# mushroomfire/mdapy

Measured on AMD Instinct MI355X. Metric: atoms/sec for neighbor+CNA on 10M-atom FCC Cu; 1/2/4/8-GPU scaling, higher is better.
Workload: dtype f64 (CNA pair tests: f32 filter + f64 finish, labels exact); 1 GPU; FCC Cu a=3.615, 136^3 cells per GPU (10061824 atoms/GPU, 10061824 total), build_neighbor(rc=0.854a=3.08721, max_neigh=16) + fixed-cutoff CNA as one C-ABI call (mdh_build_neighbor_fcna: lists and labels), positions resident in HBM; atoms_per_gpu=10061824, max_neigh=16, parallelism=single, world_size_checked=1, launched_by=single process

## Files before the change

### include/mdapy_amd.h

```cpp
#ifndef MDAPY_AMD_H
#define MDAPY_AMD_H

#include <stdint.h>

#ifdef __cplusplus
extern "C" {
#endif

#define MDH_HOST 0
#define MDH_DEVICE 1

#define MDH_OK 0
#define MDH_ERR_BOX (-1)
#define MDH_ERR_HIP (-2)
#define MDH_ERR_ARG (-3)
#define MDH_ERR_NOMEM (-4)

const char *mdh_last_error(void);
int mdh_version(void);
int mdh_device_count(void);
int mdh_set_device(int device);
int mdh_warm(void);
int mdh_min_max_i32(const int *v, int64_t n, int *min_max2, int space, void *stream);
int mdh_dense_codes_i32(const int *v, int64_t n, int low, int span, int *codes, int64_t *counts_span, int space, void *stream);
int mdh_release_workspace(void);
int64_t mdh_workspace_bytes(void);
int mdh_prof_enable(int on);
int mdh_prof_reset(void);
int mdh_prof_report(char *buf, int buflen);
int mdh_debug_set_neighbor_variant(int variant);
int mdh_debug_set_indirect(int on);
int mdh_debug_neighbor_plan(int *plan8);
int mdh_debug_set_fcna_variant(int variant);
int mdh_debug_track_counters(int on);
int mdh_debug_counters(int64_t *out4);
int mdh_debug_set_rdf_variant(int variant);
int mdh_debug_set_knn_variant(int variant);
int mdh_debug_set_sq_variant(int variant);
int mdh_debug_set_entropy_variant(int variant);
int mdh_debug_set_ptm_order_cap(int cap);
int mdh_debug_image_thresholds(double L, double *out4);

int mdh_parse_table(const char *text, int64_t nbytes, int text_space, int64_t nrows, int ncol, const int *kinds,
                    void *const *columns, int64_t *redo, int64_t redo_cap, int64_t *status4, int space, void *stream);
int mdh_debug_text_pow5(int q, uint64_t *out2);
int mdh_debug_parse_double(const char *s, int64_t len, double *out);
int64_t mdh_debug_assign_groups(const int *cells, int64_t n, int *head, int *count, int *rank);

int mdh_build_neighbor(const double *x, const double *y, const double *z, int64_t N, const double *box9,
                       const double *origin3, const int *boundary3, double rc, int *verlet, double *dist, int *nn,
                       int64_t max_neigh, int fill_pads, int space, void *stream);
int mdh_build_neighbor_keyed(const double *x, const double *y, const double *z, int64_t N, const double *box9,
                             const double *origin3, const int *boundary3, double rc, int *verlet, double *dist, int *nn,
                             int64_t max_neigh, int fill_pads, const int64_t *key, int space, void *stream);

int mdh_build_neighbor_fcna(const double *x, const double *y, const double *z, int64_t N, const double *box9,
                            const double *origin3, const int *boundary3, double rc, int *verlet, double *dist, int *nn,
                            int64_t max_neigh, int fill_pads, int *pattern, const int64_t *key, int space, void *stream);

int mdh_hint_cell_window(int axis, double frac_lo, double frac_hi);
int mdh_hint_centre_window(int axis, double frac_lo, double frac_hi);
int mdh_cell_window_check(void *stream);

int mdh_slab_halo_select(const double *x, const double *y, const double *z, int64_t n, const double *origin3_host,
                         const double *hi3_host, double up_from, double down_below, int *up, int *down, int64_t *counts_host,
                         const int64_t *gid, double *up_pack, double *down_pack, int64_t capacity, int space, void *stream);
int mdh_slab_halo_messages(const double *x, const double *y, const double *z, int64_t n, const double *origin3_host,
                           const double *hi3_host, double up_from, double down_below, const int64_t *gid,
                           const double *const *extras_host_array_of_device_pointers, int nextra, double *msg_up,
                           double *msg_down, int64_t cap, void *stream);
int mdh_slab_append_ghosts(const double *msg_from_left, const double *msg_from_right, int64_t cap, int64_t nl, int64_t nr,
                           double *const *columns_host_array_of_device_pointers, int ncol, int64_t *gid, int64_t n_owned,
                           void *stream);
int mdh_slab_append_ghosts_static(const double *msg_from_left, const double *msg_from_right, int64_t cap,
                                  double *const *columns_host_array_of_device_pointers, int ncol, int64_t *gid, int64_t n_owned,
                                  void *stream);
int mdh_slab_overflow_check(void);
int mdh_slab_reset_absent_rows(const double *x, int *verlet, double *dist, int *nn, int64_t first, int64_t n, int64_t max_neigh, double pad,
                               void *stream);

int mdh_order_statistic(const double *x, const double *y, const double *z, int64_t N, const double *box9, const double *origin3,
                        const int *boundary3, double *far_fraction, int space, void *stream);
int mdh_spatial_sort(const double *x, const double *y, const double *z, int64_t N, const double *box9, const double *origin3,
                     const int *boundary3, double *xs, double *ys, double *zs, int *perm, int64_t *n_sorted, int space, void *stream);
int mdh_permute(const void *in, const int *perm, int64_t N, int elem_bytes, int scatter, void *out, int space, void *stream);
int mdh_gather_positions(const double *x, const double *y, const double *z, const int *perm, int64_t N, double *xs, double *ys, double *zs,
                         int space, void *stream);
int mdh_translate_rows(const int *verlet_sorted, const double *dist_sorted, const int *nn_sorted, const int *perm, int64_t N,
                       int64_t M, int *verlet, double *dist, int *nn, int space, void *stream);

int mdh_neighbor_count(const double *x, const double *y, const double *z, int64_t N, const double *box9,
                       const double *origin3, const int *boundary3, double rc, int *nn, int *max_count, int space,
                       void *stream);

typedef int (*mdh_alloc_rows_fn)(void *user, int64_t N, int64_t M, int **verlet, double **dist);
int mdh_build_neighbor_exact(const double *x, const double *y, const double *z, int64_t N, const double *box9,
                             const double *origin3, const int *boundary3, double rc, int *nn, int64_t *width,
                             mdh_alloc_rows_fn alloc, void *user, int space, void *stream);
int mdh_build_neighbor_exact_keyed(const double *x, const double *y, const double *z, int64_t N, const double *box9,
                                   const double *origin3, const int *boundary3, double rc, int *nn, int64_t *width,
                                   mdh_alloc_rows_fn alloc, void *user, const int64_t *key, int space, void *stream);
int mdh_build_neighbor_exact_fcna(const double *x, const double *y, const double *z, int64_t N, const double *box9,
                                  const double *origin3, const int *boundary3, double rc, int *nn, int64_t *width,
                                  mdh_alloc_rows_fn alloc, void *user, int *pattern, const int64_t *key, int space, void *stream);

int mdh_sort_verlet_by_distance(int *verlet, double *dist, int64_t N, int64_t M, int sort_num, int space,
                                void *stream);

int mdh_wrap_positions(double *x, double *y, double *z, int64_t N, const double *box9, const double *origin3,
                       const int *boundary3, int space, void *stream);

int mdh_average_by_neighbor(double rc, const int *verlet, const double *dist, const int *nn, int64_t N, int64_t M,
                            const double *value, double *value_ave, int include_self, int space, void *stream);

// ... 153 lines not shown
```

### mdapy_amd/_lib.py

```python
from __future__ import annotations

import ctypes as C
import os

import numpy as np

_HERE = os.path.dirname(os.path.abspath(__file__))
LIB_PATH = os.path.join(_HERE, "csrc", "libmdapy_amd.so")

HOST, DEVICE = 0, 1
ERR_BOX, ERR_HIP, ERR_ARG, ERR_NOMEM = -1, -2, -3, -4

_lib = None

i64, dbl, cint, vp = C.c_int64, C.c_double, C.c_int, C.c_void_p
ALLOC_ROWS = C.CFUNCTYPE(C.c_int, C.c_void_p, C.c_int64, C.c_int64, C.POINTER(C.POINTER(C.c_int)), C.POINTER(C.POINTER(C.c_double)))

_SIGNATURES = {
    "mdh_last_error": [],
    "mdh_version": [],
    "mdh_device_count": [],
    "mdh_set_device": [cint],
    "mdh_warm": [],
    "mdh_min_max_i32": [vp, i64, vp, cint, vp],
    "mdh_dense_codes_i32": [vp, i64, cint, cint, vp, vp, cint, vp],
    "mdh_release_workspace": [],
    "mdh_workspace_bytes": [],
    "mdh_prof_enable": [cint],
    "mdh_prof_reset": [],
    "mdh_prof_report": [vp, cint],
    "mdh_debug_set_neighbor_variant": [cint],
    "mdh_debug_set_indirect": [cint],
    "mdh_debug_neighbor_plan": [vp],
    "mdh_debug_set_fcna_variant": [cint],
    "mdh_debug_track_counters": [cint],
    "mdh_debug_counters": [vp],
    "mdh_debug_set_rdf_variant": [cint],
    "mdh_debug_set_knn_variant": [cint],
    "mdh_debug_set_sq_variant": [cint],
    "mdh_debug_set_entropy_variant": [cint],
    "mdh_debug_set_ptm_order_cap": [cint],
    "mdh_debug_image_thresholds": [dbl, vp],
    "mdh_parse_table": [vp, i64, cint, i64, cint, vp, vp, vp, i64, vp, cint, vp],
    "mdh_debug_text_pow5": [cint, vp],
    "mdh_debug_parse_double": [C.c_char_p, i64, vp],
    "mdh_debug_assign_groups": [vp, i64, vp, vp, vp],
    "mdh_build_neighbor": [vp, vp, vp, i64, vp, vp, vp, dbl, vp, vp, vp, i64, cint, cint, vp],
    "mdh_slab_halo_select": [vp, vp, vp, i64, vp, vp, dbl, dbl, vp, vp, vp, vp, vp, vp, i64, cint, vp],
    "mdh_hint_cell_window": [cint, dbl, dbl],
    "mdh_hint_centre_window": [cint, dbl, dbl],
    "mdh_cell_window_check": [vp],
    "mdh_slab_halo_messages": [vp, vp, vp, i64, vp, vp, dbl, dbl, vp, vp, cint, vp, vp, i64, vp],
    "mdh_slab_append_ghosts": [vp, vp, i64, i64, i64, vp, cint, vp, i64, vp],
    "mdh_order_statistic": [vp, vp, vp, i64, vp, vp, vp, vp, cint, vp],
    "mdh_spatial_sort": [vp, vp, vp, i64, vp, vp, vp, vp, vp, vp, vp, vp, cint, vp],
    "mdh_permute": [vp, vp, i64, cint, cint, vp, cint, vp],
    "mdh_gather_positions": [vp, vp, vp, vp, i64, vp, vp, vp, cint, vp],
    "mdh_translate_rows": [vp, vp, vp, vp, i64, i64, vp, vp, vp, cint, vp],
    "mdh_slab_append_ghosts_static": [vp, vp, i64, vp, cint, vp, i64, vp],
    "mdh_slab_overflow_check": [],
    "mdh_slab_reset_absent_rows": [vp, vp, vp, vp, i64, i64, i64, dbl, vp],
    "mdh_build_neighbor_keyed": [vp, vp, vp, i64, vp, vp, vp, dbl, vp, vp, vp, i64, cint, vp, cint, vp],
    "mdh_build_neighbor_fcna": [vp, vp, vp, i64, vp, vp, vp, dbl, vp, vp, vp, i64, cint, vp, vp, cint, vp],
    "mdh_neighbor_count": [vp, vp, vp, i64, vp, vp, vp, dbl, vp, vp, cint, vp],
    "mdh_build_neighbor_exact": [vp, vp, vp, i64, vp, vp, vp, dbl, vp, vp, ALLOC_ROWS, vp, cint, vp],
    "mdh_build_neighbor_exact_keyed": [vp, vp, vp, i64, vp, vp, vp, dbl, vp, vp, ALLOC_ROWS, vp, vp, cint, vp],
    "mdh_build_neighbor_exact_fcna": [vp, vp, vp, i64, vp, vp, vp, dbl, vp, vp, ALLOC_ROWS, vp, vp, vp, cint, vp],
    "mdh_sort_verlet_by_distance": [vp, vp, i64, i64, cint, cint, vp],
    "mdh_wrap_positions": [vp, vp, vp, i64, vp, vp, vp, cint, vp],
    "mdh_average_by_neighbor": [dbl, vp, vp, vp, i64, i64, vp, vp, cint, cint, vp],
    "mdh_fcna": [vp, vp, vp, i64, vp, vp, vp, vp, i64, vp, vp, dbl, cint, vp],
    "mdh_acna": [vp, vp, vp, i64, vp, vp, vp, vp, i64, vp, cint, vp],
    "mdh_ids": [vp, vp, vp, i64, vp, vp, vp, vp, i64, vp, vp, cint, vp],
    "mdh_csp": [vp, vp, vp, i64, vp, vp, vp, vp, i64, cint, vp, cint, vp],
    "mdh_get_sq": [vp, vp, vp, i64, vp, vp, vp, vp, vp, i64, vp, vp, vp, cint, cint, cint, cint, cint, cint, cint,
                   dbl, cint, vp, vp, vp, cint, vp],
    "mdh_identify_solid_liquid": [cint, vp, vp, vp, vp, i64, i64, vp, vp, cint, cint, dbl, cint, vp, vp, cint, cint,
                                  dbl, cint, vp],
    "mdh_rdf": [vp, vp, vp, vp, i64, i64, vp, cint, dbl, cint, cint, vp],
    "mdh_rdf_single_species": [vp, vp, vp, i64, i64, vp, dbl, cint, cint, vp],
    "mdh_rdf_streaming": [vp, vp, vp, vp, i64, vp, vp, vp, vp, cint, dbl, cint, cint, vp],
    "mdh_bond_analysis": [vp, vp, vp, i64, vp, vp, vp, vp, vp, vp, i64, dbl, dbl, dbl, cint, vp, vp, cint, vp],
    "mdh_angular_distribution": [vp, vp, vp, i64, vp, vp, vp, vp, vp, vp, vp, i64, dbl, vp, vp, cint, cint, vp, cint, vp],
    "mdh_debug_angle_edges": [cint, dbl, vp],
    "mdh_debug_set_bond_variant": [cint],
    "mdh_strain_pack": [vp, vp, vp, i64, vp, vp, cint, vp],
    "mdh_atomic_strain_records": [vp, vp, i64, i64, vp, vp, vp, vp, vp, vp, vp, vp, vp, cint, vp],
    "mdh_atomic_strain": [vp, vp, i64, i64, vp, vp, vp, vp, vp, vp, vp, vp, vp, vp, vp, vp, vp, vp, cint, vp],
    "mdh_chill_plus": [vp, vp, vp, i64, vp, vp, vp, vp, vp, vp, i64, dbl, vp, cint, vp],
    "mdh_wcp": [vp, vp, vp, i64, i64, cint, vp, cint, vp],
    "mdh_wcp_counts": [vp, vp, vp, vp, i64, i64, cint, vp, cint, vp],
    "mdh_knn": [vp, vp, vp, i64, vp, vp, vp, cint, vp, vp, cint, vp],
    "mdh_knn_keyed": [vp, vp, vp, i64, vp, vp, vp, cint, vp, vp, vp, cint, vp],
    "mdh_knn_keyed_rows": [vp, vp, vp, i64, vp, vp, vp, cint, vp, vp, vp, vp, vp, cint, vp, cint, vp],
    "mdh_knn_rows_width": [cint],
    "mdh_repeat_cell": [vp, vp, vp, i64, cint, cint, cint, cint, vp],
    "mdh_ptm": [C.c_char_p, vp, vp, vp, i64, vp, vp, vp, vp, i64, vp, dbl, vp, cint, vp, cint, cint, vp],
    "mdh_ptm_flags": [C.c_char_p],
    "mdh_aja": [vp, vp, vp, i64, vp, vp, vp, vp, vp, i64, vp, cint, vp],
    "mdh_cnp": [vp, vp, vp, i64, vp, vp, vp, vp, vp, vp, i64, vp, dbl, cint, vp],
    "mdh_structure_entropy": [dbl, dbl, cint, dbl, vp, vp, i64, i64, vp, cint, vp],
    "mdh_atomic_temperature": [vp, vp, i64, i64, vp, vp, vp, vp, vp, dbl, cint, vp],
    "mdh_cluster": [vp, vp, vp, i64, i64, dbl, cint, vp, vp, cint, vp],
    "mdh_identify_sftb_fcc": [vp, i64, vp, vp, vp, i64, vp, cint, cint, vp],
    "mdh_filter_overlap_atom": [vp, vp, vp, i64, vp, vp, vp, dbl, vp, cint, vp],
    "mdh_voronoi_volume_number_radius": [vp, vp, vp, i64, vp, vp, vp, vp, vp, vp, cint, vp],
    "mdh_voronoi_neighbor_count": [vp, vp, vp, i64, vp, vp, vp, vp, vp, cint, vp],
    "mdh_voronoi_neighbor": [vp, vp, vp, i64, vp, vp, vp, dbl, dbl, vp, vp, vp, cint, cint, vp],
    "mdh_voronoi_neighbor_rows": [vp, vp, vp, i64, vp, vp, vp, dbl, dbl, vp, vp, vp, cint, vp, vp, cint, vp],
    "mdh_filter_overlap_atom_with_grain": [vp, vp, vp, vp, vp, i64, vp, vp, vp, dbl, dbl, dbl, vp, cint, vp],
    "mdh_transform_and_filter": [vp, vp, vp, i64, vp, vp, vp, vp, cint, vp, vp, cint, vp],
    "mdh_voronoi_cell_info": [vp, vp, vp, i64, vp, vp, vp, cint, cint, vp, vp, vp, vp, vp, vp, vp, cint, vp],
    "mdh_voronoi_row_distance": [vp, i64, cint, vp, vp, vp, vp, vp, vp, vp, cint, vp],
    "mdh_sfc_direct": [vp, vp, vp, i64, vp, vp, cint, dbl, dbl, vp, vp, vp, i64, C.c_uint, cint, vp],
    "mdh_sfc_direct_partial": [vp, vp, vp, vp, cint, i64, vp, vp, cint, dbl, dbl, cint, vp],
# ... 88 lines not shown
```

### mdapy_amd/csrc/cell_grid.hip

```cpp
#include "common.hpp"
#include "grid.hpp"
#include "assign_groups.hpp"
#include <algorithm>
#include <atomic>

namespace mdh {
static std::atomic<int> g_indirect{[] { const char *e = std::getenv("MDH_INDIRECT"); return e ? std::atoi(e) : 1; }()};

struct CellPlanes { int p0, p1, p2, p3; int *bad; };
template <bool TRI, int K>
__global__ __launch_bounds__(256) void k_assign(const double *__restrict__ x, const double *__restrict__ y,
                                                const double *__restrict__ z, int64_t N, DBox b, Grid g,
                                                int wrap_first, int2 *__restrict__ ent,
                                                unsigned *__restrict__ cell_count, unsigned *__restrict__ ctl, unsigned gen,
                                                double slack, unsigned short *__restrict__ mv, CellPlanes win,
                                                CellGrid::Packed *__restrict__ rec, int drop_absent)
{
    const int lane = threadIdx.x & 63;
    const int64_t i0 = ((int64_t)blockIdx.x * (blockDim.x >> 6) + (threadIdx.x >> 6)) * (64 * K) + lane;
    bool moved = false, outside = false, coded = false;
    double xr[K], yr[K], zr[K];
#pragma unroll
    for (int k = 0; k < K; ++k) {
        const int64_t i = i0 + 64 * k;
        xr[k] = yr[k] = zr[k] = 0.0;
        if (i < N) { xr[k] = x[i]; yr[k] = y[i]; zr[k] = z[i]; }
    }
    int cells[K];
#pragma unroll
    for (int k = 0; k < K; ++k) {
        const int64_t i = i0 + 64 * k;
        int cell = -1 - lane;
        const bool absent = drop_absent && i < N && xr[k] != xr[k];
        if (absent && mv) mv[i] = (unsigned short)img::ATOM_NEUTRAL;
        if (i < N && !absent) {
            double xi = xr[k], yi = yr[k], zi = zr[k];
            int code = img::ATOM_NEUTRAL;
            if (wrap_first && b.anypbc) {
                wrap<TRI>(b, xi, yi, zi);
                if (!TRI) {
                    const double raw[3] = {xr[k], yr[k], zr[k]}, wrp[3] = {xi, yi, zi};
                    code = 0;
#pragma unroll
                    for (int d = 0; d < 3; ++d) {
                        double m = 0.0;
                        if (b.pbc[d] && raw[d] != wrp[d]) {
                            m = rint((raw[d] - wrp[d]) / b.h[d * 4]);
                            if (!(fabs(m) <= (double)img::MAX_M) || !(fabs(raw[d] - m * b.h[d * 4] - wrp[d]) <= slack)) { moved = true; m = 0.0; }
                        }
                        code |= ((int)m + 15) << (5 * d);
                    }
                }
            }
            if (mv) mv[i] = (unsigned short)code;
            if (rec) rec[i] = CellGrid::Packed{xr[k], yr[k], zr[k], (int)i, code};
            coded = coded || code != img::ATOM_NEUTRAL;
            int c0, c1, c2;
            cell_coords<TRI>(b, g, xi, yi, zi, c0, c1, c2);
            cell = (c0 * g.nc[1] + c1) * g.nc[2] + c2;
            if (win.bad && !((c0 >= win.p0 && c0 < win.p1) || (c0 >= win.p2 && c0 < win.p3))) {
                outside = true;
                cell = -1 - lane;
            }
        }
        cells[k] = cell;
    }
    unsigned base[K];
    int head[K], slot[K];
#pragma unroll
    for (int k = 0; k < K; ++k) {
        const int cell = cells[k];
        const int c1 = __shfl_up(cell, 1, 64);
        const unsigned eq = assign_groups::equal_bits(cell, c1, __shfl_up(cell, 2, 64), __shfl_up(cell, 3, 64), lane);
        const unsigned long long primary = __ballot(eq == 0);
        int d = assign_groups::member_distance(eq, primary, lane);
        const bool start = assign_groups::starts_run(cell, c1, lane);
        const unsigned long long starts = __ballot(start);
        int count;
        if (assign_groups::use_runs(__popcll(__ballot(start && cell >= 0)), __popcll(__ballot(d == 0 && cell >= 0))))
            d = assign_groups::run_distance(starts, lane, &count, &slot[k]);
        else
            assign_groups::count_and_rank(d, __ballot(d == 1), __ballot(d == 2), __ballot(d == 3), lane, &count, &slot[k]);
        head[k] = lane - d;
        base[k] = 0;
        if (d == 0 && cell >= 0)
            base[k] = atomicAdd(&cell_count[cell], (unsigned)count);
    }
#pragma unroll
    for (int k = 0; k < K; ++k) {
        const unsigned bs = __shfl(base[k], head[k], 64);
        const int64_t i = i0 + 64 * k;
        if (i < N)
            ent[i] = make_int2(cells[k], (int)(bs + (unsigned)slot[k]));
    }
    if (__any(moved) && lane == 0)
        ctl[1] = gen;
    if (__any(coded) && lane == 0)
        ctl[2] = gen;
    if (__any(outside) && lane == 0)
        *win.bad = 1;
}

static constexpr int SCAN_BLOCK = 256;
static constexpr int SCAN_ITEMS = 4;
static constexpr int SCAN_ITEMS_BIG = 32;
static constexpr int64_t SCAN_BIG_FROM = 1 << 19;

__device__ __forceinline__ unsigned wave_incl_scan(unsigned v, int lane)
{
#pragma unroll
    for (int d = 1; d < 64; d <<= 1) {
        unsigned t = __shfl_up(v, d, 64);
        if (lane >= d) v += t;
    }
    return v;
}

__device__ __forceinline__ unsigned block_excl_scan(unsigned v, unsigned *tot)
{
    __shared__ unsigned wsum[4];
    const int lane = threadIdx.x & 63, w = threadIdx.x >> 6;
    unsigned inc = wave_incl_scan(v, lane);
    if (lane == 63) wsum[w] = inc;
    __syncthreads();
    unsigned off = 0, t = 0;
#pragma unroll
    for (int k = 0; k < 4; ++k) {
        if (k < w) off += wsum[k];
        t += wsum[k];
    }
    __syncthreads();
    *tot = t;
    return off + inc - v;
}

static std::atomic<unsigned> g_scan_gen{0};
static unsigned next_scan_gen()
{
    unsigned g = (++g_scan_gen) & 0x3fffffffu;
    if (g == 0) {
        reset_kept_blocks(Scope::KEEP_SCAN);
        g = (++g_scan_gen) & 0x3fffffffu;
    }
    return g;
}

template <bool REZERO, int ITEMS = SCAN_ITEMS>
__global__ __launch_bounds__(SCAN_BLOCK) void k_scan_onepass(unsigned *__restrict__ in, int *__restrict__ out, int64_t n,
                                                             unsigned *__restrict__ ctl, unsigned gen, int *__restrict__ flags)
{
    constexpr int SCAN_ITEMS = ITEMS;
    __shared__ unsigned s_blk, s_excl;
    unsigned long long *status = reinterpret_cast<unsigned long long *>(ctl + 64);
    const int tid = threadIdx.x, lane = tid & 63;
    if (tid == 0) s_blk = atomicAdd(&ctl[0], 1u);
    __syncthreads();
    const unsigned blk = s_blk, nblk = gridDim.x;
    if (tid == 0) {
        if (blk == nblk - 1) ctl[0] = 0;
        if (blk == 0 && flags) {
            flags[0] = ctl[1] == gen ? 1 : 0; flags[1] = 0; flags[2] = 0; flags[3] = 0;
            flags[4] = ctl[2] == gen ? 1 : 0; flags[5] = 0; flags[6] = 0; flags[7] = 0;
        }
    }
    const int64_t base = ((int64_t)blk * SCAN_BLOCK + tid) * SCAN_ITEMS;
    unsigned v[SCAN_ITEMS], s = 0;
    const bool vec = base + SCAN_ITEMS <= n && ((reinterpret_cast<uintptr_t>(in + base) | reinterpret_cast<uintptr_t>(out + base)) & 15u) == 0;
    if (vec) {
#pragma unroll
        for (int c = 0; c < SCAN_ITEMS / 4; ++c) {
            const uint4 q = reinterpret_cast<const uint4 *>(in + base)[c];
            v[4 * c] = q.x; v[4 * c + 1] = q.y; v[4 * c + 2] = q.z; v[4 * c + 3] = q.w;
        }
        if (REZERO) {
// ... 64 lines not shown
}

static size_t scan_ctl_bytes(int64_t n)
{
    const int64_t per = (int64_t)SCAN_BLOCK * SCAN_ITEMS;
    return 256 + (size_t)((n + per - 1) / per) * 8;
}
static void launch_scan_gen(hipStream_t st, unsigned *in, int *out, int64_t n, unsigned *ctl, unsigned gen, bool rezero, int *flags)
{
    const bool big = n >= SCAN_BIG_FROM;
    const int64_t per = (int64_t)SCAN_BLOCK * (big ? SCAN_ITEMS_BIG : SCAN_ITEMS);
    const dim3 grid((unsigned)std::max<int64_t>(1, (n + per - 1) / per)), block(SCAN_BLOCK);
    if (big) {
        if (rezero) hipLaunchKernelGGL((k_scan_onepass<true, SCAN_ITEMS_BIG>), grid, block, 0, st, in, out, n, ctl, gen, flags);
        else hipLaunchKernelGGL((k_scan_onepass<false, SCAN_ITEMS_BIG>), grid, block, 0, st, in, out, n, ctl, gen, flags);
    } else {
        if (rezero) hipLaunchKernelGGL((k_scan_onepass<true, SCAN_ITEMS>), grid, block, 0, st, in, out, n, ctl, gen, flags);
        else hipLaunchKernelGGL((k_scan_onepass<false, SCAN_ITEMS>), grid, block, 0, st, in, out, n, ctl, gen, flags);
    }
}
static void launch_scan(hipStream_t st, unsigned *in, int *out, int64_t n, unsigned *ctl, bool rezero, int *flags)
{
    launch_scan_gen(st, in, out, n, ctl, next_scan_gen(), rezero, flags);
}

int exclusive_scan_u32(Scope &sc, const unsigned *in, int *out, int64_t n)
{
    unsigned *ctl = static_cast<unsigned *>(sc.alloc_kept(scan_ctl_bytes(n), Scope::KEEP_SCAN));
    if (sc.failed())
        return sc.error();
    launch_scan(sc.stream(), const_cast<unsigned *>(in), out, n, ctl, false, nullptr);
    MDH_HIP(hipGetLastError());
    return MDH_OK;
}

__global__ __launch_bounds__(256) void k_scatter(const int2 *__restrict__ ent, const int *__restrict__ cell_start,
                                                 int *__restrict__ order, int64_t N)
{
    const int64_t i = 2 * ((int64_t)blockIdx.x * blockDim.x + threadIdx.x);
    if (i >= N)
        return;
    int4 e;
    if (i + 1 < N) e = *reinterpret_cast<const int4 *>(ent + i);
    else { const int2 last = ent[i]; e = make_int4(last.x, last.y, -1, 0); }
    if (e.x >= 0)
        order[cell_start[e.x] + e.y] = (int)i;
    if (e.z >= 0)
        order[cell_start[e.z] + e.w] = (int)(i + 1);
}

template <int W, typename K>
__device__ __forceinline__ void sort_cell_net(int *__restrict__ order, int s, int n, const int64_t *__restrict__ key)
{
    int id[W];
    K k[W];
#pragma unroll
    for (int u = 0; u < W; ++u) id[u] = order[s + min(u, n - 1)];
#pragma unroll
    for (int u = 0; u < W; ++u) {
        const K v = key ? (K)key[id[u]] : (K)id[u];
        k[u] = u < n ? v : (sizeof(K) == 8 ? (K)INT64_MIN : (K)INT32_MIN);
    }
    auto ce = [&](int a, int b) {
        const bool sw = k[a] < k[b];
        const K ka = sw ? k[b] : k[a], kb = sw ? k[a] : k[b];
        const int ia = sw ? id[b] : id[a], ib = sw ? id[a] : id[b];
        k[a] = ka; k[b] = kb; id[a] = ia; id[b] = ib;
    };
    if (W == 4) {
        ce(0, 1); ce(2, 3); ce(0, 2); ce(1, 3); ce(1, 2);
    } else {
        ce(0, 1); ce(2, 3); ce(4, 5); ce(6, 7);
        ce(0, 2); ce(1, 3); ce(4, 6); ce(5, 7);
        ce(1, 2); ce(5, 6);
        ce(0, 4); ce(1, 5); ce(2, 6); ce(3, 7);
        ce(2, 4); ce(3, 5);
        ce(1, 2); ce(3, 4); ce(5, 6);
    }
#pragma unroll
    for (int u = 0; u < W; ++u)
        if (u < n) order[s + u] = id[u];
}

__global__ __launch_bounds__(256) void k_sort_cells(const int *__restrict__ cell_start, int *__restrict__ order,
                                                    int64_t ncell, const int64_t *__restrict__ key, int *__restrict__ tmp)
{
    int64_t c = (int64_t)blockIdx.x * blockDim.x + threadIdx.x;
    if (c >= ncell)
        return;
    const int s = cell_start[c], e = cell_start[c + 1];
    const int n = e - s;
    if (n <= 1)
        return;
    if (n <= 4) {
        if (key) sort_cell_net<4, int64_t>(order, s, n, key);
        else sort_cell_net<4, int>(order, s, n, nullptr);
        return;
    }
    if (n <= 8) {
        if (key) sort_cell_net<8, int64_t>(order, s, n, key);
        else sort_cell_net<8, int>(order, s, n, nullptr);
        return;
    }
    if (!key && tmp) {
        for (int a = s; a < e; ++a) tmp[a] = order[a];
        for (int a = s; a < e; ++a) {
            const int mine = tmp[a];
            int larger = 0;
            for (int q = s; q < e; ++q) larger += tmp[q] > mine ? 1 : 0;
            order[s + larger] = mine;
        }
        return;
    }
    for (int a = s + 1; a < e; ++a) {
        int v = order[a], q = a - 1;
        const int64_t kv = key ? key[v] : (int64_t)v;
        while (q >= s && (key ? key[order[q]] : (int64_t)order[q]) < kv) {
            order[q + 1] = order[q];
            --q;
        }
        order[q + 1] = v;
    }
}

constexpr int SORT_DENSE_CAP = 64;
__global__ __launch_bounds__(256) void k_sort_cells_dense(const int *__restrict__ cell_start, int *__restrict__ order, int64_t ncell,
                                                          int *__restrict__ tmp)
{
    __shared__ int ids[32 * SORT_DENSE_CAP];
    const int sub = threadIdx.x & 7, lc = threadIdx.x >> 3;
    const int64_t c = (int64_t)blockIdx.x * 32 + lc;
    int s = 0, n = 0;
    if (c < ncell) {
        s = cell_start[c];
        n = cell_start[c + 1] - s;
    }
    const bool staged = n > 1 && n <= SORT_DENSE_CAP, big = n > SORT_DENSE_CAP;
    if (staged)
        for (int a = sub; a < n; a += 8) ids[lc * SORT_DENSE_CAP + a] = order[s + a];
    if (big)
        for (int a = sub; a < n; a += 8) tmp[s + a] = order[s + a];
    __syncthreads();
    if (staged) {
        for (int a = sub; a < n; a += 8) {
            const int mine = ids[lc * SORT_DENSE_CAP + a];
            int larger = 0;
            for (int q = 0; q < n; ++q) larger += ids[lc * SORT_DENSE_CAP + q] > mine ? 1 : 0;
            order[s + larger] = mine;
        }
    } else if (big) {
        for (int a = sub; a < n; a += 8) {
            const int mine = tmp[s + a];
            int larger = 0;
            for (int q = 0; q < n; ++q) larger += tmp[s + q] > mine ? 1 : 0;
            order[s + larger] = mine;
        }
    }
}

__global__ __launch_bounds__(256) void k_gather(const double *__restrict__ x, const double *__restrict__ y,
                                                const double *__restrict__ z, const int *__restrict__ order,
                                                double *__restrict__ xs, double *__restrict__ ys,
                                                double *__restrict__ zs, int64_t N,
                                                const unsigned short *__restrict__ mv, unsigned short *__restrict__ mvs,
                                                CellGrid::Packed *__restrict__ pk, const int *__restrict__ any_code,
                                                const int *__restrict__ n_binned)
{
    int64_t p = (int64_t)blockIdx.x * blockDim.x + threadIdx.x;
    if (p >= N)
        return;
    if (n_binned && p >= *n_binned)
        return;
    const int i = order[p];

    const double a = x[i], b = y[i], c = z[i];
    const unsigned short m = *any_code ? mv[i] : (unsigned short)img::ATOM_NEUTRAL;
    if (pk) {
        pk[p] = CellGrid::Packed{a, b, c, i, (int)m};
        return;
    }
    xs[p] = a;
    ys[p] = b;
    zs[p] = c;
    mvs[p] = m;
}

__global__ __launch_bounds__(256) void k_gather_records(const CellGrid::Packed *__restrict__ rec, const int *__restrict__ order,
                                                        CellGrid::Packed *__restrict__ pk, int64_t N, const int *__restrict__ n_binned)
{
    const int64_t p = (int64_t)blockIdx.x * blockDim.x + threadIdx.x;
    if (p >= N || p >= *n_binned)
        return;
    pk[p] = rec[order[p]];
}

__global__ __launch_bounds__(256) void k_unpack(const CellGrid::Packed *__restrict__ pk, int64_t N, double *__restrict__ xs,
                                                double *__restrict__ ys, double *__restrict__ zs, unsigned short *__restrict__ mvs)
{
    const int64_t p = (int64_t)blockIdx.x * blockDim.x + threadIdx.x;
    if (p >= N)
        return;
    const CellGrid::Packed r = pk[p];
    xs[p] = r.x; ys[p] = r.y; zs[p] = r.z; mvs[p] = (unsigned short)r.code;
}

int ensure_unpacked(Scope &sc, CellGrid &cg, int64_t N)
{
    if ((!cg.pk && !cg.ix) || cg.xs)
        return MDH_OK;
    cg.xs = sc.alloc_n<double>((size_t)N);
    cg.ys = sc.alloc_n<double>((size_t)N);
    cg.zs = sc.alloc_n<double>((size_t)N);
    cg.mvs = sc.alloc_n<unsigned short>((size_t)N);
    if (sc.failed())
        return sc.error();
    if (cg.pk)
        hipLaunchKernelGGL(k_unpack, dim3(grid_for(N, 256)), dim3(256), 0, sc.stream(), cg.pk, N, cg.xs, cg.ys, cg.zs, cg.mvs);
    else
        hipLaunchKernelGGL(k_gather, dim3(grid_for(N, 256)), dim3(256), 0, sc.stream(), cg.ix, cg.iy, cg.iz, cg.order, cg.xs, cg.ys, cg.zs, N, cg.imv,
                           cg.mvs, (CellGrid::Packed *)nullptr, cg.flags + 4, cg.cell_start + cg.g.ncell);
    MDH_HIP(hipGetLastError());
    return MDH_OK;
}

struct CellWindow { int axis = 0; double lo = 0.0, hi = 0.0; bool set = false; };
struct PendingWindows { CellWindow cells, centre; };
static thread_local PendingWindows g_pending;
static thread_local int *g_window_violations = nullptr;

static int take_pending_windows(PendingWindows &w)
{
    w = g_pending;
    g_pending = PendingWindows{};
    if (g_window_violations && *(volatile int *)g_window_violations != 0) {
        *g_window_violations = 0;
        set_error("an earlier neighbor build on this thread found atoms outside the cell window it had been promised (mdh_hint_cell_window)");
        return MDH_ERR_ARG;
    }
    return MDH_OK;
}
// ... 7 lines not shown
        return;
    }
    const int64_t a4 = (a + 3) & ~(int64_t)3, b4 = b & ~(int64_t)3;
    const int64_t q = a4 + 4 * i;
    if (q + 4 <= b4) *reinterpret_cast<int4 *>(out + q) = make_int4(val, val, val, val);
    if (i < 4) {
        if (a + i < a4) out[a + i] = val;
        if (b4 + i < b) out[b4 + i] = val;
    }
}
__global__ __launch_bounds__(256) void k_fill_outside(int *__restrict__ out, int64_t a0, int64_t a1, int64_t n1, const int *__restrict__ v)
{
    const int val = *v;
    const int64_t q = 4 * ((int64_t)blockIdx.x * blockDim.x + threadIdx.x);
    const int64_t head4 = (a0 + 3) >> 2 << 2;
    const int64_t t0 = (a1 + 1 + 3) & ~(int64_t)3;
    if (q < head4) {
        if (q + 4 <= a0) *reinterpret_cast<int4 *>(out + q) = make_int4(0, 0, 0, 0);
        else for (int64_t i = q; i < a0; ++i) out[i] = 0;
        return;
    }
    const int64_t r = q - head4 + t0;
    if (r == t0) for (int64_t i = a1 + 1; i < t0 && i < n1; ++i) out[i] = val;
    if (r + 4 <= n1) *reinterpret_cast<int4 *>(out + r) = make_int4(val, val, val, val);
    else for (int64_t i = r; i < n1; ++i) out[i] = val;
}
static void fill_from(hipStream_t st, int *out, int64_t a, int64_t b, const int *v)
{
    if (b > a)
        hipLaunchKernelGGL(k_fill_from, dim3(grid_for((b - a) / 4 + 8, 256)), dim3(256), 0, st, out, a, b, v);
}

__global__ __launch_bounds__(256) void k_add_from(int *__restrict__ out, int64_t a, int64_t b, const int *__restrict__ v, int64_t skip)
{
    const int64_t i = a + (int64_t)blockIdx.x * blockDim.x + threadIdx.x;
    if (i < b && i != skip) out[i] += *v;
}

int neighbor_grid_dims(const DBox &b, double rc, Grid &g)
{
    double nc_total = 1.0;
    for (int d = 0; d < 3; ++d) {
        double f = std::floor(b.thick[d] / rc);
        if (!(f < 2147483647.0)) { set_error("cell grid too large (box thickness / rc overflows int)"); return MDH_ERR_ARG; }
        int n = (int)f;
        g.nc[d] = n > 3 ? n : 3;
        nc_total *= (double)g.nc[d];
    }
    if (nc_total > 2147483000.0) {
        set_error("cell grid too large: " + std::to_string(nc_total) + " cells (the reference indexes cells with int32)");
        return MDH_ERR_ARG;
    }
    g.ncell = (int64_t)g.nc[0] * g.nc[1] * g.nc[2];
    g.rc_inv = 1.0 / rc;
    g.mode = 0;
    return MDH_OK;
}

__global__ __launch_bounds__(1024) void k_order_far_flag(const double *__restrict__ x, const double *__restrict__ y, const double *__restrict__ z,
                                                         int64_t N, DBox b, double nb0, double nb1, double nb2, int *__restrict__ flag)
{
    __shared__ int s_far;
    if (threadIdx.x == 0) s_far = 0;
    __syncthreads();
    const int64_t step = (N - 1) / 1024 > 0 ? (N - 1) / 1024 : 1;
    const int64_t i = (int64_t)threadIdx.x * step;
    bool far = false;
    if (i + 1 < N) {
        const double dx = x[i + 1] - x[i], dy = y[i + 1] - y[i], dz = z[i + 1] - z[i];
        double f[3] = {dx * b.hi[0] + dy * b.hi[3] + dz * b.hi[6], dx * b.hi[1] + dy * b.hi[4] + dz * b.hi[7], dx * b.hi[2] + dy * b.hi[5] + dz * b.hi[8]};
        const double nb[3] = {nb0, nb1, nb2};
#pragma unroll
        for (int d = 0; d < 3; ++d) {
            if (b.pbc[d]) f[d] -= rint(f[d]);
            far = far || !(fabs(f[d]) * nb[d] <= 2.0);
        }
    }
    const unsigned long long m = __ballot(far);
    if ((threadIdx.x & 63) == 0 && m) atomicAdd(&s_far, __popcll(m));
    __syncthreads();
    if (threadIdx.x == 0) *flag = 4 * s_far > 1024 ? 1 : 0;
}

int build_cell_grid(Scope &sc, const double *x, const double *y, const double *z, int64_t N, const DBox &b, const GridRequest &rq,
                    CellGrid &cg)
{
    PendingWindows hints;
    MDH_TRY(take_pending_windows(hints));
    const CellWindow &window = hints.cells, &centre = hints.centre;
    const bool packed = rq.atoms != GridRequest::SORTED_ARRAYS;
    bool scattered = rq.atoms == GridRequest::FOR_ROWS_UNORDERED;
    const Grid &g = cg.g;
    hipStream_t st = sc.stream();

    unsigned *cell_count = static_cast<unsigned *>(sc.alloc_kept(sizeof(unsigned) * (size_t)g.ncell, Scope::KEEP_ZERO));
    unsigned *ctl = static_cast<unsigned *>(sc.alloc_kept(scan_ctl_bytes(g.ncell), Scope::KEEP_SCAN));
    cg.flags = sc.alloc_n<int>(8);
    cg.cell_start = sc.alloc_n<int>((size_t)g.ncell + 1);
    int2 *ent = sc.alloc_n<int2>((size_t)N);
    int *rank = reinterpret_cast<int *>(ent);
    cg.order = sc.alloc_n<int>((size_t)N + 4);
    unsigned short *mv = sc.alloc_n<unsigned short>((size_t)N);
    cg.xs = cg.ys = cg.zs = nullptr;
    cg.mvs = nullptr;
    cg.pk = nullptr;
    CellGrid::Packed *rec = nullptr;
    int *rec_flag = nullptr;
    cg.ix = cg.iy = cg.iz = nullptr;
    cg.imv = nullptr;
    if (packed) {
        if (!scattered && N >= (int64_t(1) << 18)) {
            const OrderHint h = order_hint(1, N, g.ncell, x);
            scattered = h.word && *(volatile int *)h.word != 0;
            if (h.word && h.sample) rec_flag = h.word;
        }
        const bool indirect = g_indirect.load(std::memory_order_relaxed) != 0 && !scattered && rq.sort_desc && (double)N <= 6.0 * (double)g.ncell && rq.row_width <= 16;
        if (!indirect) cg.pk = sc.alloc_n<CellGrid::Packed>((size_t)N);
        if (scattered) rec = sc.alloc_n<CellGrid::Packed>((size_t)N);
    } else {
        cg.xs = sc.alloc_n<double>((size_t)N);
        cg.ys = sc.alloc_n<double>((size_t)N);
        cg.zs = sc.alloc_n<double>((size_t)N);
        cg.mvs = sc.alloc_n<unsigned short>((size_t)N);
    }
    if (sc.failed())
        return sc.error();

    int p0 = 0, p1 = g.nc[0], p2 = 0, p3 = 0;
    bool windowed = false;
    if (window.set) {
        const CellWindow &w = window;
        if (packed && w.axis == 0 && !b.tri && g.mode == 0 && g.nc[0] >= 16 && w.hi > w.lo && w.hi - w.lo < 0.75) {
            const double L = b.h[0];
            int lo = (int)std::floor(w.lo * L * g.rc_inv) - 1, hi = (int)std::ceil(w.hi * L * g.rc_inv) + 1;
            if (hi - lo < g.nc[0] - 2) {
                windowed = true;
                if (lo < 0) { p0 = 0; p1 = std::min(hi, g.nc[0]); p2 = g.nc[0] + lo; p3 = g.nc[0]; }
                else if (hi > g.nc[0]) { p0 = 0; p1 = hi - g.nc[0]; p2 = lo; p3 = g.nc[0]; }
                else { p0 = lo; p1 = hi; p2 = p3 = 0; }
                if (p2 < p1 && p3 > p2) { windowed = false; p0 = 0; p1 = g.nc[0]; p2 = p3 = 0; }
            }
        }
    }
    const int64_t plane = (int64_t)g.nc[1] * g.nc[2];
    cg.win_lo = cg.win_hi = 0;
    if (windowed && p3 <= p2) { cg.win_lo = p0; cg.win_hi = p1; }
    cg.cen_lo = cg.cen_hi = 0;
    if (centre.set) {
        const CellWindow &c = centre;
        if (packed && c.axis == 0 && !b.tri && g.mode == 0 && c.hi > c.lo && c.lo >= 0.0 && c.hi <= 1.0) {
            const double L = b.h[0];
            cg.cen_lo = std::max(0, std::min(g.nc[0] - 1, (int)std::floor(c.lo * L * g.rc_inv * (1.0 - 1e-9) - 1e-9)));
            cg.cen_hi = std::min(g.nc[0], (int)std::floor(c.hi * L * g.rc_inv * (1.0 + 1e-9) + 1e-9) + 1);
        }
    }
    cg.flags_fresh = true;
    const double slack = 0.01 / (g.rc_inv > 0 ? g.rc_inv : 1.0);
    CellPlanes win{p0, p1, p2, p3, nullptr};
    if (windowed) {
        if (!g_window_violations) MDH_HIP(hipHostMalloc(reinterpret_cast<void **>(&g_window_violations), sizeof(int), hipHostMallocDefault));
        *g_window_violations = 0;
        win.bad = g_window_violations;
    }
    if (rec_flag) {
        const double *h = b.h;
        const double vol = std::fabs(h[0] * (h[4] * h[8] - h[5] * h[7]) - h[1] * (h[3] * h[8] - h[5] * h[6]) + h[2] * (h[3] * h[7] - h[4] * h[6]));
        const double edge = std::cbrt(64.0 * vol / (double)N);
        double nb[3];
        for (int d = 0; d < 3; ++d) nb[d] = std::max(1.0, std::floor(b.thick[d] / edge));
        hipLaunchKernelGGL(k_order_far_flag, dim3(1), dim3(1024), 0, st, x, y, z, N, b, nb[0], nb[1], nb[2], rec_flag);
    }
    const unsigned gen = next_scan_gen();
    const bool assign4 = N >= (int64_t)1 << 20 && !scattered;
#define MDH_ASSIGN(TRI, K) hipLaunchKernelGGL((k_assign<TRI, K>), dim3(grid_for(N, 256 * K)), dim3(256), 0, st, x, y, z, N, b, g, (int)rq.wrap_first, ent, cell_count, ctl, gen, slack, mv, win, rec, packed ? 1 : 0)
    if (b.tri) {
        if (assign4) MDH_ASSIGN(true, 4); else MDH_ASSIGN(true, 1);
    } else {
        if (assign4) MDH_ASSIGN(false, 4); else MDH_ASSIGN(false, 1);
    }
#undef MDH_ASSIGN
    auto scan_piece = [&](int64_t from, int64_t to, unsigned use_gen, int *flags) {
        launch_scan_gen(st, cell_count + from, cg.cell_start + from, to - from, ctl, use_gen, true, flags);
    };
    if (!windowed) {
        scan_piece(0, g.ncell, gen, cg.flags);
    } else {
        const int64_t a0 = p0 * plane, a1 = p1 * plane, b0 = p2 * plane, b1 = p3 * plane;
        hipError_t fill_err = hipSuccess;
        auto fill_const = [&](int64_t from, int64_t to, int v) {
            if (to > from && fill_err == hipSuccess)
                fill_err = hipMemsetD32Async(reinterpret_cast<hipDeviceptr_t>(cg.cell_start + from), v, (size_t)(to - from), st);
        };
        if (b1 > b0) fill_const(0, a0, 0);
        scan_piece(a0 & ~(int64_t)3, a1, gen, cg.flags);
        if (b1 <= b0) {
            const int64_t n1 = g.ncell + 1, quads = ((a0 + 3) >> 2) + ((n1 - std::min(n1, (a1 + 1 + 3) & ~(int64_t)3) + 3) >> 2) + 1;
            hipLaunchKernelGGL(k_fill_outside, dim3(grid_for(quads, 256)), dim3(256), 0, st, cg.cell_start, a0, a1, n1, cg.cell_start + a1);
        } else if (b1 > b0) {
            fill_from(st, cg.cell_start, a1 + 1, b0, cg.cell_start + a1);
            scan_piece(b0, b1, next_scan_gen(), nullptr);
            hipLaunchKernelGGL(k_add_from, dim3(grid_for(b1 - b0 + 1, 256)), dim3(256), 0, st, cg.cell_start, b0, b1 + 1, cg.cell_start + a1, (int64_t)-1);
            if (b1 < g.ncell)
                fill_from(st, cg.cell_start, b1 + 1, g.ncell + 1, cg.cell_start + b1);
        }
        MDH_HIP(fill_err);
    }
    sc.keep_confirm(cell_count);
    hipLaunchKernelGGL(k_scatter, dim3(grid_for((N + 1) / 2, 256)), dim3(256), 0, st, ent, cg.cell_start, cg.order, N);
    if (rq.sort_desc) {
        if (!windowed && !rq.sort_key && (double)N > 6.0 * (double)g.ncell) {
            hipLaunchKernelGGL(k_sort_cells_dense, dim3(grid_for(g.ncell, 32)), dim3(256), 0, st, cg.cell_start, cg.order, g.ncell, rank);
        } else if (!windowed) {
            hipLaunchKernelGGL(k_sort_cells, dim3(grid_for(g.ncell, 256)), dim3(256), 0, st, cg.cell_start, cg.order, g.ncell, rq.sort_key, rank);
        } else {
            hipLaunchKernelGGL(k_sort_cells, dim3(grid_for((p1 - p0) * plane, 256)), dim3(256), 0, st, cg.cell_start + p0 * plane, cg.order, (p1 - p0) * plane, rq.sort_key, rank);
            if (p3 > p2)
                hipLaunchKernelGGL(k_sort_cells, dim3(grid_for((p3 - p2) * plane, 256)), dim3(256), 0, st, cg.cell_start + p2 * plane, cg.order, (p3 - p2) * plane, rq.sort_key, rank);
        }
    }
    const int *n_binned = cg.cell_start + g.ncell;
    if (packed && !cg.pk) { cg.ix = x; cg.iy = y; cg.iz = z; cg.imv = mv; }
    else if (rec) hipLaunchKernelGGL(k_gather_records, dim3(grid_for(N, 256)), dim3(256), 0, st, rec, cg.order, cg.pk, N, n_binned);
    else hipLaunchKernelGGL(k_gather, dim3(grid_for(N, 256)), dim3(256), 0, st, x, y, z, cg.order, cg.xs, cg.ys, cg.zs, N, mv, cg.mvs, cg.pk, cg.flags + 4, n_binned);
    MDH_HIP(hipGetLastError());
    return MDH_OK;
}

}

using namespace mdh;

extern "C" {

int mdh_hint_centre_window(int axis, double frac_lo, double frac_hi)
{
    g_pending.centre = CellWindow{axis, frac_lo, frac_hi, true};
    return MDH_OK;
}

int mdh_hint_cell_window(int axis, double frac_lo, double frac_hi)
{
    g_pending.cells = CellWindow{axis, frac_lo, frac_hi, true};
    return MDH_OK;
}

int mdh_cell_window_check(void *stream)
{
    if (!g_window_violations)
        return MDH_OK;
    MDH_HIP(hipStreamSynchronize(reinterpret_cast<hipStream_t>(stream)));
    if (*(volatile int *)g_window_violations != 0) {
        *g_window_violations = 0;
        set_error("the last neighbor build on this thread found atoms outside the cell window it had been promised (mdh_hint_cell_window): its rows are incomplete");
        return MDH_ERR_ARG;
    }
    return MDH_OK;
}

int mdh_debug_set_indirect(int on) { return g_indirect.exchange(on ? 1 : 0); }
}

MDH_WARM_UNIT(cell_grid)

extern "C" int64_t mdh_debug_assign_groups(const int *cells, int64_t n, int *head, int *count, int *rank)
{
    int64_t atomics = 0;
    for (int64_t s0 = 0; s0 < n; s0 += 64) {
        int c[64], h[64], k[64], r[64];
        for (int l = 0; l < 64; ++l) c[l] = s0 + l < n ? cells[s0 + l] : -1 - l;
        mdh::assign_groups::slice(c, h, k, r);
        for (int l = 0; l < 64 && s0 + l < n; ++l) {
            head[s0 + l] = h[l]; count[s0 + l] = k[l]; rank[s0 + l] = r[l];
            atomics += k[l] > 0 && c[l] >= 0 ? 1 : 0;
        }
    }
    return atomics;
}
```

### mdapy_amd/csrc/common.hpp

```cpp
#pragma once
#include <hip/hip_runtime.h>
#include <stdint.h>
#include <string>
#include "../../include/mdapy_amd.h"

namespace mdh {

struct DBox {
    double h[9];
    double hi[9];
    double o[3];
    double thick[3];
    double tn[3][4];
    int pbc[3];
    int tri;
    int anypbc;
};

int make_box(DBox &b, const double *box9, const double *origin3, const int *boundary3);

__device__ __forceinline__ double pbc_axis(double d, double L, const double *t)
{
    double n;
    if (d >= t[0] && d < t[3])
// ... 4 lines not shown
}

template <bool TRI>
__device__ __forceinline__ void pbc(const DBox &b, double &dx, double &dy, double &dz)
{
    if (TRI) {
        double fx = dx * b.hi[0] + dy * b.hi[3] + dz * b.hi[6];
        double fy = dx * b.hi[1] + dy * b.hi[4] + dz * b.hi[7];
        double fz = dx * b.hi[2] + dy * b.hi[5] + dz * b.hi[8];
        if (b.pbc[0]) fx -= floor(fx + 0.5);
        if (b.pbc[1]) fy -= floor(fy + 0.5);
        if (b.pbc[2]) fz -= floor(fz + 0.5);
        dx = fx * b.h[0] + fy * b.h[3] + fz * b.h[6];
        dy = fx * b.h[1] + fy * b.h[4] + fz * b.h[7];
        dz = fx * b.h[2] + fy * b.h[5] + fz * b.h[8];
    } else {
        if (b.pbc[0]) dx = pbc_axis(dx, b.h[0], b.tn[0]);
        if (b.pbc[1]) dy = pbc_axis(dy, b.h[4], b.tn[1]);
        if (b.pbc[2]) dz = pbc_axis(dz, b.h[8], b.tn[2]);
    }
}

__device__ __forceinline__ double wrap_count(double d, double L)
{
    if (d >= 0.0 && d < L * 0.999999999999)
        return 0.0;
    return floor(d / L);
}

template <bool TRI>
__device__ __forceinline__ void wrap(const DBox &b, double &x, double &y, double &z)
{
    if (TRI) {
        double dx = x - b.o[0], dy = y - b.o[1], dz = z - b.o[2];
        double fx = dx * b.hi[0] + dy * b.hi[3] + dz * b.hi[6];
        double fy = dx * b.hi[1] + dy * b.hi[4] + dz * b.hi[7];
        double fz = dx * b.hi[2] + dy * b.hi[5] + dz * b.hi[8];
        if (b.pbc[0]) fx -= floor(fx);
        if (b.pbc[1]) fy -= floor(fy);
        if (b.pbc[2]) fz -= floor(fz);
        x = b.o[0] + fx * b.h[0] + fy * b.h[3] + fz * b.h[6];
        y = b.o[1] + fx * b.h[1] + fy * b.h[4] + fz * b.h[7];
        z = b.o[2] + fx * b.h[2] + fy * b.h[5] + fz * b.h[8];
    } else {
        if (b.pbc[0]) { double d = x - b.o[0]; x = b.o[0] + d - b.h[0] * wrap_count(d, b.h[0]); }
        if (b.pbc[1]) { double d = y - b.o[1]; y = b.o[1] + d - b.h[4] * wrap_count(d, b.h[4]); }
        if (b.pbc[2]) { double d = z - b.o[2]; z = b.o[2] + d - b.h[8] * wrap_count(d, b.h[8]); }
    }
}

template <bool TRI>
__device__ __forceinline__ double pair_d2(const DBox &b, double xi, double yi, double zi, double xj, double yj,
                                          double zj)
{
    double dx = xj - xi, dy = yj - yi, dz = zj - zi;
    pbc<TRI>(b, dx, dy, dz);
    return dx * dx + dy * dy + dz * dz;
}

void set_error(const std::string &msg);
int hip_fail(hipError_t e, const char *what, const char *file, int line);

#define MDH_HIP(call)                                                         \
    do {                                                                      \
        hipError_t e__ = (call);                                              \
        if (e__ != hipSuccess)                                                \
            return ::mdh::hip_fail(e__, #call, __FILE__, __LINE__);           \
    } while (0)

#define MDH_TRY(expr)                                                         \
    do {                                                                      \
        int rc__ = (expr);                                                    \
        if (rc__ != MDH_OK)                                                   \
            return rc__;                                                      \
    } while (0)

class Scope {
  public:
    explicit Scope(void *stream);
    ~Scope();
    hipStream_t stream() const { return stream_; }
    void *alloc(size_t bytes);
    template <class T> T *alloc_n(size_t n) { return static_cast<T *>(alloc((n ? n : 1) * sizeof(T))); }
    enum Keep { KEEP_NONE = 0, KEEP_ZERO = 1, KEEP_SCAN = 2, KEEP_TODO = 3 };
    void *alloc_kept(size_t bytes, Keep tag);
    void keep_confirm(void *p);

    template <class T> T *stage(T *p, size_t n, int space, bool in, bool out)
    {
        return static_cast<T *>(stage_raw(const_cast<void *>(static_cast<const void *>(p)), n * sizeof(T), space, in, out));
    }
    template <class T> const T *stage_in(const T *p, size_t n, int space)
    {
        return static_cast<const T *>(stage_raw(const_cast<T *>(p), n * sizeof(T), space, true, false));
    }
    int finish(int space);
    bool failed() const { return failed_; }
    int error() const { return err_; }

  private:
    void *stage_raw(void *p, size_t bytes, int space, bool in, bool out);
    struct Out { void *host; void *dev; size_t bytes; };
    hipStream_t stream_;
    int device_;
    bool failed_ = false;
    int err_ = MDH_ERR_NOMEM;
    static const int kMaxHeld = 64;
    void *held_[kMaxHeld];
    size_t held_bytes_[kMaxHeld];
    unsigned char held_keep_[kMaxHeld];
    int nheld_ = 0;
    void *alloc_impl(size_t bytes, int tag);
    Out outs_[16];
    int nouts_ = 0;
};

void reset_kept_blocks(int tag);

struct OrderHint { int *word; bool sample; };
OrderHint order_hint(int tag, int64_t a, int64_t b, const void *array);

struct __attribute__((aligned(16))) Pos4 { double x, y, z, w; };
typedef int RowQuad __attribute__((ext_vector_type(4), aligned(4)));
template <int NI>
__device__ __forceinline__ void load_row(const int *__restrict__ row, int (&ids)[NI])
{
#pragma unroll
    for (int q = 0; q < NI / 4; ++q) {
        const RowQuad v = *reinterpret_cast<const RowQuad *>(row + 4 * q);
        ids[4 * q] = v.x; ids[4 * q + 1] = v.y; ids[4 * q + 2] = v.z; ids[4 * q + 3] = v.w;
    }
#pragma unroll
    for (int a = NI & ~3; a < NI; ++a) ids[a] = row[a];
}
const Pos4 *pack_positions(Scope &sc, const double *x, const double *y, const double *z, int64_t N);

constexpr int ROW_CHUNK = 16;
typedef double RowPair __attribute__((ext_vector_type(2), aligned(8)));
template <bool WITH_DIST>
__device__ __forceinline__ void stage_row_chunk(const int *__restrict__ verlet, const double *__restrict__ dist, int64_t N, int64_t M,
                                                int64_t row0, int c0, int *__restrict__ ids, double *__restrict__ dst)
{
    const int t = threadIdx.x;
#pragma unroll
    for (int e = t; e < 64 * (ROW_CHUNK / 4); e += 64) {
        const int row = e / (ROW_CHUNK / 4), c = (e % (ROW_CHUNK / 4)) * 4;
        const int64_t i = row0 + row;
        if (i < N && c0 + c < M) {
            const int *src = verlet + i * M + c0 + c;
            if (c0 + c + 3 < M) {
                const RowQuad v = *reinterpret_cast<const RowQuad *>(src);
                ids[(c + 0) * 64 + row] = v.x; ids[(c + 1) * 64 + row] = v.y; ids[(c + 2) * 64 + row] = v.z; ids[(c + 3) * 64 + row] = v.w;
            } else {
                for (int k = 0; c0 + c + k < M; ++k) ids[(c + k) * 64 + row] = src[k];
            }
        }
    }
    if (WITH_DIST) {
#pragma unroll
        for (int e = t; e < 64 * (ROW_CHUNK / 2); e += 64) {
            const int row = e / (ROW_CHUNK / 2), c = (e % (ROW_CHUNK / 2)) * 2;
            const int64_t i = row0 + row;
            if (i < N && c0 + c < M) {
                const double *src = dist + i * M + c0 + c;
                if (c0 + c + 1 < M) {
                    const RowPair v = *reinterpret_cast<const RowPair *>(src);
                    dst[(c + 0) * 64 + row] = v.x; dst[(c + 1) * 64 + row] = v.y;
                } else {
                    dst[c * 64 + row] = src[0];
// ... 35 lines not shown
```

### mdapy_amd/csrc/grid.hpp

```cpp
#pragma once
#include "common.hpp"
#include <cmath>

namespace mdh {

struct Grid {
    int nc[3];
    int64_t ncell;
    double rc_inv;
    int mode;
};

namespace img {
constexpr int MAX_M = 14;
constexpr int ATOM_NEUTRAL = 15 | (15 << 5) | (15 << 10);
constexpr int CELL_NEUTRAL = 1 | (1 << 2) | (1 << 4);
constexpr int NEUTRAL = 16 | (16 << 5) | (16 << 10);
__host__ __device__ __forceinline__ int combine(int cc, int ca)
{
    return ((cc & 3) + (ca & 31)) | ((((cc >> 2) & 3) + ((ca >> 5) & 31)) << 5) | ((((cc >> 4) & 3) + ((ca >> 10) & 31)) << 10);
}
__host__ __device__ __forceinline__ int axis(int code, int d) { return ((code >> (5 * d)) & 31) - 16; }
}

struct CellGrid {
    Grid g;
    int win_lo = 0, win_hi = 0;
    int cen_lo = 0, cen_hi = 0;
    mutable bool flags_fresh = false;
    int *cell_start;
    int *order;
    double *xs, *ys, *zs;
    int *flags;
    unsigned short *mvs;
    struct Packed { double x, y, z; int id, code; };
    Packed *pk;
    const double *ix = nullptr, *iy = nullptr, *iz = nullptr;
    const unsigned short *imv = nullptr;
};
struct SortedView {
    const double *xs, *ys, *zs;
    const int *order;
    const CellGrid::Packed *pk;
    bool indirect;
    __device__ __forceinline__ void get(int64_t q, double &x, double &y, double &z, int &id) const
    {
        if (pk) { const CellGrid::Packed r = pk[q]; x = r.x; y = r.y; z = r.z; id = r.id; }
        else if (indirect) { id = order[q]; x = xs[id]; y = ys[id]; z = zs[id]; }
        else { x = xs[q]; y = ys[q]; z = zs[q]; id = order[q]; }
    }
    __device__ __forceinline__ int id_of(int64_t q) const { return pk ? pk[q].id : order[q]; }
};
inline SortedView view_of(const CellGrid &cg)
{
    if (!cg.pk && !cg.xs && cg.ix) return SortedView{cg.ix, cg.iy, cg.iz, cg.order, nullptr, true};
    return SortedView{cg.xs, cg.ys, cg.zs, cg.order, cg.pk, false};
}
int ensure_unpacked(Scope &sc, CellGrid &cg, int64_t N);

struct TiledPlan {
    int tile;
    int tile_z;
    bool cellshift;
    bool full;
    int64_t occupied;
};
struct TileFilter {
    const unsigned char *flag = nullptr;
    const int *any = nullptr;
    const int *moved = nullptr;
    const int *list = nullptr;
    int list_cap = 0;
    int *cna_todo = nullptr;
    int tile = 1, tile_z = 1;
    int nt[3] = {1, 1, 1};
    int *listed_sink = nullptr;
};
TiledPlan plan_tiled(const DBox &b, const Grid &g, int64_t N, int64_t M, int64_t occupied_cells);
int occupied_cells_hint(Scope &sc, const CellGrid &cg, int64_t N, int64_t *occupied);

struct RowsRequest {
    enum Pads { COUNT_ONLY, KEEP_PADS, WRITE_PADS };
    int *verlet = nullptr;
    double *dist = nullptr;
    int *nn = nullptr;
    int64_t M = 1;
    Pads pads = WRITE_PADS;
    bool ids_only = false;
    int *max_count = nullptr;
    int *pattern = nullptr, *todo = nullptr;
};
int launch_neighbor_tiled(Scope &sc, const CellGrid &cg, const TiledPlan &plan, int64_t N, const DBox &b, double rc,
                          const RowsRequest &rows, TileFilter &tf);

struct GridStats {
    static constexpr int NBIN = 99;
    int v[NBIN];
    int last_listed = -1;
    int *listed_sink = nullptr;
};
struct LanePlan {
    int txy, tz;
    int cap;
    bool tk8;
    int wgs;
    int rw;
    float mid, T;
    int last_listed = -1; int *listed_sink = nullptr;
    bool full;
    int64_t occupied;
};
int grid_stats_hint(Scope &sc, const CellGrid &cg, int64_t N, GridStats *out);
LanePlan plan_lane(const DBox &b, const Grid &g, int64_t N, int64_t M, const GridStats &gs, double rc, bool fcna, bool count);
int lane_last_listed();
int launch_neighbor_lane(Scope &sc, const CellGrid &cg, const LanePlan &plan, int64_t N, const DBox &b, double rc,
                         const RowsRequest &rows, TileFilter &tf);
int neighbor_rows_device(Scope &sc, const double *dx, const double *dy, const double *dz, int64_t N, const DBox &b, double rc, int *dv,
                         double *dd, int *dn, int64_t M, const int64_t *dkey, bool ids_only);
void launch_fcna_all(hipStream_t st, const DBox &b, const double *x, const double *y, const double *z, int64_t N, const int *verlet,
                     int64_t M, const int *nn, int *pattern, double rc, int *todo, int *done = nullptr, const Pos4 *pos = nullptr, const int *use_pos = nullptr);
void launch_fcna_listed(hipStream_t st, const DBox &b, const double *x, const double *y, const double *z, int64_t N, const int *verlet,
                        int64_t M, const int *nn, int *pattern, double rc, int *todo, int *done = nullptr);

__host__ __device__ __forceinline__ int pmod(int a, int n)
{
    int r = a % n;
    return r < 0 ? r + n : r;
}

template <bool TRI>
__device__ __forceinline__ void cell_coords(const DBox &b, const Grid &g, double x, double y, double z, int &c0,
                                            int &c1, int &c2)
{
    double f0, f1, f2;
    if (TRI) {
        double dx = x - b.o[0], dy = y - b.o[1], dz = z - b.o[2];
        double nx = dx * b.hi[0] + dy * b.hi[3] + dz * b.hi[6];
        double ny = dx * b.hi[1] + dy * b.hi[4] + dz * b.hi[7];
        double nz = dx * b.hi[2] + dy * b.hi[5] + dz * b.hi[8];
        if (g.mode == 0) {
            f0 = floor(nx * b.thick[0] * g.rc_inv);
            f1 = floor(ny * b.thick[1] * g.rc_inv);
            f2 = floor(nz * b.thick[2] * g.rc_inv);
        } else {
            f0 = floor(nx * g.nc[0]);
            f1 = floor(ny * g.nc[1]);
            f2 = floor(nz * g.nc[2]);
        }
    } else if (g.mode == 0) {
        f0 = floor((x - b.o[0]) * g.rc_inv);
        f1 = floor((y - b.o[1]) * g.rc_inv);
        f2 = floor((z - b.o[2]) * g.rc_inv);
    } else {
        f0 = floor((x - b.o[0]) / b.h[0] * g.nc[0]);
        f1 = floor((y - b.o[1]) / b.h[4] * g.nc[1]);
        f2 = floor((z - b.o[2]) / b.h[8] * g.nc[2]);
    }
    f0 = fmin(fmax(f0, 0.0), (double)(g.nc[0] - 1));
    f1 = fmin(fmax(f1, 0.0), (double)(g.nc[1] - 1));
    f2 = fmin(fmax(f2, 0.0), (double)(g.nc[2] - 1));
    c0 = (int)f0;
    c1 = (int)f1;
    c2 = (int)f2;
}

int neighbor_grid_dims(const DBox &b, double rc, Grid &g);

struct GridRequest {
    enum Atoms { SORTED_ARRAYS, FOR_ROWS, FOR_ROWS_UNORDERED };
    bool wrap_first = false;
    bool sort_desc = false;
    const int64_t *sort_key = nullptr;
    Atoms atoms = SORTED_ARRAYS;
    int row_width = 0;
};
int build_cell_grid(Scope &sc, const double *x, const double *y, const double *z, int64_t N, const DBox &b, const GridRequest &rq,
                    CellGrid &cg);

int exclusive_scan_u32(Scope &sc, const unsigned *in, int *out, int64_t n);

}
```

### mdapy_amd/csrc/neighbor.hip

```cpp
#include "common.hpp"
#include "grid.hpp"
#include "cna_core.hpp"
#include <algorithm>
#include <mutex>
#include <vector>

namespace mdh {

static int *g_moved_probe = nullptr;
int g_neighbor_variant = 0;

template <bool TRI, int MODE>
__device__ __forceinline__ int neighbor_one(const SortedView &sv, const int *__restrict__ cell_start, const DBox &b,
                                            const Grid &g, double rc, int *__restrict__ verlet, double *__restrict__ dist,
                                            int *__restrict__ nn, int64_t M, int64_t p, double xi, double yi, double zi, int c0, int c1,
                                            int c2)
{
    int cnt = 0;
    const int i = sv.id_of(p);
    const double rcsq = rc * rc;
    const int64_t row = (int64_t)i * M;
    const bool zrun = (c2 >= 1) && (c2 + 1 < g.nc[2]);
    for (int a = c0 - 1; a <= c0 + 1; ++a) {
        const int ca = pmod(a, g.nc[0]);
        for (int bb = c1 - 1; bb <= c1 + 1; ++bb) {
            const int64_t base = ((int64_t)ca * g.nc[1] + pmod(bb, g.nc[1])) * g.nc[2];
            for (int seg = 0; seg < (zrun ? 1 : 3); ++seg) {
                int s, e;
                if (zrun) {
                    s = cell_start[base + c2 - 1];
                    e = cell_start[base + c2 + 2];
                } else {
                    const int cc = pmod(c2 - 1 + seg, g.nc[2]);
                    s = cell_start[base + cc];
                    e = cell_start[base + cc + 1];
                }
                for (int q0 = s; q0 < e; q0 += 4) {
                    double xq[4], yq[4], zq[4];
                    int jq[4];
#pragma unroll
                    for (int u = 0; u < 4; ++u)
                        sv.get(min(q0 + u, e - 1), xq[u], yq[u], zq[u], jq[u]);
#pragma unroll
                    for (int u = 0; u < 4; ++u) {
                        if (q0 + u >= e || jq[u] == i)
                            continue;
                        double dx = xq[u] - xi, dy = yq[u] - yi, dz = zq[u] - zi;
                        pbc<TRI>(b, dx, dy, dz);
                        const double d2 = dx * dx + dy * dy + dz * dz;
                        if (d2 <= rcsq) {
                            if (MODE != 0 && cnt < M) {
                                verlet[row + cnt] = jq[u];
                                dist[row + cnt] = sqrt(d2);
                            }
                            ++cnt;
                        }
                    }
                }
            }
        }
    }
    nn[i] = cnt;
    if (MODE == 2) {
        const double pad = rc + 1.0;
        for (int64_t n = cnt; n < M; ++n) {
            verlet[row + n] = -1;
            dist[row + n] = pad;
        }
    }
    return cnt;
}

template <bool TRI, int MODE>
__device__ __forceinline__ int neighbor_one_wave(const SortedView &sv, const int *__restrict__ cell_start, const DBox &b,
                                                 const Grid &g, double rc, int *__restrict__ verlet, double *__restrict__ dist,
                                                 int *__restrict__ nn, int64_t M, int64_t p, double xi, double yi, double zi, int c0,
                                                 int c1, int c2)
{
    const int lane = (int)(threadIdx.x & 63);
    int cnt = 0;
    const int i = sv.id_of(p);
    const double rcsq = rc * rc;
    const int64_t row = (int64_t)i * M;
    const bool zrun = (c2 >= 1) && (c2 + 1 < g.nc[2]);
    for (int a = c0 - 1; a <= c0 + 1; ++a) {
        const int ca = pmod(a, g.nc[0]);
        for (int bb = c1 - 1; bb <= c1 + 1; ++bb) {
            const int64_t base = ((int64_t)ca * g.nc[1] + pmod(bb, g.nc[1])) * g.nc[2];
            for (int seg = 0; seg < (zrun ? 1 : 3); ++seg) {
                int s, e;
                if (zrun) {
                    s = cell_start[base + c2 - 1];
                    e = cell_start[base + c2 + 2];
                } else {
                    const int cc = pmod(c2 - 1 + seg, g.nc[2]);
                    s = cell_start[base + cc];
                    e = cell_start[base + cc + 1];
                }
                for (int q0 = s; q0 < e; q0 += 64) {
                    const int q = q0 + lane;
                    bool hit = false;
                    int j = -1;
                    double d2 = 0.0;
                    if (q < e) {
                        double xq, yq, zq;
                        sv.get(q, xq, yq, zq, j);
                        double dx = xq - xi, dy = yq - yi, dz = zq - zi;
                        pbc<TRI>(b, dx, dy, dz);
                        d2 = dx * dx + dy * dy + dz * dz;
                        hit = j != i && d2 <= rcsq;
                    }
                    const unsigned long long m = __ballot(hit);
                    if (MODE != 0 && hit) {
                        const int slot = cnt + __popcll(m & ((1ull << lane) - 1ull));
                        if (slot < M) {
                            verlet[row + slot] = j;
                            dist[row + slot] = sqrt(d2);
                        }
                    }
                    cnt += __popcll(m);
                }
            }
        }
    }
    if (lane == 0) nn[i] = cnt;
    if (MODE == 2) {
        const double pad = rc + 1.0;
        for (int64_t n = cnt + lane; n < M; n += 64) {
            verlet[row + n] = -1;
            dist[row + n] = pad;
        }
    }
    return cnt;
}

template <bool TRI, int MODE>
__device__ __forceinline__ void neighbor_atoms_body(const SortedView &sv,
                                                  const int *__restrict__ cell_start, int64_t N, const DBox &b, const Grid &g,
                                                  double rc, int *__restrict__ verlet, double *__restrict__ dist,
                                                  int *__restrict__ nn, int64_t M, int *__restrict__ max_count,
                                                  const TileFilter &tf)
{
    const bool take_all = tf.moved && *tf.moved != 0;
    if (tf.flag && !take_all && (tf.list || *tf.any == 0))
        return;
    int cnt = 0;
    N = min(N, (int64_t)cell_start[g.ncell]);
    for (int64_t base = (int64_t)blockIdx.x * blockDim.x; base < N; base += (int64_t)gridDim.x * blockDim.x) {
        const int64_t p = base + threadIdx.x;
        bool mine = p < N;
        int c0 = 0, c1 = 0, c2 = 0;
        double xi = 0, yi = 0, zi = 0;
        if (mine) {
            { int idp; sv.get(p, xi, yi, zi, idp); }
            if (b.anypbc)
                wrap<TRI>(b, xi, yi, zi);
            cell_coords<TRI>(b, g, xi, yi, zi, c0, c1, c2);
            if (tf.flag) {
                const int t = ((c0 / tf.tile) * tf.nt[1] + (c1 / tf.tile)) * tf.nt[2] + (c2 / tf.tile_z);
                mine = take_all || tf.flag[t] != 0;
            }
        }
        if (mine) {
            cnt = max(cnt, neighbor_one<TRI, MODE>(sv, cell_start, b, g, rc, verlet, dist, nn, M, p, xi, yi, zi, c0, c1, c2));
            if (tf.cna_todo) defer(tf.cna_todo, sv.id_of(p));
        }
    }
    if (MODE == 0) {
        int m = cnt;
#pragma unroll
        for (int d = 32; d >= 1; d >>= 1) {
            int t = __shfl_xor(m, d, 64);
            m = t > m ? t : m;
        }
        if ((threadIdx.x & 63) == 0 && m > __hip_atomic_load(max_count, __ATOMIC_RELAXED, __HIP_MEMORY_SCOPE_AGENT))
            atomicMax(max_count, m);
    }
}

template <bool TRI, int MODE>
__global__ __launch_bounds__(256) void k_neighbor(SortedView sv, const int *__restrict__ cell_start, int64_t N, DBox b, Grid g, double rc,
                                                  int *__restrict__ verlet, double *__restrict__ dist, int *__restrict__ nn, int64_t M,
                                                  int *__restrict__ max_count, TileFilter tf)
{
    neighbor_atoms_body<TRI, MODE>(sv, cell_start, N, b, g, rc, verlet, dist, nn, M, max_count, tf);
}

template <bool TRI, int MODE>
__device__ __forceinline__ void neighbor_tiles_body(const SortedView &sv,
                                                        const int *__restrict__ cell_start, const DBox &b, const Grid &g, double rc,
                                                        int *__restrict__ verlet, double *__restrict__ dist, int *__restrict__ nn,
                                                        int64_t M, int *__restrict__ max_count, const TileFilter &tf)
{
    if (tf.moved && *tf.moved != 0)
        return;
    const int nlist = min(*tf.any, tf.list_cap);
    int best = 0;
    const int ncol = tf.tile * tf.tile;
    const int wave = (int)(threadIdx.x >> 6), nwave = (int)(blockDim.x >> 6);
    constexpr int MOP_CHUNKS = 8;
    for (int64_t w8 = blockIdx.x; w8 < (int64_t)nlist * ncol * MOP_CHUNKS; w8 += gridDim.x) {
        const int64_t w = w8 / MOP_CHUNKS;
        const int chunk = (int)(w8 - w * MOP_CHUNKS);
        const int t = tf.list[w / ncol], colq = (int)(w % ncol);
        const int t2 = t % tf.nt[2], t1 = (t / tf.nt[2]) % tf.nt[1], t0 = t / (tf.nt[2] * tf.nt[1]);
        const int z0 = t2 * tf.tile_z, z1 = min(z0 + tf.tile_z, g.nc[2]);
        const int a = t0 * tf.tile + colq / tf.tile, c = t1 * tf.tile + colq % tf.tile;
        if (a < g.nc[0] && c < g.nc[1]) {
            const int64_t col = ((int64_t)a * g.nc[1] + c) * g.nc[2];
            const int s = cell_start[col + z0], e = cell_start[col + z1];
            for (int p = s + chunk * nwave + wave; p < e; p += nwave * MOP_CHUNKS) {
                double xi, yi, zi;
                { int idp; sv.get(p, xi, yi, zi, idp); }
                if (b.anypbc)
                    wrap<TRI>(b, xi, yi, zi);
                int c0, c1, c2;
                cell_coords<TRI>(b, g, xi, yi, zi, c0, c1, c2);
                best = max(best, neighbor_one_wave<TRI, MODE>(sv, cell_start, b, g, rc, verlet, dist, nn, M, p, xi, yi, zi, c0, c1, c2));
                if (tf.cna_todo && (threadIdx.x & 63) == 0) defer(tf.cna_todo, sv.id_of(p));
            }
        }
    }
    if (MODE == 0) {
#pragma unroll
        for (int d = 32; d >= 1; d >>= 1) best = max(best, __shfl_xor(best, d, 64));
        if ((threadIdx.x & 63) == 0 && best > __hip_atomic_load(max_count, __ATOMIC_RELAXED, __HIP_MEMORY_SCOPE_AGENT))
            atomicMax(max_count, best);
    }
}

template <bool TRI, int MODE>
__global__ __launch_bounds__(256) void k_neighbor_tiles(SortedView sv, const int *__restrict__ cell_start, DBox b, Grid g, double rc,
                                                        int *__restrict__ verlet, double *__restrict__ dist, int *__restrict__ nn, int64_t M,
                                                        int *__restrict__ max_count, TileFilter tf)
{
    neighbor_tiles_body<TRI, MODE>(sv, cell_start, b, g, rc, verlet, dist, nn, M, max_count, tf);
}

template <bool TRI, int MODE>
__global__ __launch_bounds__(256) void k_neighbor_mop(SortedView sv, const int *__restrict__ cell_start, int64_t N, DBox b, Grid g, double rc,
                                                      int *__restrict__ verlet, double *__restrict__ dist, int *__restrict__ nn, int64_t M,
                                                      int *__restrict__ max_count, TileFilter tf)
{
    if (tf.listed_sink && blockIdx.x == 0 && threadIdx.x == 0)
        *tf.listed_sink = min(*tf.any, tf.list_cap);
    if (tf.moved && *tf.moved != 0) neighbor_atoms_body<TRI, MODE>(sv, cell_start, N, b, g, rc, verlet, dist, nn, M, max_count, tf);
    else neighbor_tiles_body<TRI, MODE>(sv, cell_start, b, g, rc, verlet, dist, nn, M, max_count, tf);
}

template <int MODE>
static void launch_neighbor(hipStream_t st, const CellGrid &cg, int64_t N, const DBox &b, double rc, int *verlet,
                            double *dist, int *nn, int64_t M, int *max_count, TileFilter tf = TileFilter{})
{
    dim3 grid(std::min(grid_for(N, 256), tf.list ? 2048 : 8192)), block(256);
    if (tf.list) {
        if (b.tri)
            hipLaunchKernelGGL((k_neighbor_mop<true, MODE>), grid, block, 0, st, view_of(cg), cg.cell_start, N, b, cg.g, rc, verlet, dist, nn, M, max_count, tf);
        else
            hipLaunchKernelGGL((k_neighbor_mop<false, MODE>), grid, block, 0, st, view_of(cg), cg.cell_start, N, b, cg.g, rc, verlet, dist, nn, M, max_count, tf);
        return;
    }
    if (b.tri)
        hipLaunchKernelGGL((k_neighbor<true, MODE>), grid, block, 0, st, view_of(cg), cg.cell_start, N, b, cg.g, rc, verlet, dist, nn, M, max_count, tf);
    else
        hipLaunchKernelGGL((k_neighbor<false, MODE>), grid, block, 0, st, view_of(cg), cg.cell_start, N, b, cg.g, rc, verlet, dist, nn, M, max_count, tf);
}

template <int L>
__global__ __launch_bounds__(64) void k_sort_rows(int *__restrict__ verlet, double *__restrict__ dist, int64_t N, int M, int k,
                                                  unsigned inv_m)
{
    constexpr int ROWS = 64 / L;
    extern __shared__ __attribute__((aligned(16))) unsigned char sort_lds[];
    double *ld = reinterpret_cast<double *>(sort_lds);
    int *lv = reinterpret_cast<int *>(ld + (size_t)M * ROWS);
    const int64_t row0 = (int64_t)blockIdx.x * ROWS;
    const int rows = (int)((N - row0) < ROWS ? (N - row0) : ROWS);
    const int total = rows * M;
    const int t = threadIdx.x;
    double *__restrict__ gd = dist + row0 * M;
    int *__restrict__ gv = verlet + row0 * M;
    auto slot = [&](int e) {
        const int r = (int)__umulhi((unsigned)e, inv_m);
        return (e - r * M) * ROWS + r;
    };
    const bool vec = rows == ROWS && ((reinterpret_cast<uintptr_t>(dist) | reinterpret_cast<uintptr_t>(verlet)) & 15) == 0;
    if (vec) {
        {
            const double2 *gd2 = reinterpret_cast<const double2 *>(gd);
            const int4 *gv4 = reinterpret_cast<const int4 *>(gv);
#pragma unroll 4
            for (int p = t; p < (total >> 1); p += 64) {
                const double2 v = gd2[p];
                ld[slot(2 * p)] = v.x; ld[slot(2 * p + 1)] = v.y;
            }
#pragma unroll 4
            for (int p = t; p < (total >> 2); p += 64) {
                const int4 v = gv4[p];
                lv[slot(4 * p)] = v.x; lv[slot(4 * p + 1)] = v.y; lv[slot(4 * p + 2)] = v.z; lv[slot(4 * p + 3)] = v.w;
            }
        }
    } else {
        for (int e = t; e < total; e += 64) { const int s = slot(e); ld[s] = gd[e]; lv[s] = gv[e]; }
    }
    __syncthreads();
    const int r = t & (ROWS - 1), j = t / ROWS;
    const bool live = r < rows;
    const double *lr = ld + r;
    int first = k;
    if (live) {
        double s = __builtin_inf();
        for (int c = k + j; c < M; c += L) {
            const double v = lr[c * ROWS];
            if (v < s) s = v;
        }
#pragma unroll
        for (int w = ROWS; w < 64; w <<= 1) {
            const double o = __shfl_xor(s, w);
            if (o < s) s = o;
        }
        for (int a = k - 1; a >= 0; --a) {
            const double v = lr[a * ROWS];
            if (s < v) first = a;
            if (v < s) s = v;
        }
    }
#pragma unroll
    for (int w = 1; w < 64; w <<= 1) {
        const int o = __shfl_xor(first, w);
        first = o < first ? o : first;
    }
    bool moved = false;
    for (int a = first; a < k; ++a) {
        int best = a;
        double db = live ? lr[a * ROWS] : 0.0;
        if (live) {
            int c = a + 1 + j;
            for (; c + 3 * L < M; c += 4 * L) {
                const double v0 = lr[c * ROWS], v1 = lr[(c + L) * ROWS], v2 = lr[(c + 2 * L) * ROWS], v3 = lr[(c + 3 * L) * ROWS];
                if (v0 < db) { db = v0; best = c; }
                if (v1 < db) { db = v1; best = c + L; }
                if (v2 < db) { db = v2; best = c + 2 * L; }
                if (v3 < db) { db = v3; best = c + 3 * L; }
            }
            for (; c < M; c += L) {
                const double v = lr[c * ROWS];
                if (v < db) { db = v; best = c; }
            }
// ... 120 lines not shown
#pragma unroll
        for (int q = 0; q < ROW_CHUNK; ++q)
            if (c0 + q < n && dst[q * 64 + threadIdx.x] <= rc) { s += val[q]; ++cnt; }
    }
    if (on) out[i] = cnt > 0 ? s / cnt : 0.0;
}

template <bool TRI>
__global__ __launch_bounds__(256) void k_filter_overlap(const double *__restrict__ xs, const double *__restrict__ ys,
                                                        const double *__restrict__ zs, const int *__restrict__ order,
                                                        const int *__restrict__ cell_start, int64_t N, DBox b, Grid g,
                                                        double rc, unsigned char *__restrict__ keep)
{
    const int64_t p = (int64_t)blockIdx.x * blockDim.x + threadIdx.x;
    if (p >= N)
        return;
    const double xr = xs[p], yr = ys[p], zr = zs[p];
    double xw = xr, yw = yr, zw = zr;
    if (b.anypbc)
        wrap<TRI>(b, xw, yw, zw);
    int c0, c1, c2;
    cell_coords<TRI>(b, g, xw, yw, zw, c0, c1, c2);
    const int j = order[p];
    const double rcsq = rc * rc;
    bool hit = false;
    for (int a = c0 - 1; a <= c0 + 1 && !hit; ++a) {
        const int ca = pmod(a, g.nc[0]);
        for (int bb = c1 - 1; bb <= c1 + 1 && !hit; ++bb) {
            const int64_t base = ((int64_t)ca * g.nc[1] + pmod(bb, g.nc[1])) * g.nc[2];
            for (int cc = c2 - 1; cc <= c2 + 1 && !hit; ++cc) {
                const int64_t cell = base + pmod(cc, g.nc[2]);
                for (int q = cell_start[cell]; q < cell_start[cell + 1]; ++q) {
                    if (order[q] >= j)
                        continue;
                    double xi = xs[q], yi = ys[q], zi = zs[q];
                    if (b.anypbc)
                        wrap<TRI>(b, xi, yi, zi);
                    double dx = xr - xi, dy = yr - yi, dz = zr - zi;
                    pbc<TRI>(b, dx, dy, dz);
                    if (dx * dx + dy * dy + dz * dz <= rcsq) { hit = true; break; }
                }
            }
        }
    }
    keep[j] = hit ? 0 : 1;
}

__global__ __launch_bounds__(256) void k_max_i32(const int *__restrict__ v, int64_t n, int *__restrict__ out)
{
    int m = 0;
    for (int64_t i = (int64_t)blockIdx.x * blockDim.x + threadIdx.x; i < n; i += (int64_t)gridDim.x * blockDim.x) m = max(m, v[i]);
#pragma unroll
    for (int d = 32; d >= 1; d >>= 1) m = max(m, __shfl_xor(m, d, 64));
    if ((threadIdx.x & 63) == 0 && m > __hip_atomic_load(out, __ATOMIC_RELAXED, __HIP_MEMORY_SCOPE_AGENT)) atomicMax(out, m);
}

static int width_hint(int64_t N, int64_t ncell, int set)
{
    struct Entry { int64_t N, ncell; int width; };
    static std::mutex mu;
    static std::vector<Entry> table;
    std::lock_guard<std::mutex> lk(mu);
    for (auto &e : table)
        if (e.N == N && e.ncell == ncell) {
            if (set >= 0) e.width = set;
            return e.width;
        }
    if (set > 0) {
        if (table.size() >= 64) table.erase(table.begin());
        table.push_back(Entry{N, ncell, set});
    }
    return 0;
}

struct RowsDone { bool labelled = false; };
static int neighbor_pass(Scope &sc, const CellGrid &cg, const DBox &b, int64_t N, double rc, const RowsRequest &rows, RowsDone &out)
{
    hipStream_t st = sc.stream();
    const bool count = rows.pads == RowsRequest::COUNT_ONLY;
    out.labelled = false;
    if (!cg.flags_fresh) MDH_HIP(hipMemsetAsync(cg.flags + 2, 0, sizeof(int) * 2, st));
    cg.flags_fresh = false;
    TileFilter tf{};
    bool done = false;
    if (g_neighbor_variant == 0) {
        GridStats gs;
        MDH_TRY(grid_stats_hint(sc, cg, N, &gs));
        const bool cna = rows.pattern && !count;
        const LanePlan lp = plan_lane(b, cg.g, N, count ? 1 : rows.M, gs, rc, cna, count);
        if (lp.txy) {
            if (cna) tf.cna_todo = rows.todo;
            MDH_TRY(launch_neighbor_lane(sc, cg, lp, N, b, rc, rows, tf));
            done = true;
            out.labelled = cna;
        }
    }
    if (!done && !count && g_neighbor_variant != 1 && !b.tri) {
        int64_t occ = 0;
        MDH_TRY(occupied_cells_hint(sc, cg, N, &occ));
        const TiledPlan plan = plan_tiled(b, cg.g, N, rows.M, occ);
        if (plan.tile) {
            MDH_TRY(ensure_unpacked(sc, const_cast<CellGrid &>(cg), N));
            MDH_TRY(launch_neighbor_tiled(sc, cg, plan, N, b, rc, rows, tf));
        }
    }
    if (count) launch_neighbor<0>(st, cg, N, b, rc, nullptr, nullptr, rows.nn, 1, rows.max_count, tf);
    else if (rows.pads == RowsRequest::WRITE_PADS) launch_neighbor<2>(st, cg, N, b, rc, rows.verlet, rows.dist, rows.nn, rows.M, nullptr, tf);
    else launch_neighbor<1>(st, cg, N, b, rc, rows.verlet, rows.dist, rows.nn, rows.M, nullptr, tf);
    if (g_moved_probe)
        MDH_HIP(hipMemcpyAsync(g_moved_probe, cg.flags, sizeof(int), hipMemcpyDeviceToHost, st));
    MDH_HIP(hipGetLastError());
    return MDH_OK;
}

static GridRequest rows_grid(const int64_t *key, int64_t row_width)
{
    GridRequest rq;
    rq.wrap_first = rq.sort_desc = true; rq.sort_key = key; rq.atoms = GridRequest::FOR_ROWS;
    rq.row_width = (int)std::min<int64_t>(row_width, 1 << 20);
    return rq;
}

static int launch_labels(Scope &sc, const DBox &b, const double *dx, const double *dy, const double *dz, int64_t N, const RowsRequest &rows,
                          double rc, int *done, const RowsDone &pass)
{
    ProfRange pr("k_fcna", sc.stream());
    if (pass.labelled) launch_fcna_listed(sc.stream(), b, dx, dy, dz, N, rows.verlet, rows.M, rows.nn, rows.pattern, rc, rows.todo, done);
    else launch_fcna_all(sc.stream(), b, dx, dy, dz, N, rows.verlet, rows.M, rows.nn, rows.pattern, rc, rows.todo, done);
    MDH_HIP(hipGetLastError());
    sc.keep_confirm(done);
    return MDH_OK;
}

int neighbor_rows_device(Scope &sc, const double *dx, const double *dy, const double *dz, int64_t N, const DBox &b, double rc, int *dv,
                         double *dd, int *dn, int64_t M, const int64_t *dkey, bool ids_only)
{
    CellGrid cg;
    MDH_TRY(neighbor_grid_dims(b, rc, cg.g));
    MDH_TRY(build_cell_grid(sc, dx, dy, dz, N, b, rows_grid(dkey, M), cg));
    RowsRequest rows;
    rows.verlet = dv; rows.dist = dd; rows.nn = dn; rows.M = M;
    rows.pads = RowsRequest::WRITE_PADS; rows.ids_only = ids_only;
    RowsDone pass;
    return neighbor_pass(sc, cg, b, N, rc, rows, pass);
}

int moved_probe(int enable)
{
    if (enable > 0 && !g_moved_probe) {
        if (hipHostMalloc(reinterpret_cast<void **>(&g_moved_probe), sizeof(int), hipHostMallocDefault) != hipSuccess) { g_moved_probe = nullptr; return -1; }
        *g_moved_probe = -1;
    } else if (enable == 0 && g_moved_probe) {
        int *p = g_moved_probe;
        g_moved_probe = nullptr;
        (void)hipDeviceSynchronize();
        (void)hipHostFree(p);
    }
    return g_moved_probe ? *(volatile int *)g_moved_probe : -1;
}

}

using namespace mdh;

extern "C" {

int mdh_build_neighbor(const double *x, const double *y, const double *z, int64_t N, const double *box9,
                       const double *origin3, const int *boundary3, double rc, int *verlet, double *dist, int *nn,
                       int64_t max_neigh, int fill_pads, int space, void *stream)
{
    return mdh_build_neighbor_keyed(x, y, z, N, box9, origin3, boundary3, rc, verlet, dist, nn, max_neigh, fill_pads, nullptr,
                                    space, stream);
}

int mdh_build_neighbor_keyed(const double *x, const double *y, const double *z, int64_t N, const double *box9,
                             const double *origin3, const int *boundary3, double rc, int *verlet, double *dist, int *nn,
                             int64_t max_neigh, int fill_pads, const int64_t *key, int space, void *stream)
{
    return mdh_build_neighbor_fcna(x, y, z, N, box9, origin3, boundary3, rc, verlet, dist, nn, max_neigh, fill_pads, nullptr, key,
                                   space, stream);
}

int mdh_build_neighbor_fcna(const double *x, const double *y, const double *z, int64_t N, const double *box9,
                            const double *origin3, const int *boundary3, double rc, int *verlet, double *dist, int *nn,
                            int64_t max_neigh, int fill_pads, int *pattern, const int64_t *key, int space, void *stream)
{
    if (N < 0 || N >= 2147483647LL || !(rc > 0) || max_neigh <= 0) { set_error(pattern ? "mdh_build_neighbor_fcna: invalid N, rc or max_neigh" : "mdh_build_neighbor: invalid N, rc or max_neigh"); return MDH_ERR_ARG; }
    DBox b;
    MDH_TRY(make_box(b, box9, origin3, boundary3));
    if (N == 0)
        return MDH_OK;
    Scope sc(stream);
    const double *dx = sc.stage_in(x, (size_t)N, space), *dy = sc.stage_in(y, (size_t)N, space), *dz = sc.stage_in(z, (size_t)N, space);
    RowsRequest rows;
    rows.verlet = sc.stage(verlet, (size_t)(N * max_neigh), space, !fill_pads, true);
    rows.dist = sc.stage(dist, (size_t)(N * max_neigh), space, !fill_pads, true);
    rows.nn = sc.stage(nn, (size_t)N, space, false, true);
    rows.M = max_neigh; rows.pads = fill_pads ? RowsRequest::WRITE_PADS : RowsRequest::KEEP_PADS;
    int *done = nullptr;
    if (pattern) {
        rows.pattern = sc.stage(pattern, (size_t)N, space, true, true);
        done = static_cast<int *>(sc.alloc_kept(sizeof(int) * ((size_t)N + 1 + 64), Scope::KEEP_TODO));
// ... 262 lines not shown
```

### mdapy_amd/csrc/neighbor_lane.hip

```cpp
#include "common.hpp"
#include "grid.hpp"
#include "cna_core.hpp"
#include <algorithm>
#include <cmath>
#include <type_traits>
#include <cstdio>
#include <cstdlib>
#include <cstring>
#include <mutex>
#include <vector>

namespace mdh {
namespace lane {

constexpr int NW = 4;
constexpr int CEN_CAP = 80 * NW;
__host__ __device__ constexpr int ticket_row(int M, bool cna_rows) { return (cna_rows && ((M + 4) & ~3) < 28) ? 28 : ((M + 4) & ~3); }
static constexpr int NEUTRAL = img::CELL_NEUTRAL;
static constexpr int NEUTRAL3 = img::NEUTRAL;

struct FastDiv {
    unsigned mul, sh1, sh2, d;
    __device__ __forceinline__ unsigned div(unsigned n) const
    {
// ... 181 lines not shown
        if (j < len) {
            const double2 cj = lxy[k];
            const double d2 = exact_d2<TRI ? 2 : 1>(b, cj.x, cj.y, lz[k], xi, yi, zi, TRI ? 0 : lsh[k]);
            h = (d2 <= rcsq) && (!SELF || k != li);
        }
        m = m + m + (h ? 1u : 0u);
    }
    return m;
}

template <int NN, class Index>
__device__ __forceinline__ int lane_fcna_f32(Index index_of, const float4 *__restrict__ f4, float negc, float W)
{
    float ux[NN], uy[NN], uz[NN];
#pragma unroll
    for (int a = 0; a < NN; ++a) {
        const float4 c = f4[index_of(a)];
        ux[a] = c.x; uy[a] = c.y; uz[a] = c.z;
    }
    unsigned adj[NN];
#pragma unroll
    for (int a = 0; a < NN; ++a)
        adj[a] = 0;
    unsigned w = 0x7f7fffffu;
    pair_tests_f32_rev<NN, NN, 0>(ux, uy, uz, negc, adj, w);
    unsigned r[NN];
#pragma unroll
    for (int a = 0; a < NN; ++a)
        r[a] = adj[NN - 1 - a];
    if (w <= __float_as_uint(W))
        return -1;
    if constexpr (NN == 12) {
        if (fcc_certificate<NN>(r))
            return 1;
        return fcna_label_pairs<NN>(r);
    }
    return fcna_label_words<NN, RowsReg<NN>>(r, RowsReg<NN>(r));
}

__device__ __forceinline__ int bit_select(int m, int a, int b)
{
    int d;
    asm("v_bfi_b32 %0, %1, %2, %3" : "=v"(d) : "v"(m), "v"(a), "v"(b));
    return d;
}
__device__ __forceinline__ void quad_transpose(int (&P)[4][4], int odd1, int odd2)
{
#pragma unroll
    for (int pp = 0; pp < 4; pp += 2)
#pragma unroll
        for (int w = 0; w < 4; ++w) {
            const int x = bit_select(odd1, P[pp][w], P[pp + 1][w]);
            const int y = __builtin_amdgcn_mov_dpp(x, 0xB1, 0xF, 0xF, true);
            P[pp + 1][w] = bit_select(odd1, P[pp + 1][w], y);
            P[pp][w] = bit_select(odd1, y, P[pp][w]);
        }
#pragma unroll
    for (int pp = 0; pp < 2; ++pp)
#pragma unroll
        for (int w = 0; w < 4; ++w) {
            const int x = bit_select(odd2, P[pp][w], P[pp + 2][w]);
            const int y = __builtin_amdgcn_mov_dpp(x, 0x4E, 0xF, 0xF, true);
            P[pp + 2][w] = bit_select(odd2, P[pp + 2][w], y);
            P[pp][w] = bit_select(odd2, y, P[pp][w]);
        }
}

struct IndirectSrc { const double *x, *y, *z; const unsigned short *mv; const int *order; };
__device__ __forceinline__ CellGrid::Packed load_atom(const IndirectSrc &src, int id, int coded)
{
    int code = (int)img::ATOM_NEUTRAL;
    if (coded) code = src.mv[id];
    return CellGrid::Packed{src.x[id], src.y[id], src.z[id], id, code};
}
struct __attribute__((packed, aligned(4))) Ids4 { int v[4]; };
template <bool IND>
__device__ __forceinline__ CellGrid::Packed load_record(const CellGrid::Packed *__restrict__ pk, const IndirectSrc &src, int q, int coded)
{
    if (!IND)
        return pk[q];
    return load_atom(src, src.order[q], coded);
}

template <bool COUNT, bool TRI, bool LOOP, bool FCNA, bool TK8, bool IND = false>
__global__ __launch_bounds__(NW * 64, (TK8 && (!FCNA || !LOOP)) ? 16 / NW : 1) void k_neighbor_lane(
    const CellGrid::Packed *__restrict__ pk, const int *__restrict__ cell_start, DBox b,
    Grid g, double rc, float negc, float W, int *__restrict__ verlet, double *__restrict__ dist, int *__restrict__ nn,
    int M, int write_pads, int cap, int *__restrict__ flags, unsigned char *__restrict__ tile_flag, int nt0,
    int nt1, int nt2, Shape ts, const int *__restrict__ tile_list, const int *__restrict__ n_live, int list_mode,
    int *__restrict__ max_count, int *__restrict__ flagged, const int *__restrict__ parent, int parent_nt2, int nsub,
    int flag_slot, int *__restrict__ pattern, int *__restrict__ cna_todo, int jt0, int rw, int tile_base, int *__restrict__ listed_sink,
    int cen_lo, int cen_hi, IndirectSrc isrc)
{
    const int TXY = ts.txy, TZ = ts.tz;
    const int coded = IND ? flags[4] : 0;
    const int HXY = TXY + 2, HZ = TZ + 2, NH = HXY * HXY * HZ;

    extern __shared__ __attribute__((aligned(16))) unsigned char smem[];
    const int tid = threadIdx.x, lane = tid & 63;
    typedef typename std::conditional<TK8, unsigned char, unsigned short>::type Ticket;
    constexpr int JB = TK8 ? 5 : 8;
    float4 *f4 = reinterpret_cast<float4 *>(smem);
    double2 *lxy = reinterpret_cast<double2 *>(f4 + cap);
    double *lz = reinterpret_cast<double *>(lxy + cap);
    unsigned *cen = reinterpret_cast<unsigned *>(lz + cap);
    unsigned short *lsh = reinterpret_cast<unsigned short *>(cen + CEN_CAP);
    Ticket *tk = reinterpret_cast<Ticket *>(lsh + cap + (cap & 1));
    const unsigned f4_lds = (unsigned)(unsigned long)(lds_byte *)smem;
    const int TKS = ticket_row(M, false);
    const int wstride = max(rw * TKS, 256 / (int)sizeof(Ticket));
    auto hc = [&](int t) -> unsigned & { return reinterpret_cast<unsigned *>(tk + (size_t)(t >> 6) * wstride)[t & 63]; };
    __shared__ unsigned hr[NW * 64 + 2];
    __shared__ int scan_tmp[NW];
    __shared__ int s_flag[4];

    const double rcsq = rc * rc, pad = rc + 1.0;
    const double cw = rc;
    int vmax = 0;

    const int nlive = parent ? min(*n_live, nt0 * nt1 * parent_nt2) * nsub : ((list_mode && tile_list) ? *n_live : nt0 * nt1 * nt2);
    const int per = (nlive + 7) / 8;
    if (parent && listed_sink && blockIdx.x == 0 && tid == 0)
        *listed_sink = min(*n_live, nt0 * nt1 * parent_nt2);
    struct Tile { int id, T0, T1, T2; bool empty; };
    struct Halo { int cnt, src, img, hz; bool edge, centre; };
    auto tile_of = [&](int slot) {
        Tile t;
        int t0, t1, t2;
        if (parent) {
            const int pt = parent[slot / nsub];
            t2 = (pt % parent_nt2) * nsub + slot % nsub;
            t1 = (pt / parent_nt2) % nt1;
            t0 = pt / (parent_nt2 * nt1);
            t.id = (t0 * nt1 + t1) * nt2 + t2;
        } else {
            t.id = (list_mode && tile_list) ? tile_list[slot] : slot + tile_base;
            const unsigned col = ts.by_nt2.div((unsigned)t.id);
            t2 = t.id - (int)col * nt2;
            t0 = (int)ts.by_nt1.div(col);
            t1 = (int)col - t0 * nt1;
        }
        t.T0 = t0 * TXY; t.T1 = t1 * TXY; t.T2 = t2 * TZ;
        t.empty = t.T2 >= g.nc[2];
        return t;
    };
    auto halo_of = [&](const Tile &t) {
        Halo h{0, 0, NEUTRAL, 0, false, false};
        if (tid < NH && !t.empty) {
            const int hcol = (int)(((unsigned)tid * ts.mhz) >> 16);
            h.hz = tid - hcol * HZ;
            const int hx = (int)(((unsigned)hcol * ts.mhxy) >> 16), hy = hcol - hx * HXY;
            const int g0 = t.T0 + hx - 1, g1 = t.T1 + hy - 1, g2 = t.T2 + h.hz - 1;
            const bool in0 = b.pbc[0] ? (g0 >= -1 && g0 <= g.nc[0]) : (g0 >= 0 && g0 < g.nc[0]);
            const bool in1 = b.pbc[1] ? (g1 >= -1 && g1 <= g.nc[1]) : (g1 >= 0 && g1 < g.nc[1]);
            const bool in2 = b.pbc[2] ? (g2 >= -1 && g2 <= g.nc[2]) : (g2 >= 0 && g2 < g.nc[2]);
            if (in0 && in1 && in2) {
                const int a0 = g0 < 0 ? g0 + g.nc[0] : (g0 >= g.nc[0] ? g0 - g.nc[0] : g0);
                const int a1 = g1 < 0 ? g1 + g.nc[1] : (g1 >= g.nc[1] ? g1 - g.nc[1] : g1);
                const int a2 = g2 < 0 ? g2 + g.nc[2] : (g2 >= g.nc[2] ? g2 - g.nc[2] : g2);
                const int c = (a0 * g.nc[1] + a1) * g.nc[2] + a2;
                h.src = cell_start[c];
                h.cnt = cell_start[c + 1] - h.src;
                const int n0 = g0 < 0 ? 1 : (g0 >= g.nc[0] ? -1 : 0);
                const int n1 = g1 < 0 ? 1 : (g1 >= g.nc[1] ? -1 : 0);
                const int n2 = g2 < 0 ? 1 : (g2 >= g.nc[2] ? -1 : 0);
                h.img = (n0 + 1) | ((n1 + 1) << 2) | ((n2 + 1) << 4);
                h.edge = (!b.pbc[0] && (a0 == 0 || a0 == g.nc[0] - 1)) || (!b.pbc[1] && (a1 == 0 || a1 == g.nc[1] - 1)) ||
                         (!b.pbc[2] && (a2 == 0 || a2 == g.nc[2] - 1));
                h.centre = hx >= 1 && hx <= TXY && hy >= 1 && hy <= TXY && h.hz >= 1 && h.hz <= TZ && g0 < g.nc[0] && g1 < g.nc[1] && g2 < g.nc[2] &&
                           g0 >= cen_lo && g0 < cen_hi;
            }
        }
        return h;
    };
    auto request = [&](const Halo &h, double (&ra)[4], double (&rb)[4], double (&rc4)[4], int (&rd)[4], int (&rm)[4]) {
        Ids4 ids{};
        if (IND) ids = *reinterpret_cast<const Ids4 *>(isrc.order + h.src);
#pragma unroll
        for (int v = 0; v < 4; ++v) {
            const int q = h.cnt > 0 ? h.src + min(v, h.cnt - 1) : 0;
            const CellGrid::Packed a = IND ? load_atom(isrc, v < h.cnt ? ids.v[v] : (h.cnt > 0 ? ids.v[0] : 0), coded) : load_record<false>(pk, isrc, q, coded);
            ra[v] = a.x; rb[v] = a.y; rc4[v] = a.z; rd[v] = a.id; rm[v] = a.code;
        }
    };
    for (int jt = jt0 + (int)(blockIdx.x >> 3); jt < per; jt += (int)(gridDim.x >> 3)) {
        const int slot = (int)(blockIdx.x & 7) * per + jt;
        if (slot >= nlive)
            break;
        const Tile tile = tile_of(slot);
        STAMP(0);
        Halo cur = halo_of(tile);
#ifdef MDH_STAMPS
        asm volatile("" : "+v"(cur.src), "+v"(cur.cnt));
        STAMP(1);
#endif
        double pa[4], pb[4], pc[4];
        int pd[4], pm[4];
        request(cur, pa, pb, pc, pd, pm);
        if (flags[0] != 0)
            return;
        const int tile_id = tile.id, T0 = tile.T0, T1 = tile.T1, T2 = tile.T2;
        const int cnt = cur.cnt, src = cur.src, img = cur.img, hz = cur.hz;
        const bool edge = cur.edge, centre_cell = cur.centre;
        if (tid == 0) { s_flag[0] = 0; s_flag[1] = 0; s_flag[2] = 0; s_flag[3] = 0; }
        hc(tid) = (unsigned)cnt;

        int total2;
        const int off2 = excl_scan_block(cnt | (centre_cell ? cnt << 16 : 0), scan_tmp, &total2);
        const int total = total2 & 0xffff, ncentres = total2 >> 16;
        const int off0 = off2 & 0xffff, coff = off2 >> 16;
        bool ok = !(total > cap || ncentres > CEN_CAP);
        const bool no_centres = ncentres == 0;
        if (no_centres) ok = false;
        STAMP(2);
        if (ok && tid < NH && hz >= 1 && hz <= HZ - 2) {
            const unsigned k0 = (unsigned)off0 - hc(tid - 1), len = hc(tid - 1) + (unsigned)cnt + hc(tid + 1);
            hr[tid] = k0 | (len << 16);
            if (len > (TK8 ? 32u : 96u)) s_flag[2] = 1;
            if (TK8 && len > 12u) s_flag[3] = 1;
        }
        if (ok && cnt > 0) {
            double X0, Y0, Z0, XS, YS, ZS;
            const int code0 = combine_codes(img, img::ATOM_NEUTRAL);
            if (TRI) {
                const double f0 = (double)(T0 - 1) * (cw / b.thick[0]) + (double)img::axis(code0, 0);
                const double f1 = (double)(T1 - 1) * (cw / b.thick[1]) + (double)img::axis(code0, 1);
                const double f2 = (double)(T2 - 1) * (cw / b.thick[2]) + (double)img::axis(code0, 2);
                XS = b.o[0] + f0 * b.h[0] + f1 * b.h[3] + f2 * b.h[6];
                YS = b.o[1] + f0 * b.h[1] + f1 * b.h[4] + f2 * b.h[7];
                ZS = b.o[2] + f0 * b.h[2] + f1 * b.h[5] + f2 * b.h[8];
                X0 = XS; Y0 = YS; Z0 = ZS;
            } else {
                X0 = b.o[0] + (double)(T0 - 1) * cw; Y0 = b.o[1] + (double)(T1 - 1) * cw; Z0 = b.o[2] + (double)(T2 - 1) * cw;
                XS = X0 + b.h[0] * (double)img::axis(code0, 0); YS = Y0 + b.h[4] * (double)img::axis(code0, 1);
                ZS = Z0 + b.h[8] * (double)img::axis(code0, 2);
            }
            const float flo = (float)(-1.5 * cw);
            const float fhx = (float)(((double)HXY + 1.5) * cw), fhz = (float)(((double)HZ + 1.5) * cw);
            bool general = code0 != NEUTRAL3, far = false;
            auto stage4 = [&](int k, const double (&a)[4], const double (&bb)[4], const double (&c)[4], const int (&d)[4], const int (&m)[4]) {
#pragma unroll
                for (int v = 0; v < 4; ++v) {
                    if (k + v < cnt) {
                        int code = code0;
                        float ux, uy, uz;
                        if (TRI) {
                            double wx = a[v], wy = bb[v], wz = c[v];
                            wrap<true>(b, wx, wy, wz);
                            const double rx = wx - XS, ry = wy - YS, rz = wz - ZS;
                            ux = (float)rx; uy = (float)ry; uz = (float)rz;
                            if (edge) {
                                const double s0 = (rx * b.hi[0] + ry * b.hi[3] + rz * b.hi[6]) * (b.thick[0] / cw);
                                const double s1 = (rx * b.hi[1] + ry * b.hi[4] + rz * b.hi[7]) * (b.thick[1] / cw);
                                const double s2 = (rx * b.hi[2] + ry * b.hi[5] + rz * b.hi[8]) * (b.thick[2] / cw);
                                far = far || !(s0 >= -1.5 && s0 <= (double)HXY + 1.5 && s1 >= -1.5 && s1 <= (double)HXY + 1.5 && s2 >= -1.5 && s2 <= (double)HZ + 1.5);
                            }
                        } else {
                            ux = (float)(a[v] - XS); uy = (float)(bb[v] - YS); uz = (float)(c[v] - ZS);
                        }
                        if (!TRI && m[v] != img::ATOM_NEUTRAL) {
                            code = combine_codes(img, m[v]);
                            ux = (float)((a[v] - b.h[0] * (double)img::axis(code, 0)) - X0);
                            uy = (float)((bb[v] - b.h[4] * (double)img::axis(code, 1)) - Y0);
                            uz = (float)((c[v] - b.h[8] * (double)img::axis(code, 2)) - Z0);
                            general = true;
                        }
                        if (!TRI && edge)
                            far = far || !(ux >= flo && ux <= fhx && uy >= flo && uy <= fhx && uz >= flo && uz <= fhz);
                        const int p = off0 + k + v;
                        f4[p] = make_float4(ux, uy, uz, __int_as_float(d[v]));
                        lxy[p] = make_double2(a[v], bb[v]);
                        lz[p] = c[v];
                        lsh[p] = (unsigned short)code;
                        if (centre_cell) cen[coff + k + v] = (unsigned)p | ((unsigned)tid << 11);
                    }
                }
            };
            if (TK8) {
                for (int k = 0; k < cnt; k += 4) {
                    double a[4], bb[4], c[4];
                    int d[4], m[4];
#pragma unroll
                    for (int v = 0; v < 4; ++v) {
                        if (k == 0) { a[v] = pa[v]; bb[v] = pb[v]; c[v] = pc[v]; d[v] = pd[v]; m[v] = pm[v]; }
                        else {
                            const int q = src + min(k + v, cnt - 1);
                            const CellGrid::Packed r = load_record<IND>(pk, isrc, q, coded);
                            a[v] = r.x; bb[v] = r.y; c[v] = r.z; d[v] = r.id; m[v] = r.code;
                        }
                    }
                    stage4(k, a, bb, c, d, m);
                }
            } else {
                double a[4], bb[4], c[4];
                int d[4], m[4];
#pragma unroll
                for (int v = 0; v < 4; ++v) { a[v] = pa[v]; bb[v] = pb[v]; c[v] = pc[v]; d[v] = pd[v]; m[v] = pm[v]; }
                for (int k = 0; k < cnt; k += 4) {
                    double na[4], nb[4], nc[4];
                    int nd[4], nm[4];
#pragma unroll
                    for (int v = 0; v < 4; ++v) {
                        const int q = src + min(k + 4 + v, cnt - 1);
                        const CellGrid::Packed r = load_record<IND>(pk, isrc, q, coded);
                        na[v] = r.x; nb[v] = r.y; nc[v] = r.z; nd[v] = r.id; nm[v] = r.code;
                    }
                    stage4(k, a, bb, c, d, m);
#pragma unroll
                    for (int v = 0; v < 4; ++v) { a[v] = na[v]; bb[v] = nb[v]; c[v] = nc[v]; d[v] = nd[v]; m[v] = nm[v]; }
                }
            }
            if (general) s_flag[0] = 1;
            if (far) s_flag[1] = 1;
        }
        __syncthreads();
        STAMP(3);
        if (ok && (s_flag[1] | s_flag[2]))
            ok = false;
        if (!ok && !no_centres && tid == 0) {
            if (tile_flag) tile_flag[tile_id] = 1;
            flagged[atomicAdd(&flags[flag_slot], 1)] = tile_id;
        }
        const bool general_tile = s_flag[0] != 0;
        const bool short_runs = TK8 && s_flag[3] == 0;
        const int wv = tid >> 6;
        Ticket *tkw = tk + (size_t)wv * wstride;
        const int A2 = HXY * HZ;
        auto run_cell = [&](int cbv, int r) {
            const int r3 = (r * 11) >> 5;
            return cbv + __mul24(r3, A2 - 3 * HZ) + __mul24(r, HZ) - (A2 + HZ);
        };
        for (int cbase = (int)((unsigned)(wv - jt) & (unsigned)(NW - 1)) * rw; ok && cbase < ncentres; cbase += NW * rw) {
            const int q = cbase + lane;
            const bool mine = lane < rw && q < ncentres;
            int kept = 0, kept8 = 0, cb = 0, id = 0;
            double xi = 0, yi = 0, zi = 0;
            Ticket *my = tkw + (size_t)lane * TKS;
            if (mine) {
                const unsigned cv = cen[q];
                const int li = (int)(cv & 2047u);
                cb = (int)(cv >> 11);
                const float4 s = f4[li];
                constexpr bool WIDE = !TK8;
                unsigned hv[9], mk[9], mk2[WIDE ? 9 : 1], mk3[WIDE ? 9 : 1];
#pragma unroll
                for (int r = 0; r < 9; ++r)
                    hv[r] = hr[cb + ((r / 3 - 1) * HXY + (r % 3 - 1)) * HZ];
                unsigned w = 0x7f7fffffu;
                if (TK8 && short_runs) {
#pragma unroll
                    for (int r = 0; r < 9; ++r) {
                        const int len = (int)(hv[r] >> 16);
                        scan_run12_asm(f4_lds + ((hv[r] & 0xffffu) << 4), s.x, s.y, s.z, negc, mk[r], w);
                        mk[r] = (mk[r] << 20) & (~0u << ((32 - len) & 31)) & (len > 0 ? ~0u : 0u);
                    }
                } else {
#pragma unroll
                    for (int r = 0; r < 9; ++r) {
                        const int len = (int)(hv[r] >> 16), la = WIDE ? min(len, 32) : len;
                        scan_run_asm(f4_lds + ((hv[r] & 0xffffu) << 4), la, s.x, s.y, s.z, negc, mk[r], w);
                        mk[r] &= ~0u << (run_slots(la) - la);
                        if (TK8) mk[r] <<= (32 - run_slots(la)) & 31;
                        if (WIDE) {
                            const int lb = min(len - la, 32), lc = len - la - lb;
                            mk2[r] = 0;
                            mk3[r] = 0;
                            if (__builtin_amdgcn_ballot_w64(lb > 0)) {
                                scan_run_asm(f4_lds + (((hv[r] & 0xffffu) + 32u) << 4), lb, s.x, s.y, s.z, negc, mk2[r], w);
                                mk2[r] &= lb > 0 ? ~0u << (run_slots(lb) - lb) : 0u;
                                if (__builtin_amdgcn_ballot_w64(lc > 0)) {
                                    scan_run_asm(f4_lds + (((hv[r] & 0xffffu) + 64u) << 4), lc, s.x, s.y, s.z, negc, mk3[r], w);
                                    mk3[r] &= lc > 0 ? ~0u << (run_slots(lc) - lc) : 0u;
                                }
                            }
                        }
                    }
                }
                {
                    const int len = (int)(hv[4] >> 16), idx = li - (int)(hv[4] & 0xffffu);
                    if (TK8) mk[4] &= ~(0x80000000u >> idx);
                    else if (idx < 32) mk[4] &= ~(1u << (run_slots(min(len, 32)) - 1 - idx));
                    else if (idx < 64) mk2[4] &= ~(1u << (run_slots(min(len - 32, 32)) - 1 - (idx - 32)));
                    else mk3[4] &= ~(1u << (run_slots(len - 64) - 1 - (idx - 64)));
                }
                STAMP(4);
                {
// ... 218 lines not shown
                    }
                    if (g0 < maxk) {
                        const uint2 t4 = *reinterpret_cast<const uint2 *>(my + g0);
                        int k[4];
                        bool h[4];
#pragma unroll
                        for (int u = 0; u < 4; ++u) {
                            h[u] = g0 + u < kept;
                            const unsigned t = ((u < 2 ? t4.x : t4.y) >> (16 * (u & 1))) & 0xffffu;
                            const int r = h[u] ? (int)(t >> JB) : 4;
                            k[u] = (int)(hr[run_cell(cb, r)] & 0xffffu) + (h[u] ? (int)(t & ((1u << JB) - 1u)) : 0);
                        }
                        double2 cj[4];
                        double zj[4], d2[4];
                        int nid[4], sh[4];
#pragma unroll
                        for (int u = 0; u < 4; ++u) {
                            cj[u] = lxy[k[u]];
                            zj[u] = lz[k[u]];
                            nid[u] = __float_as_int(f4[k[u]].w);
                            sh[u] = (!TRI && general_tile) ? (int)lsh[k[u]] : 0;
                        }
                        bool slow = false;
                        double rr[4] = {pad, pad, pad, pad};
                        if (!ids_only) {
#pragma unroll
                        for (int u = 0; u < 4; ++u) {
                            if (TRI) d2[u] = exact_d2<2>(b, cj[u].x, cj[u].y, zj[u], xi, yi, zi, 0);
                            else if (general_tile) d2[u] = exact_d2<1>(b, cj[u].x, cj[u].y, zj[u], xi, yi, zi, sh[u]);
                            else d2[u] = exact_d2<0>(b, cj[u].x, cj[u].y, zj[u], xi, yi, zi, 0);
                            d2[u] = h[u] ? d2[u] : 1.0;
                            slow = slow || !sqrt_fast_ok(d2[u]);
                        }
                        if (__builtin_expect(__builtin_amdgcn_ballot_w64(slow) == 0, 1)) {
#pragma unroll
                            for (int u = 0; u < 4; ++u) rr[u] = sqrt_fast(d2[u]);
                        } else {
#pragma unroll
                            for (int u = 0; u < 4; ++u) rr[u] = sqrt(d2[u]);
                        }
                        }
#pragma unroll
                        for (int u = 0; u < 4; ++u) {
                            idv[u] = h[u] ? nid[u] : -1;
                            dv[u] = h[u] ? rr[u] : pad;
                        }
                    }
                    if (mine) {
                        if (write_pads && g0 + 4 <= M) {
                            *reinterpret_cast<Int4 *>(verlet + row + g0) = Int4{idv[0], idv[1], idv[2], idv[3]};
                            if (!ids_only) {
                                Int4 *dp = reinterpret_cast<Int4 *>(dist + row + g0);
                                dp[0] = Int4{__double2loint(dv[0]), __double2hiint(dv[0]), __double2loint(dv[1]), __double2hiint(dv[1])};
                                dp[1] = Int4{__double2loint(dv[2]), __double2hiint(dv[2]), __double2loint(dv[3]), __double2hiint(dv[3])};
                            }
                        } else {
#pragma unroll
                            for (int u = 0; u < 4; ++u)
                                if (g0 + u < M && (g0 + u < kept || write_pads)) {
                                    verlet[row + g0 + u] = idv[u];
                                    if (!ids_only) dist[row + g0 + u] = dv[u];
                                }
                        }
                    }
                }
                STAMP(6);
                __builtin_amdgcn_fence(__ATOMIC_RELEASE, "wavefront");
                __builtin_amdgcn_wave_barrier();
                STAMP(7);
            }
        }
        if (!LOOP)
            break;
        if (jt + (int)(gridDim.x >> 3) < per) lds_barrier();
    }
    if (COUNT) {
        int m = vmax;
#pragma unroll
        for (int d = 32; d >= 1; d >>= 1) m = max(m, __shfl_xor(m, d, 64));
        if (lane == 0 && m > __hip_atomic_load(max_count, __ATOMIC_RELAXED, __HIP_MEMORY_SCOPE_AGENT)) atomicMax(max_count, m);
    }
}

__global__ __launch_bounds__(256) void k_tile_live(const int *__restrict__ cell_start, Grid g, int nt0, int nt1, int nt2, Shape ts,
                                                   unsigned *__restrict__ live)
{
    const int t = blockIdx.x * blockDim.x + threadIdx.x;
    if (t >= nt0 * nt1 * nt2)
        return;
    const int t2 = t % nt2, t1 = (t / nt2) % nt1, t0 = t / (nt2 * nt1);
    const int z0 = t2 * ts.tz, z1 = min(z0 + ts.tz, g.nc[2]);
    bool any = false;
    for (int a = t0 * ts.txy; a < min((t0 + 1) * ts.txy, g.nc[0]) && !any; ++a)
        for (int c = t1 * ts.txy; c < min((t1 + 1) * ts.txy, g.nc[1]) && !any; ++c) {
            const int64_t col = ((int64_t)a * g.nc[1] + c) * g.nc[2];
            any = cell_start[col + z1] > cell_start[col + z0];
        }
    live[t] = any ? 1u : 0u;
}

__global__ __launch_bounds__(256) void k_tile_compact(const unsigned *__restrict__ live, const int *__restrict__ slot, int ntiles,
                                                      int *__restrict__ tile_list)
{
    const int t = blockIdx.x * blockDim.x + threadIdx.x;
    if (t < ntiles && live[t]) tile_list[slot[t]] = t;
}

__global__ __launch_bounds__(256) void k_grid_stats(const int *__restrict__ cell_start, Grid g, int *__restrict__ out)
{
    __shared__ int hist[GridStats::NBIN];
    for (int k = threadIdx.x; k < GridStats::NBIN; k += blockDim.x) hist[k] = 0;
    __syncthreads();
    const int nb0 = (g.nc[0] + 3) >> 2, nb1 = (g.nc[1] + 3) >> 2, nb2 = (g.nc[2] + 3) >> 2;
    const int64_t nblk = (int64_t)nb0 * nb1 * nb2;
    int mine = 0;
    for (int64_t q = (int64_t)blockIdx.x * blockDim.x + threadIdx.x; q < nblk; q += (int64_t)gridDim.x * blockDim.x) {
        const int b2 = (int)(q % nb2), b1 = (int)((q / nb2) % nb1), b0 = (int)(q / ((int64_t)nb2 * nb1));
        const int x1 = min(b0 * 4 + 4, g.nc[0]), y1 = min(b1 * 4 + 4, g.nc[1]), z0 = b2 * 4, z1 = min(z0 + 4, g.nc[2]);
        bool any = false;
        for (int a = b0 * 4; a < x1; ++a)
            for (int c = b1 * 4; c < y1; ++c) {
                const int64_t col = ((int64_t)a * g.nc[1] + c) * g.nc[2];
                any = any || cell_start[col + z1] > cell_start[col + z0];
            }
        if (any) {
            mine += (x1 - b0 * 4) * (y1 - b1 * 4) * (z1 - z0);
            for (int a = b0 * 4; a < x1; ++a)
                for (int c = b1 * 4; c < y1; ++c) {
                    const int64_t col = ((int64_t)a * g.nc[1] + c) * g.nc[2];
                    for (int k = z0; k < z1; ++k) {
                        const int len = cell_start[col + min(k + 2, g.nc[2])] - cell_start[col + max(k - 1, 0)];
                        atomicAdd(&hist[1 + min(len, 97)], 1);
                    }
                }
        }
    }
#pragma unroll
    for (int d = 32; d >= 1; d >>= 1) mine += __shfl_xor(mine, d, 64);
    if ((threadIdx.x & 63) == 0 && mine) atomicAdd(&hist[0], mine);
    __syncthreads();
    for (int k = threadIdx.x; k < GridStats::NBIN; k += blockDim.x)
        if (hist[k]) atomicAdd(&out[k], hist[k]);
}

namespace {
struct StatEntry { int64_t N, ncell; int device; int *host; unsigned calls; };
std::mutex g_stat_mu;
std::vector<StatEntry> g_stat;
}

}

int grid_stats_hint(Scope &sc, const CellGrid &cg, int64_t N, GridStats *out)
{
    using namespace lane;
    hipStream_t st = sc.stream();
    int device = 0;
    (void)hipGetDevice(&device);
    std::lock_guard<std::mutex> lk(g_stat_mu);
    auto count = [&](int *host_dst) -> int {
        int *dcnt = sc.alloc_n<int>(GridStats::NBIN);
        if (sc.failed())
            return sc.error();
        MDH_HIP(hipMemsetAsync(dcnt, 0, sizeof(int) * GridStats::NBIN, st));
        const int blocks = (int)std::min<int64_t>((cg.g.ncell / 64 + 255) / 256 + 1, 2048);
        hipLaunchKernelGGL(k_grid_stats, dim3(blocks), dim3(256), 0, st, cg.cell_start, cg.g, dcnt);
        MDH_HIP(hipMemcpyAsync(host_dst, dcnt, sizeof(int) * GridStats::NBIN, hipMemcpyDeviceToHost, st));
        return MDH_OK;
    };
    auto read = [&](const int *host) {
        for (int k = 0; k < GridStats::NBIN; ++k) out->v[k] = ((const volatile int *)host)[k];
        if (out->v[0] <= 0) out->v[0] = (int)std::min<int64_t>(cg.g.ncell, 2147483647);
        out->last_listed = ((const volatile int *)host)[GridStats::NBIN];
        out->listed_sink = const_cast<int *>(host) + GridStats::NBIN;
    };
    for (auto &e : g_stat)
        if (e.N == N && e.ncell == cg.g.ncell && e.device == device) {
            read(e.host);
            if ((++e.calls & 7u) == 0)
                MDH_TRY(count(e.host));
            return MDH_OK;
        }
    int *host = nullptr;
    if (g_stat.size() >= 64) {
        host = g_stat.front().host;
        g_stat.erase(g_stat.begin());
    } else {
        MDH_HIP(hipHostMalloc(reinterpret_cast<void **>(&host), sizeof(int) * (GridStats::NBIN + 1), hipHostMallocDefault));
    }
    host[GridStats::NBIN] = -1;
    MDH_TRY(count(host));
    MDH_HIP(hipStreamSynchronize(st));
    read(host);
    g_stat.push_back(StatEntry{N, cg.g.ncell, device, host, 0u});
    return MDH_OK;
}

namespace lane {

static size_t lds_bytes(int cap, int64_t M, bool tk8, int rw, bool fcna = false)
{
    const size_t wave = std::max<size_t>((size_t)rw * (size_t)ticket_row((int)M, false) * (tk8 ? 1 : 2), 256);
    const size_t tk = (size_t)NW * wave;
    return (size_t)cap * 16 + (size_t)cap * 16 + (size_t)cap * 8 + (size_t)CEN_CAP * 4 + (size_t)(cap + (cap & 1)) * 2 + ((tk + 15) & ~(size_t)15);
}

}

static int lane_refusal(const DBox &b, const Grid &g, int64_t M)
{
    if (g.mode != 0 || M <= 0 || M > 128) return -1;
    for (int d = 0; d < 3; ++d)
        if (g.nc[d] < (b.pbc[d] ? 7 : 4)) return -3;
    return 0;
}

static LanePlan plan_lane_fresh(const DBox &b, const Grid &g, int64_t N, int64_t M, const GridStats &gs, double rc, bool fcna, bool count);

LanePlan plan_lane(const DBox &b, const Grid &g, int64_t N, int64_t M, const GridStats &gs, double rc, bool fcna, bool count)
{
    struct Key { int nc[3], pbc[3], tri; int64_t N, M; double rc, o[3], h[9], thick[3]; int fcna, count; int v[GridStats::NBIN]; };
    struct Memo { bool set = false; Key key; LanePlan plan; int hook[8]; };
    static thread_local Memo memo;
    Key k;
    std::memset(&k, 0, sizeof(k));
    for (int d = 0; d < 3; ++d) { k.nc[d] = g.nc[d]; k.pbc[d] = b.pbc[d]; k.o[d] = b.o[d]; k.thick[d] = b.thick[d]; }
    for (int d = 0; d < 9; ++d) k.h[d] = b.h[d];
    k.tri = b.tri; k.N = N; k.M = M; k.rc = rc; k.fcna = fcna; k.count = count;
    for (int q = 0; q < GridStats::NBIN; ++q) k.v[q] = gs.v[q];
    if (memo.set && std::memcmp(&k, &memo.key, sizeof(k)) == 0) {
        LanePlan p = memo.plan;
        p.last_listed = gs.last_listed;
        p.listed_sink = gs.listed_sink;
        lane::g_last_listed = gs.listed_sink ? *(volatile int *)gs.listed_sink : gs.last_listed;
        for (int q = 0; q < 8; ++q) lane::g_last_plan[q] = memo.hook[q];
        return p;
    }
    const LanePlan p = plan_lane_fresh(b, g, N, M, gs, rc, fcna, count);
    memo.key = k;
    memo.plan = p;
    for (int q = 0; q < 8; ++q) memo.hook[q] = lane::g_last_plan[q];
    memo.set = true;
    return p;
}

static LanePlan plan_lane_fresh(const DBox &b, const Grid &g, int64_t N, int64_t M, const GridStats &gs, double rc, bool fcna, bool count)
{
    using namespace lane;
    LanePlan p{};
// ... 40 lines not shown
                const double score = util * (0.35 + reuse) * (wpc == 16 ? 1.1 : (wpc == 12 ? 1.0 : (wpc == 8 ? 0.85 : (M > 64 ? 0.45 : 0.6))));
                if (score > best_score) { best_score = score; best = Shape{txy, tz}; best_cap = cap; best_wgs = wgs; best_rw = rw; }
            }
    }
    if (!best.txy) { g_last_plan[6] = -6; return p; }
    const int hmax = std::max(best.txy, best.tz) + 2;
    double E = ((double)hmax + 1.5) * rc;
    double big = E;
    if (b.tri) {
        double ext = 0, span = 0;
        for (int d = 0; d < 3; ++d) {
            const double len = std::sqrt(b.h[3 * d] * b.h[3 * d] + b.h[3 * d + 1] * b.h[3 * d + 1] + b.h[3 * d + 2] * b.h[3 * d + 2]);
            ext += ((double)((d == 2 ? best.tz : best.txy) + 2) + 1.5) * len * rc / b.thick[d];
            span += len;
        }
        E = ext;
        big = E + 3.0 * span;
        for (int d = 0; d < 3; ++d) big += std::fabs(b.o[d]);
        big *= 4.0;
    } else {
        for (int d = 0; d < 3; ++d) big = std::max(big, std::fabs(b.o[d]) + (double)(img::MAX_M + 2) * std::fabs(b.h[d * 4]) + E);
    }
    const double du = std::ldexp(E, -24) * 1.01 + std::ldexp(big, -49);
    const double rcsq = rc * rc;
    const double tol = 2.0 * (11.0 * du * rc + 12.0 * std::ldexp(rcsq, -24));
    float c = (float)(rcsq - tol);
    while ((double)c > rcsq - tol) c = std::nextafterf(c, -INFINITY);
    const double want = (rcsq - (double)c) + tol;
    float W = (float)want;
    while ((double)W < want) W = std::nextafterf(W, INFINITY);
    p.mid = c;
    p.T = W;
    p.txy = best.txy;
    p.tz = best.tz;
    p.cap = best_cap;
    p.tk8 = tk8;
    p.wgs = best_wgs;
    p.rw = best_rw;
    p.occupied = occ;
    p.last_listed = gs.last_listed;
    p.listed_sink = gs.listed_sink;
    g_last_listed = gs.listed_sink ? *(volatile int *)gs.listed_sink : gs.last_listed;
    p.full = (double)occ >= 0.98 * (double)g.ncell;
    g_last_plan[0] = p.txy; g_last_plan[1] = p.tz; g_last_plan[2] = p.cap; g_last_plan[3] = (int)lds_bytes(p.cap, M, tk8, p.rw, fcna);
    g_last_plan[4] = p.full | (p.tk8 ? 2 : 0) | (p.wgs << 2); g_last_plan[5] = (int)(1000.0 * pop); g_last_plan[6] = (int)std::min<int64_t>(occ, 2147483647); g_last_plan[7] = 1;
    return p;
}

int launch_neighbor_lane(Scope &sc, const CellGrid &cg, const LanePlan &plan, int64_t N, const DBox &b, double rc,
                         const RowsRequest &rows, TileFilter &tf)
{
    using namespace lane;
    const bool count = rows.pads == RowsRequest::COUNT_ONLY, fill_pads = rows.pads == RowsRequest::WRITE_PADS;
    int *const verlet = rows.verlet, *const nn = rows.nn, *const max_count = rows.max_count, *const pattern = count ? nullptr : rows.pattern;
    double *const dist = rows.dist; const int64_t M = count ? 1 : rows.M;
    int nt[3];
    for (int d = 0; d < 3; ++d) {
        const int T = d == 2 ? plan.tz : plan.txy;
        nt[d] = (cg.g.nc[d] + T - 1) / T;
    }
    const int64_t ntiles = (int64_t)nt[0] * nt[1] * nt[2];
    const Shape ts = make_shape(plan.txy, plan.tz, nt[1], nt[2]);
    const int nsub = ts.tz;
    unsigned *live = sc.alloc_n<unsigned>((size_t)ntiles);
    int *slot = sc.alloc_n<int>((size_t)ntiles + 1);
    int *tile_list = sc.alloc_n<int>((size_t)ntiles);
    int *flagged = sc.alloc_n<int>((size_t)ntiles);
    int *flagged2 = sc.alloc_n<int>((size_t)ntiles * (size_t)nsub);
    if (sc.failed())
        return sc.error();
    hipStream_t st = sc.stream();
    int per = (int)((ntiles + 7) / 8);
    int list_mode = 0, tile_base = 0, nt0_run = nt[0];
    if (plan.full) {
        tile_list = nullptr;
    } else if (cg.win_hi > cg.win_lo) {
        tile_list = nullptr;
        const int w_lo = cg.cen_hi > cg.cen_lo ? std::max(cg.win_lo, cg.cen_lo) : cg.win_lo, w_hi = cg.cen_hi > cg.cen_lo ? std::min(cg.win_hi, cg.cen_hi) : cg.win_hi;
        const int t_lo = w_lo / ts.txy, t_hi = (std::max(w_hi, w_lo + 1) - 1) / ts.txy;
        tile_base = t_lo * nt[1] * nt[2];
        nt0_run = t_hi - t_lo + 1;
        per = (int)(((int64_t)nt0_run * nt[1] * nt[2] + 7) / 8);
    } else {
        hipLaunchKernelGGL(k_tile_live, dim3(grid_for(ntiles, 256)), dim3(256), 0, st, cg.cell_start, cg.g, nt[0], nt[1], nt[2], ts, live);
        MDH_TRY(exclusive_scan_u32(sc, live, slot, ntiles));
        hipLaunchKernelGGL(k_tile_compact, dim3(grid_for(ntiles, 256)), dim3(256), 0, st, live, slot, (int)ntiles, tile_list);
        const int64_t est_live = std::max<int64_t>(1, plan.occupied / std::max(1, ts.txy * ts.txy * ts.tz) * 2);
        per = std::max(1, std::min(per, (int)((est_live + est_live / 4 + 7) / 8)));
        list_mode = 1;
    }
    const dim3 grid((unsigned)(per * 8));
    const size_t lds = lds_bytes(plan.cap, count ? 1 : M, plan.tk8, plan.rw, pattern != nullptr);
    const int cen_lo = cg.cen_hi > cg.cen_lo ? cg.cen_lo : 0, cen_hi = cg.cen_hi > cg.cen_lo ? cg.cen_hi : 0x7fffffff;
    const int Mi = (int)M, wp = fill_pads ? (rows.ids_only ? 3 : 1) : 0;
    const float negc = -plan.mid;
    const int nt2b = nt[2] * nsub;
    const bool slice_pass = plan.last_listed != 0;
    const dim3 grid2(1024u);
    const Shape ts2 = make_shape(ts.txy, 1, nt[1], nt2b);
    const bool indirect = !cg.pk;
    const lane::IndirectSrc isrc{cg.ix, cg.iy, cg.iz, cg.imv, cg.order};
#define MDH_LANE_PASS_I(COUNT, TRI, LOOP, FCNA, TK8, IND, GRID, JT0, ...)                                                                 \
    do {                                                                                                                                  \
        if (lds > 60 * 1024)                             \
            (void)hipFuncSetAttribute(reinterpret_cast<const void *>(&k_neighbor_lane<COUNT, TRI, LOOP, FCNA, TK8, IND>), hipFuncAttributeMaxDynamicSharedMemorySize, (int)lds); \
        hipLaunchKernelGGL((k_neighbor_lane<COUNT, TRI, LOOP, FCNA, TK8, IND>), GRID, dim3(NW * 64), lds, st, cg.pk, cg.cell_start, b, \
                           cg.g, rc, negc, plan.T, verlet, dist, nn, Mi, wp, plan.cap, cg.flags, nullptr, __VA_ARGS__, pattern, tf.cna_todo, JT0, plan.rw, tile_base, plan.listed_sink, \
                           cen_lo, cen_hi, isrc); \
    } while (0)
#define MDH_LANE_PASS(COUNT, TRI, LOOP, FCNA, TK8, GRID, JT0, ...)                                                                        \
    do {                                                                                                                                  \
        if (indirect) MDH_LANE_PASS_I(COUNT, TRI, LOOP, FCNA, TK8, true, GRID, JT0, __VA_ARGS__);                                         \
        else MDH_LANE_PASS_I(COUNT, TRI, LOOP, FCNA, TK8, false, GRID, JT0, __VA_ARGS__);                                                 \
    } while (0)
#define MDH_LANE_LAUNCH(COUNT, TRI, FCNA, TK8)                                                                                            \
    do {                                                                                                                                  \
        if (list_mode) {                                                                                                                  \
            MDH_LANE_PASS(COUNT, TRI, false, FCNA, TK8, grid, 0, nt[0], nt[1], nt[2], ts, tile_list, slot + ntiles, 1, max_count, flagged, nullptr, 0, 1, 2); \
            if ((int64_t)per * 8 < ntiles)                                                                                                \
                MDH_LANE_PASS(COUNT, TRI, true, FCNA, TK8, dim3(512), per, nt[0], nt[1], nt[2], ts, tile_list, slot + ntiles, 1, max_count, flagged, nullptr, 0, 1, 2); \
        } else {                                                                                                                          \
            MDH_LANE_PASS(COUNT, TRI, false, FCNA, TK8, grid, 0, nt0_run, nt[1], nt[2], ts, nullptr, slot + ntiles, 0, max_count, flagged, nullptr, 0, 1, 2); \
        }                                                                                                                                 \
        if (slice_pass)                                                                                                                   \
            MDH_LANE_PASS(COUNT, TRI, true, FCNA, TK8, grid2, 0, nt[0], nt[1], nt2b, ts2, nullptr, cg.flags + 2, 1, max_count, flagged2, flagged, nt[2], nsub, 3); \
    } while (0)
    if (count) {
        if (plan.tk8) { if (b.tri) MDH_LANE_LAUNCH(true, true, false, true); else MDH_LANE_LAUNCH(true, false, false, true); }
        else { if (b.tri) MDH_LANE_LAUNCH(true, true, false, false); else MDH_LANE_LAUNCH(true, false, false, false); }
    } else if (plan.tk8) {
        if (pattern) { if (b.tri) MDH_LANE_LAUNCH(false, true, true, true); else MDH_LANE_LAUNCH(false, false, true, true); }
        else { if (b.tri) MDH_LANE_LAUNCH(false, true, false, true); else MDH_LANE_LAUNCH(false, false, false, true); }
    } else {
        if (pattern) { if (b.tri) MDH_LANE_LAUNCH(false, true, true, false); else MDH_LANE_LAUNCH(false, false, true, false); }
        else { if (b.tri) MDH_LANE_LAUNCH(false, true, false, false); else MDH_LANE_LAUNCH(false, false, false, false); }
    }
#undef MDH_LANE_PASS
#undef MDH_LANE_PASS_I
#undef MDH_LANE_LAUNCH
    MDH_HIP(hipGetLastError());
    tf.flag = reinterpret_cast<const unsigned char *>(flagged2);
    tf.any = cg.flags + (slice_pass ? 3 : 2);
    tf.moved = cg.flags;
    tf.list = slice_pass ? flagged2 : flagged;
    tf.list_cap = (int)std::min<int64_t>(slice_pass ? ntiles * nsub : ntiles, 2147483647);
    tf.tile = ts.txy;
    tf.tile_z = slice_pass ? ts2.tz : ts.tz;
    tf.nt[0] = nt[0]; tf.nt[1] = nt[1]; tf.nt[2] = slice_pass ? nt2b : nt[2];
    tf.listed_sink = slice_pass ? nullptr : plan.listed_sink;
    return MDH_OK;
}

}

#ifdef MDH_STAMPS
extern "C" int mdh_debug_lane_stamps(unsigned long long *out, int n)
{
    return hipMemcpyFromSymbol(out, HIP_SYMBOL(mdh::lane::g_stamps), sizeof(unsigned long long) * (size_t)n) == hipSuccess ? 0 : 1;
}
#endif
namespace mdh { int lane_last_listed() { return lane::g_last_listed; } }
extern "C" int mdh_debug_neighbor_plan(int *plan8)
{
    for (int k = 0; k < 8; ++k) plan8[k] = mdh::lane::g_last_plan[k];
    mdh::lane::g_last_plan[7] = 0;
    return MDH_OK;
}

MDH_WARM_UNIT(neighbor_lane)
```

### mdapy_amd/csrc/runtime.hip

```cpp
#include "common.hpp"
#include <algorithm>
#include <atomic>
#include <cmath>
#include <cstdlib>
#include <cstring>
#include <mutex>
#include <vector>

extern "C" int mdh_warm(void);

namespace mdh {

static thread_local std::string g_err;

void set_error(const std::string &msg) { g_err = msg; }

int hip_fail(hipError_t e, const char *what, const char *file, int line)
{
    g_err = std::string("HIP error: ") + hipGetErrorString(e) + " in " + what + " (" + file + ":" + std::to_string(line) + ")";
    return MDH_ERR_HIP;
}

struct DoneEvent { hipEvent_t ev; hipStream_t stream; int refs; };
struct Block { void *p; size_t bytes; bool busy; int device; DoneEvent *done; int tag; };
static std::mutex g_mu;
static std::vector<Block> g_blocks;
static std::vector<DoneEvent *> g_event_pool;

static DoneEvent *event_acquire(hipStream_t st)
{
    DoneEvent *e = nullptr;
    if (!g_event_pool.empty()) {
        e = g_event_pool.back();
        g_event_pool.pop_back();
    } else {
        e = new DoneEvent{nullptr, nullptr, 0};
        if (hipEventCreateWithFlags(&e->ev, hipEventDisableTiming) != hipSuccess) { delete e; return nullptr; }
    }
    e->stream = st;
    e->refs = 0;
    return e;
}

static void event_release(DoneEvent *e)
{
    if (e && --e->refs == 0)
        g_event_pool.push_back(e);
}

Scope::Scope(void *stream) : stream_(static_cast<hipStream_t>(stream))
{
    device_ = 0;
    int n = 0;
    hipError_t e = hipGetDeviceCount(&n);
    if (e != hipSuccess || n < 1) {
        set_error(std::string("HIP error: no ROCm device available (") + hipGetErrorString(e) + "); mdapy_amd needs an AMD GPU (gfx950)");
        failed_ = true;
        err_ = MDH_ERR_HIP;
        return;
    }
    (void)hipGetDevice(&device_);
    static std::atomic<unsigned long long> warmed{0};
    static const bool want = [] { const char *e = std::getenv("MDAPY_HIP_WARM"); return !(e && e[0] == '0'); }();
    if (want && device_ < 64 && !((warmed.load(std::memory_order_relaxed) >> device_) & 1ull)) {
        warmed.fetch_or(1ull << device_, std::memory_order_relaxed);
        (void)mdh_warm();
    }
}

Scope::~Scope()
{
    if (nheld_ == 0)
        return;
    for (int i = 0; i < nheld_; ++i)
        if (held_keep_[i] == KEEP_ZERO || held_keep_[i] == KEEP_TODO)
            (void)hipMemsetAsync(held_[i], 0, held_keep_[i] == KEEP_TODO ? std::min<size_t>(512, held_bytes_[i]) : held_bytes_[i], stream_);
    std::lock_guard<std::mutex> lk(g_mu);
    DoneEvent *done = event_acquire(stream_);
    if (done && hipEventRecord(done->ev, stream_) != hipSuccess) {
        (void)hipStreamSynchronize(stream_);
        g_event_pool.push_back(done);
        done = nullptr;
    } else if (!done) {
        (void)hipStreamSynchronize(stream_);
    }
    for (int i = 0; i < nheld_; ++i)
        for (auto &b : g_blocks)
            if (b.p == held_[i]) {
                event_release(b.done);
                b.done = done;
                if (done) ++done->refs;
                b.busy = false;
                break;
            }
    if (done && done->refs == 0)
        g_event_pool.push_back(done);
}

void *Scope::alloc(size_t bytes) { return alloc_impl(bytes, KEEP_NONE); }

void *Scope::alloc_kept(size_t bytes, Keep tag) { return alloc_impl(bytes, (int)tag); }

void Scope::keep_confirm(void *p)
{
    for (int i = 0; i < nheld_; ++i)
        if (held_[i] == p) held_keep_[i] |= 0x80;
}

void *Scope::alloc_impl(size_t bytes, int tag)
{
    if (failed_)
        return nullptr;
    if (nheld_ >= kMaxHeld) { set_error("internal: too many scratch buffers in one call"); failed_ = true; return nullptr; }
    bytes = (bytes + 255) & ~size_t(255);
    if (bytes == 0) bytes = 256;
    std::lock_guard<std::mutex> lk(g_mu);
    int best = -1, best_any = -1;
    for (size_t i = 0; i < g_blocks.size(); ++i) {
        const Block &b = g_blocks[i];
        if (b.busy || b.device != device_ || b.bytes < bytes || b.tag != tag)
            continue;
        if (best_any < 0 || b.bytes < g_blocks[best_any].bytes)
            best_any = (int)i;
        if ((!b.done || b.done->stream == stream_) && (best < 0 || b.bytes < g_blocks[best].bytes))
            best = (int)i;
    }
    const bool fits = best >= 0 && g_blocks[best].bytes <= 2 * bytes + (1u << 20);
    if (!fits && bytes > (size_t(4) << 20))
        best = best_any;
    if (tag != KEEP_NONE && best < 0)
        best = best_any;
    if (best >= 0 && (tag != KEEP_NONE || g_blocks[best].bytes <= 2 * bytes + (1u << 20))) {
        Block &b = g_blocks[best];
        if (b.done && b.done->stream != stream_)
            (void)hipStreamWaitEvent(stream_, b.done->ev, 0);
        b.busy = true;
        held_[nheld_] = b.p;
        held_keep_[nheld_] = (unsigned char)tag;
        held_bytes_[nheld_++] = b.bytes;
        return b.p;
    }
    if (tag != KEEP_NONE)
        bytes = (bytes + bytes / 8 + 4095) & ~size_t(4095);
    void *p = nullptr;
    hipError_t e = hipMalloc(&p, bytes);
    if (e != hipSuccess) {
        for (size_t i = 0; i < g_blocks.size();) {
            if (!g_blocks[i].busy && g_blocks[i].device == device_) { (void)hipFree(g_blocks[i].p); event_release(g_blocks[i].done); g_blocks.erase(g_blocks.begin() + i); }
            else ++i;
        }
        e = hipMalloc(&p, bytes);
    }
    if (e != hipSuccess) {
        set_error(std::string("device allocation of ") + std::to_string(bytes) + " bytes failed: " + hipGetErrorString(e));
        failed_ = true;
        return nullptr;
    }
    if (tag != KEEP_NONE) {
        e = hipMemsetAsync(p, 0, bytes, stream_);
        if (e != hipSuccess) { (void)hipFree(p); hip_fail(e, "hipMemsetAsync(kept block)", __FILE__, __LINE__); failed_ = true; err_ = MDH_ERR_HIP; return nullptr; }
    }
    g_blocks.push_back(Block{p, bytes, true, device_, nullptr, tag});
    held_[nheld_] = p;
    held_keep_[nheld_] = (unsigned char)tag;
    held_bytes_[nheld_++] = bytes;
    return p;
}

void reset_kept_blocks(int tag)
{
    (void)hipDeviceSynchronize();
    std::lock_guard<std::mutex> lk(g_mu);
    for (auto &b : g_blocks)
        if (b.tag == tag) (void)hipMemset(b.p, 0, b.bytes);
}

void *Scope::stage_raw(void *p, size_t bytes, int space, bool in, bool out)
{
    if (space == MDH_DEVICE || p == nullptr)
        return p;
    void *d = alloc(bytes);
    if (!d)
        return nullptr;
    if (in && bytes) {
        hipError_t e = hipMemcpyAsync(d, p, bytes, hipMemcpyHostToDevice, stream_);
        if (e != hipSuccess) { hip_fail(e, "hipMemcpyAsync(H2D)", __FILE__, __LINE__); failed_ = true; err_ = MDH_ERR_HIP; return nullptr; }
    }
    if (out) {
        if (nouts_ >= 16) { set_error("internal: too many staged outputs"); failed_ = true; return nullptr; }
// ... 388 lines not shown
```

Measured before the change: 7.661 billion atoms/s.

## Bin atoms into fixed-capacity per-cell slots instead of count-scan-scatter cell lists

Adds a slot-grid path in which the assign kernel writes atom ids directly into fixed-capacity per-cell slots (with a spill list for overflow), so the prefix scan and the separate scatter pass are skipped. A small kernel then sorts each cell's slots with a sorting network, and the neighbor-lane kernel and the tile and stats kernels are templated to read per-cell counts instead of cell_start offsets. A host-side history of oversized cells and a double-buffered count block decide whether the path is taken and avoid re-zeroing. Risks include extra memory for padded slots, a fallback that depends on host-visible big-cell flags, and more kernel variants.

New measurement: 7.864 billion atoms/s, median of 6. 1.03x the previous value.

```diff
diff --git a/include/mdapy_amd.h b/include/mdapy_amd.h
--- a/include/mdapy_amd.h
+++ b/include/mdapy_amd.h
@@ -30,6 +30,9 @@
 int mdh_prof_report(char *buf, int buflen);
 int mdh_debug_set_neighbor_variant(int variant);
 int mdh_debug_set_indirect(int on);
+int mdh_debug_set_slot_grid(int on);
+int mdh_debug_slot_grid_counters(int64_t *out4);
+int mdh_debug_slot_grid_rule(int ordered, int keyed, int windowed, int row_width, int64_t ncell, int64_t N, int seen, int big, int listed);
 int mdh_debug_neighbor_plan(int *plan8);
 int mdh_debug_set_fcna_variant(int variant);
 int mdh_debug_track_counters(int on);
diff --git a/mdapy_amd/_lib.py b/mdapy_amd/_lib.py
--- a/mdapy_amd/_lib.py
+++ b/mdapy_amd/_lib.py
@@ -31,6 +31,9 @@
     "mdh_prof_report": [vp, cint],
     "mdh_debug_set_neighbor_variant": [cint],
     "mdh_debug_set_indirect": [cint],
+    "mdh_debug_set_slot_grid": [cint],
+    "mdh_debug_slot_grid_counters": [vp],
+    "mdh_debug_slot_grid_rule": [cint, cint, cint, cint, i64, i64, cint, cint, cint],
     "mdh_debug_neighbor_plan": [vp],
     "mdh_debug_set_fcna_variant": [cint],
     "mdh_debug_track_counters": [cint],
diff --git a/mdapy_amd/csrc/cell_grid.hip b/mdapy_amd/csrc/cell_grid.hip
--- a/mdapy_amd/csrc/cell_grid.hip
+++ b/mdapy_amd/csrc/cell_grid.hip
@@ -3,18 +3,21 @@
 #include "assign_groups.hpp"
 #include <algorithm>
 #include <atomic>
+#include <mutex>
+#include <vector>
 
 namespace mdh {
 static std::atomic<int> g_indirect{[] { const char *e = std::getenv("MDH_INDIRECT"); return e ? std::atoi(e) : 1; }()};
 
 struct CellPlanes { int p0, p1, p2, p3; int *bad; };
-template <bool TRI, int K>
+template <bool TRI, int K, bool SLOT = false>
 __global__ __launch_bounds__(256) void k_assign(const double *__restrict__ x, const double *__restrict__ y,
                                                 const double *__restrict__ z, int64_t N, DBox b, Grid g,
                                                 int wrap_first, int2 *__restrict__ ent,
                                                 unsigned *__restrict__ cell_count, unsigned *__restrict__ ctl, unsigned gen,
                                                 double slack, unsigned short *__restrict__ mv, CellPlanes win,
-                                                CellGrid::Packed *__restrict__ rec, int drop_absent)
+                                                CellGrid::Packed *__restrict__ rec, int drop_absent, int *__restrict__ slots = nullptr,
+                                                int2 *__restrict__ spill = nullptr, unsigned *__restrict__ spill_n = nullptr, int64_t slot_hi = 0)
 {
     const int lane = threadIdx.x & 63;
     const int64_t i0 = ((int64_t)blockIdx.x * (blockDim.x >> 6) + (threadIdx.x >> 6)) * (64 * K) + lane;
@@ -90,6 +93,14 @@
     for (int k = 0; k < K; ++k) {
         const unsigned bs = __shfl(base[k], head[k], 64);
         const int64_t i = i0 + 64 * k;
+        if (SLOT) {
+            if (i < N && cells[k] >= 0) {
+                const unsigned s = bs + (unsigned)slot[k];
+                if (s < (unsigned)SLOT_CAP) slots[slot_pos(cells[k], (int)s, slot_hi)] = (int)i;
+                else spill[atomicAdd(spill_n, 1u)] = make_int2(cells[k], (int)i);
+            }
+            continue;
+        }
         if (i < N)
             ent[i] = make_int2(cells[k], (int)(bs + (unsigned)slot[k]));
     }
@@ -320,14 +331,24 @@
         if (u < n) order[s + u] = id[u];
 }
 
+__device__ __forceinline__ void report_big_cell(unsigned *__restrict__ ctl, unsigned gen, int *__restrict__ sink, int n)
+{
+    if (__hip_atomic_load(&ctl[3], __ATOMIC_RELAXED, __HIP_MEMORY_SCOPE_AGENT) == gen)
+        return;
+    __hip_atomic_store(&ctl[3], gen, __ATOMIC_RELAXED, __HIP_MEMORY_SCOPE_AGENT);
+    sink[1] = n;
+}
+
 __global__ __launch_bounds__(256) void k_sort_cells(const int *__restrict__ cell_start, int *__restrict__ order,
-                                                    int64_t ncell, const int64_t *__restrict__ key, int *__restrict__ tmp)
+                                                    int64_t ncell, const int64_t *__restrict__ key, int *__restrict__ tmp,
+                                                    unsigned *__restrict__ ctl = nullptr, unsigned gen = 0, int *__restrict__ big_sink = nullptr)
 {
     int64_t c = (int64_t)blockIdx.x * blockDim.x + threadIdx.x;
     if (c >= ncell)
         return;
     const int s = cell_start[c], e = cell_start[c + 1];
     const int n = e - s;
+    if (big_sink && n > SLOT_CAP) report_big_cell(ctl, gen, big_sink, n);
     if (n <= 1)
         return;
     if (n <= 4) {
@@ -394,6 +415,44 @@
             order[s + larger] = mine;
         }
     }
+}
+
+__global__ __launch_bounds__(256) void k_sort_slots(const unsigned *__restrict__ count, int *__restrict__ slots, int64_t ncell,
+                                                    unsigned *__restrict__ idle, int64_t idle_n, unsigned *__restrict__ ctl, unsigned gen,
+                                                    int *__restrict__ big_sink, int *__restrict__ flags, int64_t slot_hi)
+{
+    const int64_t c = (int64_t)blockIdx.x * blockDim.x + threadIdx.x;
+    if (c == 0) {
+        flags[0] = ctl[1] == gen ? 1 : 0; flags[1] = 0; flags[2] = 0; flags[3] = 0;
+        flags[4] = ctl[2] == gen ? 1 : 0; flags[5] = 0; flags[6] = 0; flags[7] = 0;
+    }
+    if (c < idle_n) idle[c] = 0u;
+    if (c >= ncell)
+        return;
+    const int full = (int)count[c];
+    if (full > SLOT_CAP) report_big_cell(ctl, gen, big_sink, full);
+    const int n = min(full, SLOT_CAP);
+    if (n <= 1)
+        return;
+    int4 *cell = reinterpret_cast<int4 *>(slots + 4 * c), *cell_hi = reinterpret_cast<int4 *>(slots + slot_hi + 4 * c);
+    auto ce = [](int &a, int &b) { const int hi = max(a, b), lo = min(a, b); a = hi; b = lo; };
+    int4 q0 = cell[0];
+    int id[8] = {q0.x, n > 1 ? q0.y : INT32_MIN, n > 2 ? q0.z : INT32_MIN, n > 3 ? q0.w : INT32_MIN, INT32_MIN, INT32_MIN, INT32_MIN, INT32_MIN};
+    if (SLOT_CAP == 4 || n <= 4) {
+        ce(id[0], id[1]); ce(id[2], id[3]); ce(id[0], id[2]); ce(id[1], id[3]); ce(id[1], id[2]);
+        cell[0] = make_int4(id[0], id[1], id[2], id[3]);
+        return;
+    }
+    const int4 q1 = cell_hi[0];
+    id[4] = q1.x; id[5] = n > 5 ? q1.y : INT32_MIN; id[6] = n > 6 ? q1.z : INT32_MIN; id[7] = n > 7 ? q1.w : INT32_MIN;
+    ce(id[0], id[1]); ce(id[2], id[3]); ce(id[4], id[5]); ce(id[6], id[7]);
+    ce(id[0], id[2]); ce(id[1], id[3]); ce(id[4], id[6]); ce(id[5], id[7]);
+    ce(id[1], id[2]); ce(id[5], id[6]);
+    ce(id[0], id[4]); ce(id[1], id[5]); ce(id[2], id[6]); ce(id[3], id[7]);
+    ce(id[2], id[4]); ce(id[3], id[5]);
+    ce(id[1], id[2]); ce(id[3], id[4]); ce(id[5], id[6]);
+    cell[0] = make_int4(id[0], id[1], id[2], id[3]);
+    cell_hi[0] = make_int4(id[4], id[5], id[6], id[7]);
 }
 
 __global__ __launch_bounds__(256) void k_gather(const double *__restrict__ x, const double *__restrict__ y,
@@ -567,6 +626,56 @@
     if (threadIdx.x == 0) *flag = 4 * s_far > 1024 ? 1 : 0;
 }
 
+static std::atomic<int> g_slot_grid{[] { const char *e = std::getenv("MDH_SLOT_GRID"); return e ? std::atoi(e) : 1; }()};
+static const bool g_slot_force = [] { const char *e = std::getenv("MDH_SLOT_GRID_FORCE"); return e && std::atoi(e) != 0; }();
+static std::atomic<int> g_last_slot_build{0};
+int last_grid_was_slot() { return g_last_slot_build.load(std::memory_order_relaxed); }
+static std::mutex g_slot_mu;
+struct SlotHistory { int64_t N, ncell; int device; int *host; };
+struct SlotBlock { void *p; int next; int64_t dirty[2]; };
+static std::vector<SlotHistory *> g_slot_hist;
+static std::atomic<SlotHistory *> g_last_hist{nullptr};
+static std::vector<SlotBlock *> g_slot_blocks;
+
+static int slot_history(int64_t N, int64_t ncell, SlotHistory **out)
+{
+    int device = 0;
+    (void)hipGetDevice(&device);
+    std::lock_guard<std::mutex> lk(g_slot_mu);
+    for (SlotHistory *h : g_slot_hist)
+        if (h->N == N && h->ncell == ncell && h->device == device) { *out = h; return MDH_OK; }
+    SlotHistory *h = nullptr;
+    if (g_slot_hist.size() >= 64) {
+        h = g_slot_hist.front();
+        g_slot_hist.erase(g_slot_hist.begin());
+    } else {
+        int *host = nullptr;
+        MDH_HIP(hipHostMalloc(reinterpret_cast<void **>(&host), 2 * sizeof(int), hipHostMallocDefault));
+        h = new SlotHistory{};
+        h->host = host;
+    }
+    h->N = N; h->ncell = ncell; h->device = device;
+    h->host[0] = -1; h->host[1] = 0;
+    g_slot_hist.push_back(h);
+    *out = h;
+    return MDH_OK;
+}
+static SlotBlock *slot_block_state(void *p)
+{
+    std::lock_guard<std::mutex> lk(g_slot_mu);
+    for (SlotBlock *b : g_slot_blocks)
+        if (b->p == p) return b;
+    g_slot_blocks.push_back(new SlotBlock{p, 0, {0, 0}});
+    return g_slot_blocks.back();
+}
+
+bool slot_grid_rule(bool ordered, bool keyed, bool windowed, int row_width, int64_t ncell, int64_t N, bool seen, bool big, int listed)
+{
+    if (!ordered || keyed || windowed || row_width > 16) return false;
+    if (ncell > 2 * N || ncell * SLOT_CAP >= (int64_t(1) << 31)) return false;
+    return seen && !big && listed == 0;
+}
+
 int build_cell_grid(Scope &sc, const double *x, const double *y, const double *z, int64_t N, const DBox &b, const GridRequest &rq,
                     CellGrid &cg)
 {
@@ -578,28 +687,59 @@
     const Grid &g = cg.g;
     hipStream_t st = sc.stream();
 
-    unsigned *cell_count = static_cast<unsigned *>(sc.alloc_kept(sizeof(unsigned) * (size_t)g.ncell, Scope::KEEP_ZERO));
-    unsigned *ctl = static_cast<unsigned *>(sc.alloc_kept(scan_ctl_bytes(g.ncell), Scope::KEEP_SCAN));
-    cg.flags = sc.alloc_n<int>(8);
-    cg.cell_start = sc.alloc_n<int>((size_t)g.ncell + 1);
-    int2 *ent = sc.alloc_n<int2>((size_t)N);
-    int *rank = reinterpret_cast<int *>(ent);
-    cg.order = sc.alloc_n<int>((size_t)N + 4);
-    unsigned short *mv = sc.alloc_n<unsigned short>((size_t)N);
     cg.xs = cg.ys = cg.zs = nullptr;
     cg.mvs = nullptr;
     cg.pk = nullptr;
-    CellGrid::Packed *rec = nullptr;
-    int *rec_flag = nullptr;
     cg.ix = cg.iy = cg.iz = nullptr;
     cg.imv = nullptr;
+    cg.slot_cap = 0; cg.spill = nullptr; cg.n_spill = nullptr; cg.n_binned = N;
+    cg.big_stamp = nullptr; cg.big_gen = 0; cg.big_sink = nullptr;
+    int *rec_flag = nullptr;
+    bool indirect = false;
     if (packed) {
         if (!scattered && N >= (int64_t(1) << 18)) {
             const OrderHint h = order_hint(1, N, g.ncell, x);
             scattered = h.word && *(volatile int *)h.word != 0;
             if (h.word && h.sample) rec_flag = h.word;
         }
-        const bool indirect = g_indirect.load(std::memory_order_relaxed) != 0 && !scattered && rq.sort_desc && (double)N <= 6.0 * (double)g.ncell && rq.row_width <= 16;
+        indirect = g_indirect.load(std::memory_order_relaxed) != 0 && !scattered && rq.sort_desc && (double)N <= 6.0 * (double)g.ncell && rq.row_width <= 16;
+    }
+    SlotHistory *hist = nullptr;
+    bool slot = false;
+    const bool windows = window.set || centre.set;
+    if (packed && rq.slots_ok && slot_grid_rule(indirect, rq.sort_key != nullptr, windows, rq.row_width, g.ncell, N, true, false, 0)) {
+        MDH_TRY(slot_history(N, g.ncell, &hist));
+        g_last_hist.store(hist, std::memory_order_relaxed);
+        const int last = *(volatile int *)hist->host;
+        const bool seen = last >= 0, big = last > 0;
+        slot = g_slot_grid.load(std::memory_order_relaxed) != 0 && (g_slot_force ||
+               slot_grid_rule(indirect, rq.sort_key != nullptr, windows, rq.row_width, g.ncell, N, seen, big, lane_listed_hint(N, g.ncell)));
+    }
+    unsigned *cell_count = nullptr, *slot_block = nullptr, *slot_idle = nullptr;
+    int64_t slot_idle_n = 0;
+    SlotBlock *sb = nullptr;
+    if (slot) {
+        slot_block = static_cast<unsigned *>(sc.alloc_kept(2 * sizeof(unsigned) * (size_t)(g.ncell + 128), Scope::KEEP_SLOT));
+        if (slot_block) {
+            const size_t half = sc.held_bytes(slot_block) / 8;
+            sb = slot_block_state(slot_block);
+            cell_count = slot_block + (size_t)sb->next * half + 64;
+            slot_idle = slot_block + (size_t)(1 - sb->next) * half;
+            slot_idle_n = std::min<int64_t>(sb->dirty[1 - sb->next], (int64_t)half);
+        }
+    } else {
+        cell_count = static_cast<unsigned *>(sc.alloc_kept(sizeof(unsigned) * (size_t)g.ncell, Scope::KEEP_ZERO));
+    }
+    unsigned *ctl = static_cast<unsigned *>(sc.alloc_kept(scan_ctl_bytes(g.ncell), Scope::KEEP_SCAN));
+    cg.flags = sc.alloc_n<int>(8);
+    cg.cell_start = slot ? reinterpret_cast<int *>(cell_count) : sc.alloc_n<int>((size_t)g.ncell + 1);
+    int2 *ent = sc.alloc_n<int2>((size_t)N);
+    int *rank = reinterpret_cast<int *>(ent);
+    cg.order = sc.alloc_n<int>(slot ? (size_t)g.ncell * SLOT_CAP + 4 : (size_t)N + 4);
+    const int64_t slot_hi = 4 * g.ncell;
+    unsigned short *mv = sc.alloc_n<unsigned short>((size_t)N);
+    CellGrid::Packed *rec = nullptr;
+    if (packed) {
         if (!indirect) cg.pk = sc.alloc_n<CellGrid::Packed>((size_t)N);
         if (scattered) rec = sc.alloc_n<CellGrid::Packed>((size_t)N);
     } else {
@@ -658,12 +798,37 @@
     const unsigned gen = next_scan_gen();
     const bool assign4 = N >= (int64_t)1 << 20 && !scattered;
 #define MDH_ASSIGN(TRI, K) hipLaunchKernelGGL((k_assign<TRI, K>), dim3(grid_for(N, 256 * K)), dim3(256), 0, st, x, y, z, N, b, g, (int)rq.wrap_first, ent, cell_count, ctl, gen, slack, mv, win, rec, packed ? 1 : 0)
+#define MDH_ASSIGN_SLOT(TRI, K) hipLaunchKernelGGL((k_assign<TRI, K, true>), dim3(grid_for(N, 256 * K)), dim3(256), 0, st, x, y, z, N, b, g, (int)rq.wrap_first, (int2 *)nullptr, cell_count, ctl, gen, slack, mv, win, rec, 1, cg.order, ent, cell_count - 64, slot_hi)
+    if (slot) {
+        if (b.tri) { if (assign4) MDH_ASSIGN_SLOT(true, 4); else MDH_ASSIGN_SLOT(true, 1); }
+        else { if (assign4) MDH_ASSIGN_SLOT(false, 4); else MDH_ASSIGN_SLOT(false, 1); }
+        hipLaunchKernelGGL(k_sort_slots, dim3(grid_for(std::max<int64_t>(g.ncell, slot_idle_n), 256)), dim3(256), 0, st, cell_count, cg.order, g.ncell,
+                           slot_idle, slot_idle_n, ctl, gen, hist->host, cg.flags, slot_hi);
+        MDH_HIP(hipGetLastError());
+        {
+            std::lock_guard<std::mutex> lk(g_slot_mu);
+            sb->dirty[1 - sb->next] = 0;
+            sb->dirty[sb->next] = g.ncell + 64;
+            sb->next = 1 - sb->next;
+        }
+        sc.keep_confirm(slot_block);
+        cg.big_stamp = ctl + 3; cg.big_gen = gen; cg.big_sink = hist->host;
+        cg.slot_cap = SLOT_CAP;
+        cg.slot_hi = slot_hi;
+        cg.spill = ent;
+        cg.n_spill = cell_count - 64;
+        cg.ix = x; cg.iy = y; cg.iz = z; cg.imv = mv;
+        g_last_slot_build = 1;
+        return MDH_OK;
+    }
+    g_last_slot_build = 0;
     if (b.tri) {
         if (assign4) MDH_ASSIGN(true, 4); else MDH_ASSIGN(true, 1);
     } else {
         if (assign4) MDH_ASSIGN(false, 4); else MDH_ASSIGN(false, 1);
     }
 #undef MDH_ASSIGN
+#undef MDH_ASSIGN_SLOT
     auto scan_piece = [&](int64_t from, int64_t to, unsigned use_gen, int *flags) {
         launch_scan_gen(st, cell_count + from, cg.cell_start + from, to - from, ctl, use_gen, true, flags);
     };
@@ -696,7 +861,9 @@
         if (!windowed && !rq.sort_key && (double)N > 6.0 * (double)g.ncell) {
             hipLaunchKernelGGL(k_sort_cells_dense, dim3(grid_for(g.ncell, 32)), dim3(256), 0, st, cg.cell_start, cg.order, g.ncell, rank);
         } else if (!windowed) {
-            hipLaunchKernelGGL(k_sort_cells, dim3(grid_for(g.ncell, 256)), dim3(256), 0, st, cg.cell_start, cg.order, g.ncell, rq.sort_key, rank);
+            hipLaunchKernelGGL(k_sort_cells, dim3(grid_for(g.ncell, 256)), dim3(256), 0, st, cg.cell_start, cg.order, g.ncell, rq.sort_key, rank, ctl, gen,
+                               hist ? hist->host : (int *)nullptr);
+            if (hist) { cg.big_stamp = ctl + 3; cg.big_gen = gen; cg.big_sink = hist->host; }
         } else {
             hipLaunchKernelGGL(k_sort_cells, dim3(grid_for((p1 - p0) * plane, 256)), dim3(256), 0, st, cg.cell_start + p0 * plane, cg.order, (p1 - p0) * plane, rq.sort_key, rank);
             if (p3 > p2)
@@ -743,6 +910,28 @@
 }
 
 int mdh_debug_set_indirect(int on) { return g_indirect.exchange(on ? 1 : 0); }
+int mdh_debug_set_slot_grid(int on)
+{
+    if (on == 2) {
+        std::lock_guard<std::mutex> lk(g_slot_mu);
+        for (SlotHistory *h : g_slot_hist) h->host[0] = -1;
+    }
+    return g_slot_grid.exchange(on ? 1 : 0);
+}
+int mdh_debug_slot_grid_counters(int64_t *out4)
+{
+    const SlotHistory *h = g_last_hist.load(std::memory_order_relaxed);
+    const int last = h ? ((const volatile int *)h->host)[0] : 0, big = h ? ((const volatile int *)h->host)[1] : 0;
+    out4[0] = last_grid_was_slot();
+    out4[1] = last > 0 ? 1 : 0;
+    out4[2] = out4[1] ? big : 0;
+    out4[3] = SLOT_CAP;
+    return MDH_OK;
+}
+int mdh_debug_slot_grid_rule(int ordered, int keyed, int windowed, int row_width, int64_t ncell, int64_t N, int seen, int big, int listed)
+{
+    return slot_grid_rule(ordered != 0, keyed != 0, windowed != 0, row_width, ncell, N, seen != 0, big != 0, listed) ? 1 : 0;
+}
 }
 
 MDH_WARM_UNIT(cell_grid)
diff --git a/mdapy_amd/csrc/common.hpp b/mdapy_amd/csrc/common.hpp
--- a/mdapy_amd/csrc/common.hpp
+++ b/mdapy_amd/csrc/common.hpp
@@ -110,9 +110,10 @@
     hipStream_t stream() const { return stream_; }
     void *alloc(size_t bytes);
     template <class T> T *alloc_n(size_t n) { return static_cast<T *>(alloc((n ? n : 1) * sizeof(T))); }
-    enum Keep { KEEP_NONE = 0, KEEP_ZERO = 1, KEEP_SCAN = 2, KEEP_TODO = 3 };
+    enum Keep { KEEP_NONE = 0, KEEP_ZERO = 1, KEEP_SCAN = 2, KEEP_TODO = 3, KEEP_SLOT = 4 };
     void *alloc_kept(size_t bytes, Keep tag);
     void keep_confirm(void *p);
+    size_t held_bytes(const void *p) const;
 
     template <class T> T *stage(T *p, size_t n, int space, bool in, bool out)
     {
diff --git a/mdapy_amd/csrc/grid.hpp b/mdapy_amd/csrc/grid.hpp
--- a/mdapy_amd/csrc/grid.hpp
+++ b/mdapy_amd/csrc/grid.hpp
@@ -37,7 +37,22 @@
     Packed *pk;
     const double *ix = nullptr, *iy = nullptr, *iz = nullptr;
     const unsigned short *imv = nullptr;
-};
+    int slot_cap = 0;
+    int64_t slot_hi = 0;
+    const int2 *spill = nullptr;
+    const unsigned *n_spill = nullptr;
+    int64_t n_binned = 0;
+    const unsigned *big_stamp = nullptr;
+    unsigned big_gen = 0;
+    int *big_sink = nullptr;
+};
+#ifndef MDH_SLOT_CAP
+#define MDH_SLOT_CAP 8
+#endif
+constexpr int SLOT_CAP = MDH_SLOT_CAP;
+static_assert(SLOT_CAP == 4 || SLOT_CAP == 8, "a cell's slots are one or two 16-byte loads");
+__host__ __device__ __forceinline__ int64_t slot_pos(int64_t c, int k, int64_t hi) { return c * 4 + k + (k >= 4 ? hi - 4 : 0); }
+struct SlotSpill { const int2 *list = nullptr; const unsigned *n = nullptr; int64_t hi = 0; };
 struct SortedView {
     const double *xs, *ys, *zs;
     const int *order;
@@ -75,6 +90,7 @@
     int tile = 1, tile_z = 1;
     int nt[3] = {1, 1, 1};
     int *listed_sink = nullptr;
+    const unsigned *big_stamp = nullptr; unsigned big_gen = 0; int *big_sink = nullptr;
 };
 TiledPlan plan_tiled(const DBox &b, const Grid &g, int64_t N, int64_t M, int64_t occupied_cells);
 int occupied_cells_hint(Scope &sc, const CellGrid &cg, int64_t N, int64_t *occupied);
@@ -112,6 +128,7 @@
 };
 int grid_stats_hint(Scope &sc, const CellGrid &cg, int64_t N, GridStats *out);
 LanePlan plan_lane(const DBox &b, const Grid &g, int64_t N, int64_t M, const GridStats &gs, double rc, bool fcna, bool count);
+int lane_listed_hint(int64_t N, int64_t ncell);
 int lane_last_listed();
 int launch_neighbor_lane(Scope &sc, const CellGrid &cg, const LanePlan &plan, int64_t N, const DBox &b, double rc,
                          const RowsRequest &rows, TileFilter &tf);
@@ -173,7 +190,9 @@
     const int64_t *sort_key = nullptr;
     Atoms atoms = SORTED_ARRAYS;
     int row_width = 0;
-};
+    bool slots_ok = false;
+};
+bool slot_grid_rule(bool ordered, bool keyed, bool windowed, int row_width, int64_t ncell, int64_t N, bool seen, bool big, int listed);
 int build_cell_grid(Scope &sc, const double *x, const double *y, const double *z, int64_t N, const DBox &b, const GridRequest &rq,
                     CellGrid &cg);
 
diff --git a/mdapy_amd/csrc/neighbor.hip b/mdapy_amd/csrc/neighbor.hip
--- a/mdapy_amd/csrc/neighbor.hip
+++ b/mdapy_amd/csrc/neighbor.hip
@@ -10,16 +10,93 @@
 static int *g_moved_probe = nullptr;
 int g_neighbor_variant = 0;
 
-template <bool TRI, int MODE>
+__device__ __forceinline__ int next_id_below(const SortedView &sv, const SlotSpill &sp, int64_t cell, int prev)
+{
+    int best = -1;
+    for (int u = 0; u < SLOT_CAP; ++u) {
+        const int v = sv.order[slot_pos(cell, u, sp.hi)];
+        if (v < prev && v > best) best = v;
+    }
+    const unsigned ns = *sp.n;
+    for (unsigned w = 0; w < ns; ++w) {
+        const int2 e = sp.list[w];
+        if ((int64_t)e.x == cell && e.y < prev && e.y > best) best = e.y;
+    }
+    return best;
+}
+__device__ __forceinline__ int slot_cell_atom(const SortedView &sv, const SlotSpill &sp, int64_t cell, int k)
+{
+    if (k < SLOT_CAP)
+        return sv.order[slot_pos(cell, k, sp.hi)];
+    k -= SLOT_CAP;
+    const unsigned ns = *sp.n;
+    for (unsigned w = 0; w < ns; ++w) {
+        const int2 e = sp.list[w];
+        if ((int64_t)e.x == cell && k-- == 0) return e.y;
+    }
+    return -1;
+}
+
+template <bool TRI, int MODE, bool SLOT = false>
 __device__ __forceinline__ int neighbor_one(const SortedView &sv, const int *__restrict__ cell_start, const DBox &b,
                                             const Grid &g, double rc, int *__restrict__ verlet, double *__restrict__ dist,
                                             int *__restrict__ nn, int64_t M, int64_t p, double xi, double yi, double zi, int c0, int c1,
-                                            int c2)
+                                            int c2, const SlotSpill &sp = SlotSpill{})
 {
     int cnt = 0;
-    const int i = sv.id_of(p);
+    const int i = SLOT ? (int)p : sv.id_of(p);
     const double rcsq = rc * rc;
     const int64_t row = (int64_t)i * M;
+    if constexpr (SLOT) {
+        auto candidate = [&](int j, double xq, double yq, double zq) {
+            if (j == i)
+                return;
+            double dx = xq - xi, dy = yq - yi, dz = zq - zi;
+            pbc<TRI>(b, dx, dy, dz);
+            const double d2 = dx * dx + dy * dy + dz * dz;
+            if (d2 <= rcsq) {
+                if (MODE != 0 && cnt < M) {
+                    verlet[row + cnt] = j;
+                    dist[row + cnt] = sqrt(d2);
+                }
+                ++cnt;
+            }
+        };
+        for (int a = c0 - 1; a <= c0 + 1; ++a) {
+            const int ca = pmod(a, g.nc[0]);
+            for (int bb = c1 - 1; bb <= c1 + 1; ++bb) {
+                const int64_t base = ((int64_t)ca * g.nc[1] + pmod(bb, g.nc[1])) * g.nc[2];
+                for (int seg = 0; seg < 3; ++seg) {
+                    const int64_t cell = base + pmod(c2 - 1 + seg, g.nc[2]);
+                    const int n = cell_start[cell];
+                    if (n > SLOT_CAP) {
+                        for (int j = next_id_below(sv, sp, cell, 0x7fffffff); j >= 0; j = next_id_below(sv, sp, cell, j))
+                            candidate(j, sv.xs[j], sv.ys[j], sv.zs[j]);
+                        continue;
+                    }
+                    for (int k0 = 0; k0 < n; k0 += 4) {
+                        double xq[4], yq[4], zq[4];
+                        int jq[4];
+#pragma unroll
+                        for (int u = 0; u < 4; ++u)
+                            sv.get(slot_pos(cell, min(k0 + u, n - 1), sp.hi), xq[u], yq[u], zq[u], jq[u]);
+#pragma unroll
+                        for (int u = 0; u < 4; ++u)
+                            if (k0 + u < n) candidate(jq[u], xq[u], yq[u], zq[u]);
+                    }
+                }
+            }
+        }
+        nn[i] = cnt;
+        if (MODE == 2) {
+            const double pad = rc + 1.0;
+            for (int64_t n = cnt; n < M; ++n) {
+                verlet[row + n] = -1;
+                dist[row + n] = pad;
+            }
+        }
+        return cnt;
+    }
     const bool zrun = (c2 >= 1) && (c2 + 1 < g.nc[2]);
     for (int a = c0 - 1; a <= c0 + 1; ++a) {
         const int ca = pmod(a, g.nc[0]);
@@ -71,17 +148,73 @@
     return cnt;
 }
 
-template <bool TRI, int MODE>
+template <bool TRI, int MODE, bool SLOT = false>
 __device__ __forceinline__ int neighbor_one_wave(const SortedView &sv, const int *__restrict__ cell_start, const DBox &b,
                                                  const Grid &g, double rc, int *__restrict__ verlet, double *__restrict__ dist,
                                                  int *__restrict__ nn, int64_t M, int64_t p, double xi, double yi, double zi, int c0,
-                                                 int c1, int c2)
+                                                 int c1, int c2, const SlotSpill &sp = SlotSpill{})
 {
     const int lane = (int)(threadIdx.x & 63);
     int cnt = 0;
-    const int i = sv.id_of(p);
+    const int i = SLOT ? (int)p : sv.id_of(p);
     const double rcsq = rc * rc;
     const int64_t row = (int64_t)i * M;
+    if constexpr (SLOT) {
+        for (int a = c0 - 1; a <= c0 + 1; ++a) {
+            const int ca = pmod(a, g.nc[0]);
+            for (int bb = c1 - 1; bb <= c1 + 1; ++bb) {
+                const int64_t base = ((int64_t)ca * g.nc[1] + pmod(bb, g.nc[1])) * g.nc[2];
+                for (int seg = 0; seg < 3; ++seg) {
+                    const int64_t cell = base + pmod(c2 - 1 + seg, g.nc[2]);
+                    const int n = cell_start[cell];
+                    if (n > SLOT_CAP) {
+                        for (int j = next_id_below(sv, sp, cell, 0x7fffffff); j >= 0; j = next_id_below(sv, sp, cell, j)) {
+                            double dx = sv.xs[j] - xi, dy = sv.ys[j] - yi, dz = sv.zs[j] - zi;
+                            pbc<TRI>(b, dx, dy, dz);
+                            const double d2 = dx * dx + dy * dy + dz * dz;
+                            if (j != i && d2 <= rcsq) {
+                                if (MODE != 0 && lane == 0 && cnt < M) {
+                                    verlet[row + cnt] = j;
+                                    dist[row + cnt] = sqrt(d2);
+                                }
+                                ++cnt;
+                            }
+                        }
+                        continue;
+                    }
+                    bool hit = false;
+                    int j = -1;
+                    double d2 = 0.0;
+                    if (lane < n) {
+                        double xq, yq, zq;
+                        sv.get(slot_pos(cell, lane, sp.hi), xq, yq, zq, j);
+                        double dx = xq - xi, dy = yq - yi, dz = zq - zi;
+                        pbc<TRI>(b, dx, dy, dz);
+                        d2 = dx * dx + dy * dy + dz * dz;
+                        hit = j != i && d2 <= rcsq;
+                    }
+                    const unsigned long long m = __ballot(hit);
+                    if (MODE != 0 && hit) {
+                        const int slot = cnt + __popcll(m & ((1ull << lane) - 1ull));
+                        if (slot < M) {
+                            verlet[row + slot] = j;
+                            dist[row + slot] = sqrt(d2);
+                        }
+                    }
+                    cnt += __popcll(m);
+                }
+            }
+        }
+        if (lane == 0) nn[i] = cnt;
+        if (MODE == 2) {
+            const double pad = rc + 1.0;
+            for (int64_t n = cnt + lane; n < M; n += 64) {
+                verlet[row + n] = -1;
+                dist[row + n] = pad;
+            }
+        }
+        return cnt;
+    }
     const bool zrun = (c2 >= 1) && (c2 + 1 < g.nc[2]);
     for (int a = c0 - 1; a <= c0 + 1; ++a) {
         const int ca = pmod(a, g.nc[0]);
@@ -134,25 +267,29 @@
     return cnt;
 }
 
-template <bool TRI, int MODE>
+template <bool TRI, int MODE, bool SLOT = false>
 __device__ __forceinline__ void neighbor_atoms_body(const SortedView &sv,
                                                   const int *__restrict__ cell_start, int64_t N, const DBox &b, const Grid &g,
                                                   double rc, int *__restrict__ verlet, double *__restrict__ dist,
                                                   int *__restrict__ nn, int64_t M, int *__restrict__ max_count,
-                                                  const TileFilter &tf)
+                                                  const TileFilter &tf, const SlotSpill &sp = SlotSpill{})
 {
     const bool take_all = tf.moved && *tf.moved != 0;
     if (tf.flag && !take_all && (tf.list || *tf.any == 0))
         return;
     int cnt = 0;
-    N = min(N, (int64_t)cell_start[g.ncell]);
+    if (!SLOT) N = min(N, (int64_t)cell_start[g.ncell]);
     for (int64_t base = (int64_t)blockIdx.x * blockDim.x; base < N; base += (int64_t)gridDim.x * blockDim.x) {
         const int64_t p = base + threadIdx.x;
         bool mine = p < N;
         int c0 = 0, c1 = 0, c2 = 0;
         double xi = 0, yi = 0, zi = 0;
+        if (SLOT && mine) {
+            xi = sv.xs[p]; yi = sv.ys[p]; zi = sv.zs[p];
+            mine = xi == xi;
+        }
         if (mine) {
-            { int idp; sv.get(p, xi, yi, zi, idp); }
+            if (!SLOT) { int idp; sv.get(p, xi, yi, zi, idp); }
             if (b.anypbc)
                 wrap<TRI>(b, xi, yi, zi);
             cell_coords<TRI>(b, g, xi, yi, zi, c0, c1, c2);
@@ -162,8 +299,8 @@
             }
         }
         if (mine) {
-            cnt = max(cnt, neighbor_one<TRI, MODE>(sv, cell_start, b, g, rc, verlet, dist, nn, M, p, xi, yi, zi, c0, c1, c2));
-            if (tf.cna_todo) defer(tf.cna_todo, sv.id_of(p));
+            cnt = max(cnt, neighbor_one<TRI, MODE, SLOT>(sv, cell_start, b, g, rc, verlet, dist, nn, M, p, xi, yi, zi, c0, c1, c2, sp));
+            if (tf.cna_todo) defer(tf.cna_todo, SLOT ? (int)p : sv.id_of(p));
         }
     }
     if (MODE == 0) {
@@ -178,19 +315,22 @@
     }
 }
 
-template <bool TRI, int MODE>
+template <bool TRI, int MODE, bool SLOT = false>
 __global__ __launch_bounds__(256) void k_neighbor(SortedView sv, const int *__restrict__ cell_start, int64_t N, DBox b, Grid g, double rc,
                                                   int *__restrict__ verlet, double *__restrict__ dist, int *__restrict__ nn, int64_t M,
-                                                  int *__restrict__ max_count, TileFilter tf)
-{
-    neighbor_atoms_body<TRI, MODE>(sv, cell_start, N, b, g, rc, verlet, dist, nn, M, max_count, tf);
-}
-
-template <bool TRI, int MODE>
+                                                  int *__restrict__ max_count, TileFilter tf, SlotSpill sp)
+{
+    if (tf.big_sink && blockIdx.x == 0 && threadIdx.x == 0)
+        *tf.big_sink = *tf.big_stamp == tf.big_gen ? 1 : 0;
+    neighbor_atoms_body<TRI, MODE, SLOT>(sv, cell_start, N, b, g, rc, verlet, dist, nn, M, max_count, tf, sp);
+}
+
+template <bool TRI, int MODE, bool SLOT = false>
 __device__ __forceinline__ void neighbor_tiles_body(const SortedView &sv,
                                                         const int *__restrict__ cell_start, const DBox &b, const Grid &g, double rc,
                                                         int *__restrict__ verlet, double *__restrict__ dist, int *__restrict__ nn,
-                                                        int64_t M, int *__restrict__ max_count, const TileFilter &tf)
+                                                        int64_t M, int *__restrict__ max_count, const TileFilter &tf,
+                                                        const SlotSpill &sp = SlotSpill{})
 {
     if (tf.moved && *tf.moved != 0)
         return;
@@ -208,6 +348,27 @@
         const int a = t0 * tf.tile + colq / tf.tile, c = t1 * tf.tile + colq % tf.tile;
         if (a < g.nc[0] && c < g.nc[1]) {
             const int64_t col = ((int64_t)a * g.nc[1] + c) * g.nc[2];
+            if constexpr (SLOT) {
+                int seen = 0;
+                for (int cz = z0; cz < z1; ++cz) {
+                    const int n = cell_start[col + cz];
+                    for (int k = 0; k < n; ++k, ++seen) {
+                        if (seen % (nwave * MOP_CHUNKS) != chunk * nwave + wave)
+                            continue;
+                        const int id = slot_cell_atom(sv, sp, col + cz, k);
+                        if (id < 0)
+                            continue;
+                        double xi = sv.xs[id], yi = sv.ys[id], zi = sv.zs[id];
+                        if (b.anypbc)
+                            wrap<TRI>(b, xi, yi, zi);
+                        int c0, c1, c2;
+                        cell_coords<TRI>(b, g, xi, yi, zi, c0, c1, c2);
+                        best = max(best, neighbor_one_wave<TRI, MODE, true>(sv, cell_start, b, g, rc, verlet, dist, nn, M, id, xi, yi, zi, c0, c1, c2, sp));
+                        if (tf.cna_todo && (threadIdx.x & 63) == 0) defer(tf.cna_todo, id);
+                    }
+                }
+                continue;
+            }
             const int s = cell_start[col + z0], e = cell_start[col + z1];
             for (int p = s + chunk * nwave + wave; p < e; p += nwave * MOP_CHUNKS) {
                 double xi, yi, zi;
@@ -229,23 +390,25 @@
     }
 }
 
-template <bool TRI, int MODE>
+template <bool TRI, int MODE, bool SLOT = false>
 __global__ __launch_bounds__(256) void k_neighbor_tiles(SortedView sv, const int *__restrict__ cell_start, DBox b, Grid g, double rc,
                                                         int *__restrict__ verlet, double *__restrict__ dist, int *__restrict__ nn, int64_t M,
-                                                        int *__restrict__ max_count, TileFilter tf)
-{
-    neighbor_tiles_body<TRI, MODE>(sv, cell_start, b, g, rc, verlet, dist, nn, M, max_count, tf);
-}
-
-template <bool TRI, int MODE>
+                                                        int *__restrict__ max_count, TileFilter tf, SlotSpill sp)
+{
+    neighbor_tiles_body<TRI, MODE, SLOT>(sv, cell_start, b, g, rc, verlet, dist, nn, M, max_count, tf, sp);
+}
+
+template <bool TRI, int MODE, bool SLOT = false>
 __global__ __launch_bounds__(256) void k_neighbor_mop(SortedView sv, const int *__restrict__ cell_start, int64_t N, DBox b, Grid g, double rc,
                                                       int *__restrict__ verlet, double *__restrict__ dist, int *__restrict__ nn, int64_t M,
-                                                      int *__restrict__ max_count, TileFilter tf)
+                                                      int *__restrict__ max_count, TileFilter tf, SlotSpill sp)
 {
     if (tf.listed_sink && blockIdx.x == 0 && threadIdx.x == 0)
         *tf.listed_sink = min(*tf.any, tf.list_cap);
-    if (tf.moved && *tf.moved != 0) neighbor_atoms_body<TRI, MODE>(sv, cell_start, N, b, g, rc, verlet, dist, nn, M, max_count, tf);
-    else neighbor_tiles_body<TRI, MODE>(sv, cell_start, b, g, rc, verlet, dist, nn, M, max_count, tf);
+    if (tf.big_sink && blockIdx.x == 0 && threadIdx.x == 0)
+        *tf.big_sink = *tf.big_stamp == tf.big_gen ? 1 : 0;
+    if (tf.moved && *tf.moved != 0) neighbor_atoms_body<TRI, MODE, SLOT>(sv, cell_start, N, b, g, rc, verlet, dist, nn, M, max_count, tf, sp);
+    else neighbor_tiles_body<TRI, MODE, SLOT>(sv, cell_start, b, g, rc, verlet, dist, nn, M, max_count, tf, sp);
 }
 
 template <int MODE>
@@ -253,17 +416,16 @@
                             double *dist, int *nn, int64_t M, int *max_count, TileFilter tf = TileFilter{})
 {
     dim3 grid(std::min(grid_for(N, 256), tf.list ? 2048 : 8192)), block(256);
+    const SlotSpill sp{cg.spill, cg.n_spill, cg.slot_hi};
+#define MDH_MOP(KERNEL, TRI, SLOT, ...) hipLaunchKernelGGL((KERNEL<TRI, MODE, SLOT>), grid, block, 0, st, view_of(cg), cg.cell_start, __VA_ARGS__, b, cg.g, rc, verlet, dist, nn, M, max_count, tf, sp)
     if (tf.list) {
-        if (b.tri)
-            hipLaunchKernelGGL((k_neighbor_mop<true, MODE>), grid, block, 0, st, view_of(cg), cg.cell_start, N, b, cg.g, rc, verlet, dist, nn, M, max_count, tf);
-        else
-            hipLaunchKernelGGL((k_neighbor_mop<false, MODE>), grid, block, 0, st, view_of(cg), cg.cell_start, N, b, cg.g, rc, verlet, dist, nn, M, max_count, tf);
+        if (cg.slot_cap) { if (b.tri) MDH_MOP(k_neighbor_mop, true, true, N); else MDH_MOP(k_neighbor_mop, false, true, N); }
+        else { if (b.tri) MDH_MOP(k_neighbor_mop, true, false, N); else MDH_MOP(k_neighbor_mop, false, false, N); }
         return;
     }
-    if (b.tri)
-        hipLaunchKernelGGL((k_neighbor<true, MODE>), grid, block, 0, st, view_of(cg), cg.cell_start, N, b, cg.g, rc, verlet, dist, nn, M, max_count, tf);
-    else
-        hipLaunchKernelGGL((k_neighbor<false, MODE>), grid, block, 0, st, view_of(cg), cg.cell_start, N, b, cg.g, rc, verlet, dist, nn, M, max_count, tf);
+    if (cg.slot_cap) { if (b.tri) MDH_MOP(k_neighbor, true, true, N); else MDH_MOP(k_neighbor, false, true, N); }
+    else { if (b.tri) MDH_MOP(k_neighbor, true, false, N); else MDH_MOP(k_neighbor, false, false, N); }
+#undef MDH_MOP
 }
 
 template <int L>
@@ -550,6 +712,7 @@
     if (!cg.flags_fresh) MDH_HIP(hipMemsetAsync(cg.flags + 2, 0, sizeof(int) * 2, st));
     cg.flags_fresh = false;
     TileFilter tf{};
+    tf.big_stamp = cg.big_stamp; tf.big_gen = cg.big_gen; tf.big_sink = cg.big_sink;
     bool done = false;
     if (g_neighbor_variant == 0) {
         GridStats gs;
@@ -563,7 +726,7 @@
             out.labelled = cna;
         }
     }
-    if (!done && !count && g_neighbor_variant != 1 && !b.tri) {
+    if (!done && !count && g_neighbor_variant != 1 && !b.tri && !cg.slot_cap) {
         int64_t occ = 0;
         MDH_TRY(occupied_cells_hint(sc, cg, N, &occ));
         const TiledPlan plan = plan_tiled(b, cg.g, N, rows.M, occ);
@@ -586,6 +749,7 @@
     GridRequest rq;
     rq.wrap_first = rq.sort_desc = true; rq.sort_key = key; rq.atoms = GridRequest::FOR_ROWS;
     rq.row_width = (int)std::min<int64_t>(row_width, 1 << 20);
+    rq.slots_ok = true;
     return rq;
 }
 
diff --git a/mdapy_amd/csrc/neighbor_lane.hip b/mdapy_amd/csrc/neighbor_lane.hip
--- a/mdapy_amd/csrc/neighbor_lane.hip
+++ b/mdapy_amd/csrc/neighbor_lane.hip
@@ -287,7 +287,7 @@
     return load_atom(src, src.order[q], coded);
 }
 
-template <bool COUNT, bool TRI, bool LOOP, bool FCNA, bool TK8, bool IND = false>
+template <bool COUNT, bool TRI, bool LOOP, bool FCNA, bool TK8, bool IND = false, bool SLOT = false>
 __global__ __launch_bounds__(NW * 64, (TK8 && (!FCNA || !LOOP)) ? 16 / NW : 1) void k_neighbor_lane(
     const CellGrid::Packed *__restrict__ pk, const int *__restrict__ cell_start, DBox b,
     Grid g, double rc, float negc, float W, int *__restrict__ verlet, double *__restrict__ dist, int *__restrict__ nn,
@@ -295,7 +295,7 @@
     int nt1, int nt2, Shape ts, const int *__restrict__ tile_list, const int *__restrict__ n_live, int list_mode,
     int *__restrict__ max_count, int *__restrict__ flagged, const int *__restrict__ parent, int parent_nt2, int nsub,
     int flag_slot, int *__restrict__ pattern, int *__restrict__ cna_todo, int jt0, int rw, int tile_base, int *__restrict__ listed_sink,
-    int cen_lo, int cen_hi, IndirectSrc isrc)
+    int cen_lo, int cen_hi, IndirectSrc isrc, int slot_hi)
 {
     const int TXY = ts.txy, TZ = ts.tz;
     const int coded = IND ? flags[4] : 0;
@@ -360,16 +360,25 @@
             const bool in1 = b.pbc[1] ? (g1 >= -1 && g1 <= g.nc[1]) : (g1 >= 0 && g1 < g.nc[1]);
             const bool in2 = b.pbc[2] ? (g2 >= -1 && g2 <= g.nc[2]) : (g2 >= 0 && g2 < g.nc[2]);
             if (in0 && in1 && in2) {
+                bool over = false;
                 const int a0 = g0 < 0 ? g0 + g.nc[0] : (g0 >= g.nc[0] ? g0 - g.nc[0] : g0);
                 const int a1 = g1 < 0 ? g1 + g.nc[1] : (g1 >= g.nc[1] ? g1 - g.nc[1] : g1);
                 const int a2 = g2 < 0 ? g2 + g.nc[2] : (g2 >= g.nc[2] ? g2 - g.nc[2] : g2);
                 const int c = (a0 * g.nc[1] + a1) * g.nc[2] + a2;
-                h.src = cell_start[c];
-                h.cnt = cell_start[c + 1] - h.src;
+                if (SLOT) {
+                    const int n = cell_start[c];
+                    h.src = c << 2;
+                    h.cnt = min(n, SLOT_CAP);
+                    over = n > SLOT_CAP;
+                } else {
+                    h.src = cell_start[c];
+                    h.cnt = cell_start[c + 1] - h.src;
+                }
                 const int n0 = g0 < 0 ? 1 : (g0 >= g.nc[0] ? -1 : 0);
                 const int n1 = g1 < 0 ? 1 : (g1 >= g.nc[1] ? -1 : 0);
                 const int n2 = g2 < 0 ? 1 : (g2 >= g.nc[2] ? -1 : 0);
                 h.img = (n0 + 1) | ((n1 + 1) << 2) | ((n2 + 1) << 4);
+                if (SLOT && over) h.img |= 64;
                 h.edge = (!b.pbc[0] && (a0 == 0 || a0 == g.nc[0] - 1)) || (!b.pbc[1] && (a1 == 0 || a1 == g.nc[1] - 1)) ||
                          (!b.pbc[2] && (a2 == 0 || a2 == g.nc[2] - 1));
                 h.centre = hx >= 1 && hx <= TXY && hy >= 1 && hy <= TXY && h.hz >= 1 && h.hz <= TZ && g0 < g.nc[0] && g1 < g.nc[1] && g2 < g.nc[2] &&
@@ -417,6 +426,7 @@
         bool ok = !(total > cap || ncentres > CEN_CAP);
         const bool no_centres = ncentres == 0;
         if (no_centres) ok = false;
+        if (SLOT && (img & 64)) s_flag[2] = 1;
         STAMP(2);
         if (ok && tid < NH && hz >= 1 && hz <= HZ - 2) {
             const unsigned k0 = (unsigned)off0 - hc(tid - 1), len = hc(tid - 1) + (unsigned)cnt + hc(tid + 1);
@@ -489,7 +499,8 @@
                     for (int v = 0; v < 4; ++v) {
                         if (k == 0) { a[v] = pa[v]; bb[v] = pb[v]; c[v] = pc[v]; d[v] = pd[v]; m[v] = pm[v]; }
                         else {
-                            const int q = src + min(k + v, cnt - 1);
+                            const int kv = min(k + v, cnt - 1);
+                            const int q = src + kv + (SLOT && kv >= 4 ? slot_hi : 0);
                             const CellGrid::Packed r = load_record<IND>(pk, isrc, q, coded);
                             a[v] = r.x; bb[v] = r.y; c[v] = r.z; d[v] = r.id; m[v] = r.code;
                         }
@@ -506,7 +517,8 @@
                     int nd[4], nm[4];
 #pragma unroll
                     for (int v = 0; v < 4; ++v) {
-                        const int q = src + min(k + 4 + v, cnt - 1);
+                        const int kv = min(k + 4 + v, cnt - 1);
+                        const int q = src + kv + (SLOT && kv >= 4 ? slot_hi : 0);
                         const CellGrid::Packed r = load_record<IND>(pk, isrc, q, coded);
                         na[v] = r.x; nb[v] = r.y; nc[v] = r.z; nd[v] = r.id; nm[v] = r.code;
                     }
@@ -891,8 +903,17 @@
     }
 }
 
+__device__ __forceinline__ int column_atoms(const int *__restrict__ cell_start, int64_t col, int z0, int z1, int slot)
+{
+    if (!slot)
+        return cell_start[col + z1] - cell_start[col + z0];
+    int n = 0;
+    for (int k = z0; k < z1; ++k) n += cell_start[col + k];
+    return n;
+}
+
 __global__ __launch_bounds__(256) void k_tile_live(const int *__restrict__ cell_start, Grid g, int nt0, int nt1, int nt2, Shape ts,
-                                                   unsigned *__restrict__ live)
+                                                   unsigned *__restrict__ live, int slot)
 {
     const int t = blockIdx.x * blockDim.x + threadIdx.x;
     if (t >= nt0 * nt1 * nt2)
@@ -903,7 +924,7 @@
     for (int a = t0 * ts.txy; a < min((t0 + 1) * ts.txy, g.nc[0]) && !any; ++a)
         for (int c = t1 * ts.txy; c < min((t1 + 1) * ts.txy, g.nc[1]) && !any; ++c) {
             const int64_t col = ((int64_t)a * g.nc[1] + c) * g.nc[2];
-            any = cell_start[col + z1] > cell_start[col + z0];
+            any = column_atoms(cell_start, col, z0, z1, slot) > 0;
         }
     live[t] = any ? 1u : 0u;
 }
@@ -915,7 +936,7 @@
     if (t < ntiles && live[t]) tile_list[slot[t]] = t;
 }
 
-__global__ __launch_bounds__(256) void k_grid_stats(const int *__restrict__ cell_start, Grid g, int *__restrict__ out)
+__global__ __launch_bounds__(256) void k_grid_stats(const int *__restrict__ cell_start, Grid g, int *__restrict__ out, int slot)
 {
     __shared__ int hist[GridStats::NBIN];
     for (int k = threadIdx.x; k < GridStats::NBIN; k += blockDim.x) hist[k] = 0;
@@ -930,7 +951,7 @@
         for (int a = b0 * 4; a < x1; ++a)
             for (int c = b1 * 4; c < y1; ++c) {
                 const int64_t col = ((int64_t)a * g.nc[1] + c) * g.nc[2];
-                any = any || cell_start[col + z1] > cell_start[col + z0];
+                any = any || column_atoms(cell_start, col, z0, z1, slot) > 0;
             }
         if (any) {
             mine += (x1 - b0 * 4) * (y1 - b1 * 4) * (z1 - z0);
@@ -938,7 +959,7 @@
                 for (int c = b1 * 4; c < y1; ++c) {
                     const int64_t col = ((int64_t)a * g.nc[1] + c) * g.nc[2];
                     for (int k = z0; k < z1; ++k) {
-                        const int len = cell_start[col + min(k + 2, g.nc[2])] - cell_start[col + max(k - 1, 0)];
+                        const int len = column_atoms(cell_start, col, max(k - 1, 0), min(k + 2, g.nc[2]), slot);
                         atomicAdd(&hist[1 + min(len, 97)], 1);
                     }
                 }
@@ -973,7 +994,7 @@
             return sc.error();
         MDH_HIP(hipMemsetAsync(dcnt, 0, sizeof(int) * GridStats::NBIN, st));
         const int blocks = (int)std::min<int64_t>((cg.g.ncell / 64 + 255) / 256 + 1, 2048);
-        hipLaunchKernelGGL(k_grid_stats, dim3(blocks), dim3(256), 0, st, cg.cell_start, cg.g, dcnt);
+        hipLaunchKernelGGL(k_grid_stats, dim3(blocks), dim3(256), 0, st, cg.cell_start, cg.g, dcnt, cg.slot_cap);
         MDH_HIP(hipMemcpyAsync(host_dst, dcnt, sizeof(int) * GridStats::NBIN, hipMemcpyDeviceToHost, st));
         return MDH_OK;
     };
@@ -1180,7 +1201,7 @@
         nt0_run = t_hi - t_lo + 1;
         per = (int)(((int64_t)nt0_run * nt[1] * nt[2] + 7) / 8);
     } else {
-        hipLaunchKernelGGL(k_tile_live, dim3(grid_for(ntiles, 256)), dim3(256), 0, st, cg.cell_start, cg.g, nt[0], nt[1], nt[2], ts, live);
+        hipLaunchKernelGGL(k_tile_live, dim3(grid_for(ntiles, 256)), dim3(256), 0, st, cg.cell_start, cg.g, nt[0], nt[1], nt[2], ts, live, cg.slot_cap);
         MDH_TRY(exclusive_scan_u32(sc, live, slot, ntiles));
         hipLaunchKernelGGL(k_tile_compact, dim3(grid_for(ntiles, 256)), dim3(256), 0, st, live, slot, (int)ntiles, tile_list);
         const int64_t est_live = std::max<int64_t>(1, plan.occupied / std::max(1, ts.txy * ts.txy * ts.tz) * 2);
@@ -1198,18 +1219,20 @@
     const Shape ts2 = make_shape(ts.txy, 1, nt[1], nt2b);
     const bool indirect = !cg.pk;
     const lane::IndirectSrc isrc{cg.ix, cg.iy, cg.iz, cg.imv, cg.order};
-#define MDH_LANE_PASS_I(COUNT, TRI, LOOP, FCNA, TK8, IND, GRID, JT0, ...)                                                                 \
+    const int slot_hi = cg.slot_cap ? (int)(cg.slot_hi - 4) : 0;
+#define MDH_LANE_PASS_I(COUNT, TRI, LOOP, FCNA, TK8, IND, SLOT, GRID, JT0, ...)                                                                 \
     do {                                                                                                                                  \
         if (lds > 60 * 1024)                             \
-            (void)hipFuncSetAttribute(reinterpret_cast<const void *>(&k_neighbor_lane<COUNT, TRI, LOOP, FCNA, TK8, IND>), hipFuncAttributeMaxDynamicSharedMemorySize, (int)lds); \
-        hipLaunchKernelGGL((k_neighbor_lane<COUNT, TRI, LOOP, FCNA, TK8, IND>), GRID, dim3(NW * 64), lds, st, cg.pk, cg.cell_start, b, \
+            (void)hipFuncSetAttribute(reinterpret_cast<const void *>(&k_neighbor_lane<COUNT, TRI, LOOP, FCNA, TK8, IND, SLOT>), hipFuncAttributeMaxDynamicSharedMemorySize, (int)lds); \
+        hipLaunchKernelGGL((k_neighbor_lane<COUNT, TRI, LOOP, FCNA, TK8, IND, SLOT>), GRID, dim3(NW * 64), lds, st, cg.pk, cg.cell_start, b, \
                            cg.g, rc, negc, plan.T, verlet, dist, nn, Mi, wp, plan.cap, cg.flags, nullptr, __VA_ARGS__, pattern, tf.cna_todo, JT0, plan.rw, tile_base, plan.listed_sink, \
-                           cen_lo, cen_hi, isrc); \
+                           cen_lo, cen_hi, isrc, slot_hi); \
     } while (0)
 #define MDH_LANE_PASS(COUNT, TRI, LOOP, FCNA, TK8, GRID, JT0, ...)                                                                        \
     do {                                                                                                                                  \
-        if (indirect) MDH_LANE_PASS_I(COUNT, TRI, LOOP, FCNA, TK8, true, GRID, JT0, __VA_ARGS__);                                         \
-        else MDH_LANE_PASS_I(COUNT, TRI, LOOP, FCNA, TK8, false, GRID, JT0, __VA_ARGS__);                                                 \
+        if (indirect && cg.slot_cap) MDH_LANE_PASS_I(COUNT, TRI, LOOP, FCNA, TK8, true, true, GRID, JT0, __VA_ARGS__);                    \
+        else if (indirect) MDH_LANE_PASS_I(COUNT, TRI, LOOP, FCNA, TK8, true, false, GRID, JT0, __VA_ARGS__);                             \
+        else MDH_LANE_PASS_I(COUNT, TRI, LOOP, FCNA, TK8, false, false, GRID, JT0, __VA_ARGS__);                                          \
     } while (0)
 #define MDH_LANE_LAUNCH(COUNT, TRI, FCNA, TK8)                                                                                            \
     do {                                                                                                                                  \
@@ -1258,9 +1281,22 @@
 }
 #endif
 namespace mdh { int lane_last_listed() { return lane::g_last_listed; } }
+namespace mdh { int last_grid_was_slot(); }
+namespace mdh {
+int lane_listed_hint(int64_t N, int64_t ncell)
+{
+    int device = 0;
+    (void)hipGetDevice(&device);
+    std::lock_guard<std::mutex> lk(lane::g_stat_mu);
+    for (auto &e : lane::g_stat)
+        if (e.N == N && e.ncell == ncell && e.device == device) return ((const volatile int *)e.host)[GridStats::NBIN];
+    return -1;
+}
+}
 extern "C" int mdh_debug_neighbor_plan(int *plan8)
 {
     for (int k = 0; k < 8; ++k) plan8[k] = mdh::lane::g_last_plan[k];
+    if (plan8[0] > 0 && mdh::last_grid_was_slot()) plan8[4] |= 256;
     mdh::lane::g_last_plan[7] = 0;
     return MDH_OK;
 }
diff --git a/mdapy_amd/csrc/runtime.hip b/mdapy_amd/csrc/runtime.hip
--- a/mdapy_amd/csrc/runtime.hip
+++ b/mdapy_amd/csrc/runtime.hip
@@ -73,7 +73,7 @@
     if (nheld_ == 0)
         return;
     for (int i = 0; i < nheld_; ++i)
-        if (held_keep_[i] == KEEP_ZERO || held_keep_[i] == KEEP_TODO)
+        if (held_keep_[i] == KEEP_ZERO || held_keep_[i] == KEEP_TODO || held_keep_[i] == KEEP_SLOT)
             (void)hipMemsetAsync(held_[i], 0, held_keep_[i] == KEEP_TODO ? std::min<size_t>(512, held_bytes_[i]) : held_bytes_[i], stream_);
     std::lock_guard<std::mutex> lk(g_mu);
     DoneEvent *done = event_acquire(stream_);
@@ -105,6 +105,13 @@
 {
     for (int i = 0; i < nheld_; ++i)
         if (held_[i] == p) held_keep_[i] |= 0x80;
+}
+
+size_t Scope::held_bytes(const void *p) const
+{
+    for (int i = 0; i < nheld_; ++i)
+        if (held_[i] == p) return held_bytes_[i];
+    return 0;
 }
 
 void *Scope::alloc_impl(size_t bytes, int tag)
```
